# crate-crypto/rust-eth-kzg

Measured on AMD Instinct MI355X. Metric: blobs/sec compute_cells_and_kzg_proofs (4096-pt blob), higher is better.
Workload: dtype u32

## Files before the change

include/c_eth_kzg_test_hooks.h:

```cpp
#ifndef C_ETH_KZG_TEST_HOOKS_H
#define C_ETH_KZG_TEST_HOOKS_H
#include "c_eth_kzg.h"
#ifdef __cplusplus
extern "C" {
#endif

int eth_kzg_amd_test_fr_ntt4096(const DASContext *ctx, const uint8_t *in, uint8_t *out, int inverse_dit);
int eth_kzg_amd_test_g1_fft128(const DASContext *ctx, const uint8_t *in, uint8_t *out, int n_lanes, int inverse);
int eth_kzg_amd_test_fixed_msm(const DASContext *ctx, const uint8_t *scalars, int n_msm, uint8_t *out);
int eth_kzg_amd_test_g1_decompress(const DASContext *ctx, const uint8_t *in, int n, int subgroup_check, int32_t *status,
                                   uint8_t *out);
int eth_kzg_amd_test_field_mul(const DASContext *ctx, const uint8_t *a, const uint8_t *b, uint8_t *out, int n,
                               int is_fp);

int eth_kzg_amd_test_sha256_many(const DASContext *ctx, uint64_t n, const uint8_t *prefix, uint64_t prefix_len, const uint8_t *d_body,
                                 uint64_t body_stride, uint64_t body_len, const uint8_t *d_tail, uint64_t tail_stride, uint64_t tail_len,
                                 uint8_t *d_out);

int eth_kzg_amd_test_verify_msm(const DASContext *ctx, int form, const uint8_t *points, int n_pts, const uint8_t *sc0, int n0,
                                const uint8_t *sc1, int n1, uint8_t *out96, int32_t *sub_status);

int eth_kzg_amd_test_verify_cells_partial_device(const DASContext *ctx, uint64_t n, const uint8_t *d_commitments,
                                                 const uint64_t *d_cell_indices, const uint8_t *d_cells, const uint8_t *d_proofs, uint64_t lo,
                                                 uint64_t hi, uint8_t *out96);
int eth_kzg_amd_test_verify_blob_batch_inputs(const DASContext *ctx, uint64_t n, int on_device, const void *blobs, const void *commitments,
                                              const void *proofs, uint8_t *out96, int32_t *verified);

int eth_kzg_amd_test_rs_decode(const DASContext *ctx, int R, const uint64_t *n_cells, const uint64_t *const *cell_indices,
                               const uint8_t *const *const *cells, int flat_source, int32_t *status, int32_t *deg,
                               uint8_t *zp, uint8_t *zeval, uint8_t *zcinv, uint8_t *coeffs);

int eth_kzg_amd_test_op_info(int op, int32_t *in_words, int32_t *out_words, int32_t *device_only, const char **name);
int eth_kzg_amd_test_op(const DASContext *ctx, int op, int n, const int32_t *in, int32_t *out, int on_device);

int eth_kzg_amd_test_table_info(const DASContext *ctx, int kind, int which, int64_t *out8, int32_t *piece_first_block, int max_pieces);
int eth_kzg_amd_test_table_audit(const DASContext *ctx, int kind, int which, uint64_t *visited, uint64_t *n_findings, int32_t *findings,
                                 int max_findings, double *ms);
int eth_kzg_amd_test_table_read(const DASContext *ctx, int kind, int which, int group, int window, int base, int d0, int n, uint32_t *out);
int eth_kzg_amd_test_table_audit_buffer(const DASContext *ctx, int c, int n_groups, int nb, const uint32_t *table, const uint8_t *bases,
                                        int on_device, uint64_t *visited, uint64_t *n_findings, int32_t *findings, int max_findings);

#ifdef __cplusplus
}
#endif
#endif
```

rust-eth-kzg_amd/__init__.py:

```python
import ctypes as C

import numpy as np
import os

_HERE = os.path.dirname(os.path.abspath(__file__))
LIB_PATH = os.path.join(_HERE, "libc_eth_kzg.so")
HOOKS_LIB_PATH = os.path.join(_HERE, "libc_eth_kzg_hooks.so")

BYTES_PER_BLOB = 131072
BYTES_PER_CELL = 2048
BYTES_PER_COMMITMENT = 48
BYTES_PER_PROOF = 48
CELLS_PER_EXT_BLOB = 128
FIELD_ELEMENTS_PER_BLOB = 4096
FIELD_ELEMENTS_PER_CELL = 64


class KzgError(Exception):
    """An operation the reference would report as `Err(..)` (CResult.status == Err)."""


class CResult(C.Structure):
    _fields_ = [("status", C.c_int), ("error_msg", C.c_void_p)]


VERIFY_PARTIAL_BYTES = 96
SETUP_NO_SUBGROUP_CHECK = 1
SETUP_CHECK_POWERS = 2
SETUP_G1_POINTS = 4096
SETUP_G2_POINTS = 65

EXPORTED_SYMBOLS = [
    "eth_kzg_das_context_new", "eth_kzg_das_context_free", "eth_kzg_free_error_message",
    "eth_kzg_blob_to_kzg_commitment", "eth_kzg_compute_cells_and_kzg_proofs", "eth_kzg_compute_cells",
    "eth_kzg_verify_cell_kzg_proof_batch", "eth_kzg_recover_cells_and_proofs",
    "eth_kzg_constant_bytes_per_cell", "eth_kzg_constant_bytes_per_proof", "eth_kzg_constant_cells_per_ext_blob",
    "eth_kzg_compute_kzg_proof", "eth_kzg_compute_blob_kzg_proof", "eth_kzg_verify_kzg_proof",
    "eth_kzg_verify_blob_kzg_proof", "eth_kzg_verify_blob_kzg_proof_batch",
    "eth_kzg_amd_das_context_new_on_device",
    "eth_kzg_amd_das_context_try_new", "eth_kzg_amd_das_context_new_on_devices", "eth_kzg_amd_context_devices",
    "eth_kzg_amd_das_context_new_with_setup", "eth_kzg_amd_das_context_new_with_setup_file", "eth_kzg_amd_setup_digest",
    "eth_kzg_amd_abi_version", "eth_kzg_amd_window_count", "eth_kzg_amd_glv_table",
    "eth_kzg_amd_compute_cells_and_kzg_proofs_batch", "eth_kzg_amd_blob_to_kzg_commitment_batch",
    "eth_kzg_amd_recover_cells_and_proofs_batch", "eth_kzg_amd_recover_cells_and_proofs_device",
    "eth_kzg_amd_verify_cell_kzg_proof_batch_partial", "eth_kzg_amd_verify_cell_kzg_proof_batch_combine",
    "eth_kzg_amd_compute_cells_and_kzg_proofs_device", "eth_kzg_amd_blob_to_kzg_commitment_device",
    "eth_kzg_amd_verify_cell_kzg_proof_batch_device", "eth_kzg_amd_verify_cell_kzg_proof_batch_many",
    "eth_kzg_amd_compute_blob_kzg_proof_batch", "eth_kzg_amd_compute_kzg_proof_batch",
    "eth_kzg_amd_compute_blob_kzg_proof_device", "eth_kzg_amd_compute_kzg_proof_device",
    "eth_kzg_amd_verify_blob_kzg_proof_batch_device",
    "eth_kzg_amd_table_bytes", "eth_kzg_amd_window_bits", "eth_kzg_amd_tables_ready", "eth_kzg_amd_table_groups_ready", "eth_kzg_amd_table_build_info", "eth_kzg_amd_linmap_info",
    "eth_kzg_amd_set_profiling", "eth_kzg_amd_get_stage_times",
    "eth_kzg_amd_comm_probe", "eth_kzg_amd_comm_unique_id", "eth_kzg_amd_comm_init", "eth_kzg_amd_comm_info",
    "eth_kzg_amd_all_gather", "eth_kzg_amd_comm_destroy",
    "eth_kzg_amd_compute_cells_and_kzg_proofs_batch_multi", "eth_kzg_amd_device_count",
]
TEST_HOOK_SYMBOLS = [
    "eth_kzg_amd_test_fr_ntt4096", "eth_kzg_amd_test_g1_fft128", "eth_kzg_amd_test_fixed_msm",
    "eth_kzg_amd_test_g1_decompress", "eth_kzg_amd_test_field_mul", "eth_kzg_amd_test_op_info", "eth_kzg_amd_test_op",
    "eth_kzg_amd_test_table_info", "eth_kzg_amd_test_table_audit", "eth_kzg_amd_test_table_read", "eth_kzg_amd_test_table_audit_buffer",
    "eth_kzg_amd_test_sha256_many", "eth_kzg_amd_test_verify_msm",
    "eth_kzg_amd_test_verify_cells_partial_device", "eth_kzg_amd_test_verify_blob_batch_inputs", "eth_kzg_amd_test_rs_decode",
]

_lib = None


def load_library():
    global _lib
    if _lib is not None:
        return _lib
    path = os.environ.get("ETH_KZG_AMD_LIB", LIB_PATH)
    if not os.path.exists(path):
        raise RuntimeError(
            f"{LIB_PATH} is missing: build the HIP extension first (python -c 'import __graft_entry__ as g; g.build()' "
            "or make -C rust-eth-kzg_amd/csrc). There is no CPU fallback.")
    lib = C.CDLL(path)
    P, U8P, U64 = C.c_void_p, C.c_char_p, C.c_uint64
    lib.eth_kzg_das_context_new.restype = P
    lib.eth_kzg_das_context_new.argtypes = [C.c_bool]
    lib.eth_kzg_amd_das_context_new_on_device.restype = P
    lib.eth_kzg_amd_das_context_new_on_device.argtypes = [C.c_bool, C.c_int]
    lib.eth_kzg_amd_das_context_try_new.restype = P
    lib.eth_kzg_amd_das_context_try_new.argtypes = [C.c_bool, C.c_int, C.c_double, C.POINTER(CResult)]
    lib.eth_kzg_das_context_free.argtypes = [P]
    lib.eth_kzg_free_error_message.argtypes = [P]
    for name, args in {
        "eth_kzg_blob_to_kzg_commitment": [P, U8P, P],
        "eth_kzg_compute_cells_and_kzg_proofs": [P, U8P, P, P],
        "eth_kzg_compute_cells": [P, U8P, P],
        "eth_kzg_verify_cell_kzg_proof_batch": [P, U64, P, U64, P, U64, P, U64, P, P],
        "eth_kzg_recover_cells_and_proofs": [P, U64, P, U64, P, P, P],
        "eth_kzg_compute_kzg_proof": [P, U8P, U8P, P, P],
        "eth_kzg_compute_blob_kzg_proof": [P, U8P, U8P, P],
        "eth_kzg_verify_kzg_proof": [P, U8P, U8P, U8P, U8P, P],
        "eth_kzg_verify_blob_kzg_proof": [P, U8P, U8P, U8P, P],
        "eth_kzg_verify_blob_kzg_proof_batch": [P, U64, P, U64, P, U64, P, P],
        "eth_kzg_amd_compute_cells_and_kzg_proofs_batch": [P, U64, P, P, P, P],
        "eth_kzg_amd_blob_to_kzg_commitment_batch": [P, U64, P, P, P],
        "eth_kzg_amd_recover_cells_and_proofs_batch": [P, U64, P, P, P, P, P, P, P],
        "eth_kzg_amd_verify_cell_kzg_proof_batch_partial": [P, U64, P, U64, P, U64, P, U64, P, U64, U64, P],
        "eth_kzg_amd_verify_cell_kzg_proof_batch_combine": [P, U64, U8P, P],
        "eth_kzg_amd_recover_cells_and_proofs_device": [P, U64, P, P, P, P, P, P],
        "eth_kzg_amd_compute_cells_and_kzg_proofs_device": [P, U64, P, P, P, P, P],
        "eth_kzg_amd_blob_to_kzg_commitment_device": [P, U64, P, P, P, P],
        "eth_kzg_amd_verify_cell_kzg_proof_batch_device": [P, U64, P, P, P, P, P, P],
        "eth_kzg_amd_verify_cell_kzg_proof_batch_many": [P, U64, P, P, P, P, P, P, P, P, P, P],
        "eth_kzg_amd_compute_blob_kzg_proof_batch": [P, U64, P, P, P, P],
        "eth_kzg_amd_compute_kzg_proof_batch": [P, U64, P, P, P, P, P],
        "eth_kzg_amd_compute_blob_kzg_proof_device": [P, U64, P, P, P, P, P],
        "eth_kzg_amd_compute_kzg_proof_device": [P, U64, P, P, P, P, P, P],
        "eth_kzg_amd_verify_blob_kzg_proof_batch_device": [P, U64, P, P, P, P, P],
        "eth_kzg_amd_comm_unique_id": [P],
        "eth_kzg_amd_comm_probe": [P, P, U64],
        "eth_kzg_amd_comm_info": [P, P, P],
        "eth_kzg_amd_comm_init": [P, U8P, C.c_int, C.c_int],
        "eth_kzg_amd_all_gather": [P, P, P, U64, P],
        "eth_kzg_amd_compute_cells_and_kzg_proofs_batch_multi": [P, U64, U64, P, P, P, P],
    }.items():
        fn = getattr(lib, name)
        fn.restype = CResult
        fn.argtypes = args
    for name in ("eth_kzg_constant_bytes_per_cell", "eth_kzg_constant_bytes_per_proof",
                 "eth_kzg_constant_cells_per_ext_blob"):
        getattr(lib, name).restype = U64
    lib.eth_kzg_amd_comm_destroy.argtypes = [P]
    lib.eth_kzg_amd_comm_destroy.restype = None
    lib.eth_kzg_amd_device_count.restype = C.c_int
    lib.eth_kzg_amd_table_bytes.restype = U64
    lib.eth_kzg_amd_table_bytes.argtypes = [P]
    lib.eth_kzg_amd_window_bits.argtypes = [P]
    lib.eth_kzg_amd_tables_ready.argtypes = [P, C.c_int]
    lib.eth_kzg_amd_tables_ready.restype = C.c_int
    lib.eth_kzg_amd_table_build_info.argtypes = [P, C.POINTER(C.c_double)]
    lib.eth_kzg_amd_table_build_info.restype = None
    lib.eth_kzg_amd_table_groups_ready.argtypes = [P]
    lib.eth_kzg_amd_table_groups_ready.restype = C.c_int
    lib.eth_kzg_amd_linmap_info.argtypes = [P, P]
    lib.eth_kzg_amd_linmap_info.restype = None
    lib.eth_kzg_amd_set_profiling.argtypes = [P, C.c_int]
    lib.eth_kzg_amd_set_profiling.restype = None
    lib.eth_kzg_amd_get_stage_times.argtypes = [P, P, P, C.c_int]
    lib.eth_kzg_amd_das_context_new_on_devices.restype = P
    lib.eth_kzg_amd_das_context_new_on_devices.argtypes = [C.c_bool, P, U64, C.c_double, C.POINTER(CResult)]
    lib.eth_kzg_amd_context_devices.restype = U64
    lib.eth_kzg_amd_context_devices.argtypes = [P, P, U64]
    lib.eth_kzg_amd_abi_version.restype = C.c_int
    if hasattr(lib, "eth_kzg_amd_das_context_new_with_setup"):
        lib.eth_kzg_amd_das_context_new_with_setup.restype = P
        lib.eth_kzg_amd_das_context_new_with_setup.argtypes = [P, U64, P, U64, C.c_uint32, C.c_bool, P, U64, C.c_double, C.POINTER(CResult)]
        lib.eth_kzg_amd_das_context_new_with_setup_file.restype = P
        lib.eth_kzg_amd_das_context_new_with_setup_file.argtypes = [P, U64, C.c_uint32, C.c_bool, P, U64, C.c_double, C.POINTER(CResult)]
        lib.eth_kzg_amd_setup_digest.restype = None
        lib.eth_kzg_amd_setup_digest.argtypes = [P, P]
    lib.eth_kzg_amd_window_count.argtypes = [P]
    lib.eth_kzg_amd_glv_table.argtypes = [P]
    for name, args in {
        "eth_kzg_amd_test_fr_ntt4096": [P, U8P, P, C.c_int],
        "eth_kzg_amd_test_g1_fft128": [P, U8P, P, C.c_int, C.c_int],
        "eth_kzg_amd_test_fixed_msm": [P, U8P, C.c_int, P],
        "eth_kzg_amd_test_g1_decompress": [P, U8P, C.c_int, C.c_int, P, P],
        "eth_kzg_amd_test_field_mul": [P, U8P, U8P, P, C.c_int, C.c_int],
        "eth_kzg_amd_test_op_info": [C.c_int, P, P, P, C.POINTER(C.c_char_p)],
        "eth_kzg_amd_test_op": [P, C.c_int, C.c_int, P, P, C.c_int],
        "eth_kzg_amd_test_table_info": [P, C.c_int, C.c_int, P, P, C.c_int],
        "eth_kzg_amd_test_table_audit": [P, C.c_int, C.c_int, P, P, P, C.c_int, P],
        "eth_kzg_amd_test_table_read": [P, C.c_int, C.c_int, C.c_int, C.c_int, C.c_int, C.c_int, C.c_int, P],
        "eth_kzg_amd_test_table_audit_buffer": [P, C.c_int, C.c_int, C.c_int, P, P, C.c_int, P, P, P, C.c_int],
        "eth_kzg_amd_test_sha256_many": [P, U64, P, U64, P, U64, U64, P, U64, U64, P],
        "eth_kzg_amd_test_verify_msm": [P, C.c_int, U8P, C.c_int, U8P, C.c_int, U8P, C.c_int, P, P],
        "eth_kzg_amd_test_verify_cells_partial_device": [P, U64, P, P, P, P, U64, U64, P],
        "eth_kzg_amd_test_verify_blob_batch_inputs": [P, U64, C.c_int, P, P, P, P, P],
        "eth_kzg_amd_test_rs_decode": [P, C.c_int, P, P, P, C.c_int, P, P, P, P, P, P],
    }.items():
        if hasattr(lib, name):
            getattr(lib, name).argtypes = args
    _lib = lib
    return lib


def present_masks(n, present):
    masks = np.zeros(2 * max(1, n), dtype=np.uint64)
    prev_row, prev_mask = None, 0
    for b in range(n):
        row = present[b]
        if row is prev_row and prev_row is not None:
            m = prev_mask
        else:
            m = 0
            for c in row:
                c = int(c)
                if not 0 <= c < CELLS_PER_EXT_BLOB:
                    raise KzgError("InvalidCellIndex")
                m |= 1 << c
            prev_row, prev_mask = row, m
        masks[2 * b] = m & 0xFFFFFFFFFFFFFFFF
        masks[2 * b + 1] = m >> 64
    return masks


def parse_trusted_setup_json(text):
    import json
    try:
        doc = json.loads(text)
    except ValueError as e:
        raise KzgError(f"InvalidSetup: not JSON ({e})")
    if not isinstance(doc, dict):
        raise KzgError("InvalidSetup: the trusted setup JSON is an object with g1_monomial and g2_monomial")
    out = []
    for key, size in (("g1_monomial", 48), ("g2_monomial", 96)):
        pts = doc.get(key)
        if not isinstance(pts, list):
            raise KzgError(f"InvalidSetup: {key} is missing")
        dec = []
        for i, h in enumerate(pts):
            if not isinstance(h, str) or not h.startswith("0x"):
                raise KzgError(f"InvalidSetup: {key}[{i}] is not a 0x-prefixed hex string")
            try:
                b = bytes.fromhex(h[2:])
            except ValueError:
                raise KzgError(f"InvalidSetup: {key}[{i}] is not hex")
            if len(b) != size:
                raise KzgError(f"InvalidSetup: {key}[{i}] has {len(b)} bytes, not {size}")
            dec.append(b)
        out.append(dec)
    return out[0], out[1]


def _ptr_array(bufs):
    arr = (C.c_void_p * max(1, len(bufs)))()
    keep = []
    for i, b in enumerate(bufs):
        if isinstance(b, (bytes, bytearray)):
            b = C.create_string_buffer(bytes(b), len(b))
        keep.append(b)
        arr[i] = C.addressof(b)
    return arr, keep


def _flat_ptrs(items, size):
    n = len(items)
    flat = np.frombuffer(b"".join(bytes(x) if not isinstance(x, bytes) else x for x in items), dtype=np.uint8) if n else np.zeros(1, np.uint8)
    ptrs = np.uint64(flat.ctypes.data) + np.arange(max(1, n), dtype=np.uint64) * np.uint64(size)
    return ptrs, flat


def _out_ptrs(n_outer, n_inner, size):
    flat = np.zeros(max(1, n_outer * n_inner * size), dtype=np.uint8)
    inner = np.uint64(flat.ctypes.data) + np.arange(max(1, n_outer * n_inner), dtype=np.uint64) * np.uint64(size)
    outer = np.uint64(inner.ctypes.data) + np.arange(max(1, n_outer), dtype=np.uint64) * np.uint64(n_inner * 8)
    return flat, inner, outer


def _split(flat, n_outer, n_inner, size):
    raw = flat.tobytes()
    return [[raw[(b * n_inner + k) * size:(b * n_inner + k + 1) * size] for k in range(n_inner)] for b in range(n_outer)]


def _vp(arr):
    return arr.ctypes.data_as(C.c_void_p)


class DASContext:

    device_index = 0

    def __init__(self, use_precomp=True, device=None, wait_tables=True, table_budget_gb=None, devices=None):
        self.device_index = int(device) if device is not None else int(os.environ.get("ETH_KZG_AMD_DEVICE", "0"))
        self._lib = load_library()
        if devices is not None:
            devs = np.array([int(d) for d in devices], dtype=np.int32)
            self.device_index = int(devs[0]) if len(devs) else 0
            res = CResult()
            self._ctx = C.c_void_p(self._lib.eth_kzg_amd_das_context_new_on_devices(
                bool(use_precomp), _vp(devs) if len(devs) else None, len(devs), float(table_budget_gb or 0.0), C.byref(res)))
            if not self._ctx.value:
                msg = C.cast(res.error_msg, C.c_char_p).value.decode() if res.error_msg else "unknown"
                self._lib.eth_kzg_free_error_message(res.error_msg)
                raise KzgError(msg)
        elif table_budget_gb is not None:
            res = CResult()
            self._ctx = C.c_void_p(self._lib.eth_kzg_amd_das_context_try_new(bool(use_precomp), self.device_index, float(table_budget_gb), C.byref(res)))
            if not self._ctx.value:
                msg = C.cast(res.error_msg, C.c_char_p).value.decode() if res.error_msg else "unknown"
                self._lib.eth_kzg_free_error_message(res.error_msg)
                raise KzgError(msg)
        elif device is None:
            self._ctx = C.c_void_p(self._lib.eth_kzg_das_context_new(bool(use_precomp)))
        else:
            self._ctx = C.c_void_p(self._lib.eth_kzg_amd_das_context_new_on_device(bool(use_precomp), int(device)))
        if not self._ctx.value:
            raise RuntimeError("eth_kzg_das_context_new returned NULL")
        if wait_tables:
            self.tables_ready(-1)

    @classmethod
    def from_trusted_setup(cls, g1_monomial, g2_monomial, *, subgroup_check=True, check_powers=False, use_precomp=True, devices=None,
                           table_budget_gb=None, wait_tables=True):
        def flat(pts, size):
            if isinstance(pts, (bytes, bytearray, memoryview)):
                raw = bytes(pts)
                if len(raw) % size:
                    raise KzgError(f"InvalidSetup: {len(raw)} bytes are not a whole number of {size}-byte points")
                return raw, len(raw) // size
            pts = [bytes(x) for x in pts]
            for i, x in enumerate(pts):
                if len(x) != size:
                    raise KzgError(f"InvalidSetup: point {i} has {len(x)} bytes, not {size}")
            return b"".join(pts), len(pts)
        g1, n1 = flat(g1_monomial, 48)
        g2, n2 = flat(g2_monomial, 96)
        self = cls.__new__(cls)
        self._lib = load_library()
        self._ctx = C.c_void_p(None)
        devs = np.array([int(d) for d in devices], dtype=np.int32) if devices is not None else None
        self.device_index = int(devs[0]) if devs is not None and len(devs) else int(os.environ.get("ETH_KZG_AMD_DEVICE", "0"))
        flags = (0 if subgroup_check else SETUP_NO_SUBGROUP_CHECK) | (SETUP_CHECK_POWERS if check_powers else 0)
        res = CResult()
        b1, b2 = C.create_string_buffer(g1, max(1, len(g1))), C.create_string_buffer(g2, max(1, len(g2)))
        self._ctx = C.c_void_p(self._lib.eth_kzg_amd_das_context_new_with_setup(
            C.addressof(b1), n1, C.addressof(b2), n2, flags, bool(use_precomp), _vp(devs) if devs is not None and len(devs) else None,
            len(devs) if devs is not None else 0, float(table_budget_gb or 0.0), C.byref(res)))
        if not self._ctx.value:
            msg = C.cast(res.error_msg, C.c_char_p).value.decode() if res.error_msg else "unknown"
            self._lib.eth_kzg_free_error_message(res.error_msg)
            raise KzgError(msg)
        if wait_tables:
            self.tables_ready(-1)
        return self

    @classmethod
    def from_trusted_setup_json(cls, text_or_path, *, check_powers=True, **kwargs):
        text = text_or_path
        if not str(text_or_path).lstrip().startswith("{"):
            with open(text_or_path) as f:
                text = f.read()
        g1, g2 = parse_trusted_setup_json(text)
        return cls.from_trusted_setup(g1, g2, check_powers=check_powers, **kwargs)

    @property
    def setup_digest(self):
        out = C.create_string_buffer(32)
        self._lib.eth_kzg_amd_setup_digest(self._ctx, out)
        return out.raw

    def devices(self):
        out = np.zeros(64, dtype=np.int32)
        n = int(self._lib.eth_kzg_amd_context_devices(self._ctx, _vp(out), 64))
        return [int(d) for d in out[:n]]

    def tables_ready(self, wait_ms=0):
        return int(self._lib.eth_kzg_amd_tables_ready(self._ctx, int(wait_ms)))

    def table_build_info(self):
        out = (C.c_double * 4)()
        self._lib.eth_kzg_amd_table_build_info(self._ctx, out)
        return {"hipmalloc_ms": round(out[0], 1), "longest_hipmalloc_ms": round(out[1], 1), "pieces": int(out[2]), "bytes": int(out[3])}

    def table_groups_ready(self):
        return int(self._lib.eth_kzg_amd_table_groups_ready(self._ctx))

    def close(self):
        if getattr(self, "_ctx", None) and self._ctx.value:
            self._lib.eth_kzg_das_context_free(self._ctx)
            self._ctx = C.c_void_p(None)

    def __del__(self):
        try:
            self.close()
        except Exception:
            pass

    @property
    def handle(self):
        return self._ctx

    def _check(self, res):
        if res.status != 0:
            msg = C.string_at(res.error_msg).decode() if res.error_msg else "error"
            self._lib.eth_kzg_free_error_message(res.error_msg)
            raise KzgError(msg)

    def blob_to_kzg_commitment(self, blob):
        if len(blob) != BYTES_PER_BLOB:
            raise KzgError("BlobHasInvalidLength")
        out = C.create_string_buffer(48)
        self._check(self._lib.eth_kzg_blob_to_kzg_commitment(self._ctx, bytes(blob), out))
        return out.raw

    def compute_cells_and_kzg_proofs(self, blob):
        if len(blob) != BYTES_PER_BLOB:
            raise KzgError("BlobHasInvalidLength")
        cells = [C.create_string_buffer(BYTES_PER_CELL) for _ in range(CELLS_PER_EXT_BLOB)]
        proofs = [C.create_string_buffer(48) for _ in range(CELLS_PER_EXT_BLOB)]
        ca, _k1 = _ptr_array(cells)
        pa, _k2 = _ptr_array(proofs)
        self._check(self._lib.eth_kzg_compute_cells_and_kzg_proofs(self._ctx, bytes(blob), ca, pa))
        return [c.raw for c in cells], [p.raw for p in proofs]

    def compute_cells(self, blob):
        if len(blob) != BYTES_PER_BLOB:
            raise KzgError("BlobHasInvalidLength")
        cells = [C.create_string_buffer(BYTES_PER_CELL) for _ in range(CELLS_PER_EXT_BLOB)]
        ca, _k = _ptr_array(cells)
        self._check(self._lib.eth_kzg_compute_cells(self._ctx, bytes(blob), ca))
        return [c.raw for c in cells]

    def verify_cell_kzg_proof_batch(self, commitments, cell_indices, cells, proofs):
        if any(len(c) != 48 for c in commitments) or any(len(p) != 48 for p in proofs) \
                or any(len(c) != BYTES_PER_CELL for c in cells):
            raise KzgError("InvalidLength")
        ca, _k1 = _flat_ptrs(commitments, 48)
        cla, _k2 = _flat_ptrs(cells, BYTES_PER_CELL)
        pa, _k3 = _flat_ptrs(proofs, 48)
        idx = np.array(cell_indices, dtype=np.uint64) if len(cell_indices) else np.zeros(1, np.uint64)
        ok = C.c_bool(False)
        self._check(self._lib.eth_kzg_verify_cell_kzg_proof_batch(
            self._ctx, len(commitments), _vp(ca), len(cell_indices), _vp(idx), len(cells), _vp(cla), len(proofs), _vp(pa),
            C.byref(ok)))
        return bool(ok.value)

    def prepare_verify_cell_kzg_proof_batch(self, commitments, cell_indices, cells, proofs):
        if any(len(c) != 48 for c in commitments) or any(len(p) != 48 for p in proofs) \
                or any(len(c) != BYTES_PER_CELL for c in cells):
            raise KzgError("InvalidLength")
        ca, k1 = _flat_ptrs(commitments, 48)
        cla, k2 = _flat_ptrs(cells, BYTES_PER_CELL)
        pa, k3 = _flat_ptrs(proofs, 48)
        idx = np.array(cell_indices, dtype=np.uint64) if len(cell_indices) else np.zeros(1, np.uint64)
        n = (len(commitments), len(cell_indices), len(cells), len(proofs))

        def run(_keep=(k1, k2, k3)):
            ok = C.c_bool(False)
            self._check(self._lib.eth_kzg_verify_cell_kzg_proof_batch(
                self._ctx, n[0], _vp(ca), n[1], _vp(idx), n[2], _vp(cla), n[3], _vp(pa), C.byref(ok)))
            return bool(ok.value)
        return run

    def prepare_verify_cell_kzg_proof_batch_many(self, problems):
        nb = len(problems)
        keep, lens = [], np.zeros((4, max(1, nb)), dtype=np.uint64)
        tabs = [np.zeros(max(1, nb), dtype=np.uint64) for _ in range(4)]
        for b, (commitments, cell_indices, cells, proofs) in enumerate(problems):
            if any(len(c) != 48 for c in commitments) or any(len(p) != 48 for p in proofs) \
                    or any(len(c) != BYTES_PER_CELL for c in cells):
                commitments, cell_indices, cells, proofs = [], [0], [], []
            ca, k1 = _flat_ptrs(commitments, 48)
            cla, k2 = _flat_ptrs(cells, BYTES_PER_CELL)
            pa, k3 = _flat_ptrs(proofs, 48)
            idx = np.array(cell_indices, dtype=np.uint64) if len(cell_indices) else np.zeros(1, np.uint64)
            keep += [ca, k1, cla, k2, pa, k3, idx]
            lens[:, b] = (len(commitments), len(cell_indices), len(cells), len(proofs))
            tabs[0][b], tabs[1][b], tabs[2][b], tabs[3][b] = ca.ctypes.data, idx.ctypes.data, cla.ctypes.data, pa.ctypes.data
        lens = np.ascontiguousarray(lens)
        ver = (C.c_bool * max(1, nb))()
        st = (C.c_int32 * max(1, nb))()

        def run(_keep=keep):
            self._check(self._lib.eth_kzg_amd_verify_cell_kzg_proof_batch_many(
                self._ctx, nb, _vp(lens[0]), _vp(tabs[0]), _vp(lens[1]), _vp(tabs[1]), _vp(lens[2]), _vp(tabs[2]), _vp(lens[3]), _vp(tabs[3]),
                ver, st))
            return [bool(v) for v in ver][:nb], list(st)[:nb]
        return run

    def verify_cell_kzg_proof_batch_many(self, problems):
        return self.prepare_verify_cell_kzg_proof_batch_many(problems)()

    def verify_cell_kzg_proof_batch_partial(self, commitments, cell_indices, cells, proofs, shard_begin, shard_end):
        if any(len(c) != 48 for c in commitments) or any(len(p) != 48 for p in proofs) \
                or any(len(c) != BYTES_PER_CELL for c in cells):
            raise KzgError("InvalidLength")
        ca, _k1 = _flat_ptrs(commitments, 48)
        cla, _k2 = _flat_ptrs(cells, BYTES_PER_CELL)
        pa, _k3 = _flat_ptrs(proofs, 48)
        idx = np.array(cell_indices, dtype=np.uint64) if len(cell_indices) else np.zeros(1, np.uint64)
        out = C.create_string_buffer(VERIFY_PARTIAL_BYTES)
# ... 264 lines not shown
```

rust-eth-kzg_amd/csrc/c_api_hooks.cpp:

```cpp
#include "../../include/c_eth_kzg_test_hooks.h"
#include "c_ctx.hpp"
#include "launch.hpp"

#include <algorithm>
#include <array>
#include <cstdio>
#include <cstdlib>
#include <cstring>
#include <vector>

namespace {
kzg::Engine* eng(const DASContext* ctx) {
    if (!ctx || !ctx->engine) {
        fprintf(stderr, "c_eth_kzg: context pointer is null\n");
        abort();
    }
    return ctx->engine;
}
}

extern "C" {

int eth_kzg_amd_test_fr_ntt4096(const DASContext* ctx, const uint8_t* in, uint8_t* out, int inverse_dit) {
    return eng(ctx)->test_fr_ntt4096(in, out, inverse_dit);
}
int eth_kzg_amd_test_g1_fft128(const DASContext* ctx, const uint8_t* in, uint8_t* out, int n_lanes, int inverse) {
    return eng(ctx)->test_g1_fft128(in, out, n_lanes, inverse);
}
int eth_kzg_amd_test_fixed_msm(const DASContext* ctx, const uint8_t* scalars, int n_msm, uint8_t* out) {
    return eng(ctx)->test_fixed_msm(scalars, n_msm, out);
}
int eth_kzg_amd_test_g1_decompress(const DASContext* ctx, const uint8_t* in, int n, int subgroup_check, int32_t* status,
                                   uint8_t* out) {
    return eng(ctx)->test_g1_decompress(in, n, subgroup_check, status, out);
}
int eth_kzg_amd_test_field_mul(const DASContext* ctx, const uint8_t* a, const uint8_t* b, uint8_t* out, int n, int is_fp) {
    return eng(ctx)->test_field_mul(a, b, out, n, is_fp);
}
int eth_kzg_amd_test_sha256_many(const DASContext* ctx, uint64_t n, const uint8_t* prefix, uint64_t prefix_len, const uint8_t* d_body,
                                 uint64_t body_stride, uint64_t body_len, const uint8_t* d_tail, uint64_t tail_stride, uint64_t tail_len,
                                 uint8_t* d_out) {
    if (n > (1u << 24) || (prefix_len | body_len | tail_len) >> 31) return kzg::ERR_INPUT;
    return eng(ctx)->test_sha256_many((int)n, prefix, (uint32_t)prefix_len, d_body, body_stride, (uint32_t)body_len, d_tail, tail_stride,
                                      (uint32_t)tail_len, d_out);
}
int eth_kzg_amd_test_verify_msm(const DASContext* ctx, int form, const uint8_t* points, int n_pts, const uint8_t* sc0, int n0,
                                const uint8_t* sc1, int n1, uint8_t* out96, int32_t* sub_status) {
    if (!points || !sc0 || !sc1 || !out96) return kzg::ERR_INPUT;
    return eng(ctx)->test_verify_msm(form, points, n_pts, sc0, n0, sc1, n1, out96, sub_status);
}
int eth_kzg_amd_test_verify_cells_partial_device(const DASContext* ctx, uint64_t n, const uint8_t* d_commitments, const uint64_t* d_cell_indices,
                                                 const uint8_t* d_cells, const uint8_t* d_proofs, uint64_t lo, uint64_t hi, uint8_t* out96) {
    if (!d_commitments || !d_cell_indices || !d_cells || !d_proofs || !out96) return kzg::ERR_INPUT;
    return eng(ctx)->test_verify_cells_partial_device(n, d_commitments, d_cell_indices, d_cells, d_proofs, lo, hi, out96);
}
int eth_kzg_amd_test_verify_blob_batch_inputs(const DASContext* ctx, uint64_t n, int on_device, const void* blobs, const void* commitments,
                                              const void* proofs, uint8_t* out96, int32_t* verified) {
    if (!blobs || !commitments || !proofs || !out96 || !verified) return kzg::ERR_INPUT;
    int v = 0;
    const int rc = eng(ctx)->test_verify_blob_batch_inputs(n, on_device, blobs, commitments, proofs, out96, &v);
    *verified = v;
    return rc;
}
int eth_kzg_amd_test_rs_decode(const DASContext* ctx, int R, const uint64_t* n_cells, const uint64_t* const* cell_indices,
                               const uint8_t* const* const* cells, int flat_source, int32_t* status, int32_t* deg, uint8_t* zp, uint8_t* zeval,
                               uint8_t* zcinv, uint8_t* coeffs) {
    if (R < 1 || R > 4096 || !n_cells || !cell_indices || !cells || (flat_source != 0 && flat_source != 1)) return kzg::ERR_INPUT;
    for (int r = 0; r < R; r++) {
        if (n_cells[r] < 64 || n_cells[r] > 128 || !cell_indices[r] || !cells[r]) return kzg::ERR_INPUT;
        for (uint64_t k = 0; k < n_cells[r]; k++) {
            if (cell_indices[r][k] >= 128 || (k && cell_indices[r][k - 1] >= cell_indices[r][k])) return kzg::ERR_INPUT;
            if (!cells[r][flat_source ? 0 : k]) return kzg::ERR_INPUT;
        }
    }
    return eng(ctx)->test_rs_decode(R, n_cells, cell_indices, cells, flat_source, status, deg, zp, zeval, zcinv, coeffs);
}
int eth_kzg_amd_test_op_info(int op, int32_t* in_words, int32_t* out_words, int32_t* device_only, const char** name) {
    int i, o, d;
    const char* nm;
    if (kzg::launch::test_op_info(op, &i, &o, &d, &nm) != 0) return -1;
    *in_words = i;
    *out_words = o;
    *device_only = d;
    *name = nm;
    return 0;
}
int eth_kzg_amd_test_op(const DASContext* ctx, int op, int n, const int32_t* in, int32_t* out, int on_device) {
    if (on_device) return eng(ctx)->test_op(op, n, in, out);
    int i, o, d;
    const char* nm;
    if (kzg::launch::test_op_info(op, &i, &o, &d, &nm) != 0 || d || n <= 0) return kzg::ERR_INPUT;
    return kzg::launch::test_op_host(op, n, in, out) == 0 ? 0 : kzg::ERR_INPUT;
}

static bool glv_shape_ok(int c, int n_groups, int nb) {
    return kzg::launch::glv_width_supported(c) && n_groups >= 1 && n_groups <= 128 && nb >= 1 && nb <= 64;
}
int eth_kzg_amd_test_table_info(const DASContext* ctx, int kind, int which, int64_t* out8, int32_t* piece_first_block, int max_pieces) {
    return eng(ctx)->test_table_info(kind, which, out8, piece_first_block, max_pieces);
}
int eth_kzg_amd_test_table_audit(const DASContext* ctx, int kind, int which, uint64_t* visited, uint64_t* n_findings, int32_t* findings,
                                 int max_findings, double* ms) {
    return eng(ctx)->test_table_audit(kind, which, visited, n_findings, findings, max_findings, ms);
}
int eth_kzg_amd_test_table_read(const DASContext* ctx, int kind, int which, int group, int window, int base, int d0, int n, uint32_t* out) {
    return eng(ctx)->test_table_read(kind, which, group, window, base, d0, n, out);
}
int eth_kzg_amd_test_table_audit_buffer(const DASContext* ctx, int c, int n_groups, int nb, const uint32_t* table, const uint8_t* bases,
                                        int on_device, uint64_t* visited, uint64_t* n_findings, int32_t* findings, int max_findings) {
    if (!glv_shape_ok(c, n_groups, nb) || max_findings < 0) return kzg::ERR_INPUT;
    if (on_device) return eng(ctx)->test_table_audit_buffer(c, n_groups, nb, table, bases, visited, n_findings, findings, max_findings);
    const int WL = kzg::launch::glv_lower_windows(c), W = kzg::launch::glv_windows(c);
    const size_t lower = kzg::launch::glv_entries_per_base(c, 0, WL) * (size_t)nb, upper = kzg::launch::glv_entries_per_base(c, WL, W) * (size_t)nb;
    std::vector<const void*> blocks((size_t)2 * n_groups);
    const char* t = (const char*)table;
    for (int g = 0; g < n_groups; g++) {
        blocks[2 * g] = t + (size_t)g * (lower + upper) * kzg::launch::SIZEOF_TABP;
        blocks[2 * g + 1] = t + ((size_t)g * (lower + upper) + lower) * kzg::launch::SIZEOF_TABP;
    }
    unsigned long long v = 0, nf = 0;
    kzg::launch::table_audit_host(blocks.data(), bases, c, n_groups, nb, &v, &nf, findings, max_findings);
    std::vector<std::array<int32_t, 5>> f(std::min<unsigned long long>(nf, (unsigned long long)max_findings));
    if (!f.empty()) {
        memcpy(f.data(), findings, f.size() * sizeof(f[0]));
        std::sort(f.begin(), f.end());
        memcpy(findings, f.data(), f.size() * sizeof(f[0]));
    }
    *visited = v;
    *n_findings = nf;
    return 0;
}

}
```

rust-eth-kzg_amd/csrc/engine.hip:

```cpp
#include "engine_internal.hpp"

namespace kzg {

static Fr fr_from_u64(uint64_t v) {
    Fr a = zero<FrParams>();
    a.v[0] = (uint32_t)v;
    a.v[1] = (uint32_t)(v >> 32);
    return to_mont(a);
}
static Fr fr_pow_limbs(const Fr& base, const uint32_t* e, int nl) {
    Fr acc = one<FrParams>();
    for (int i = 32 * nl - 1; i >= 0; i--) {
        acc = sqr(acc);
        if ((e[i >> 5] >> (i & 31)) & 1) acc = mul(acc, base);
    }
    return acc;
}
static Fr fr_root_of_unity(int log_n) {
    uint32_t e[8];
    for (int i = 0; i < 8; i++) e[i] = FrParams::MOD[i];
    e[0] -= 1;
    for (int s = 0; s < log_n; s++) {
        for (int i = 0; i < 8; i++) e[i] = (e[i] >> 1) | (i < 7 ? (e[i + 1] << 31) : 0);
    }
    return fr_pow_limbs(fr_from_u64(7), e, 8);
}
typedef unsigned __int128 u128;
static const u128 GLV_LAMBDA = ((u128)0xac45a4010001a402ULL << 64) | 0x00000000ffffffffULL;
static void glv_split(const Fr& canon, u128& k1, u128& k2) {
    u128 rem = 0, q = 0;
    for (int i = 255; i >= 0; i--) {
        bool top = (rem >> 127) & 1;
        rem = (rem << 1) | ((canon.v[i >> 5] >> (i & 31)) & 1);
        q <<= 1;
        if (top || rem >= GLV_LAMBDA) { rem -= GLV_LAMBDA; q |= 1; }
    }
    k1 = rem;
    k2 = q;
}
static void recode_glv_wnaf(const Fr& k_mont, const Fr& lambda_mont, uint32_t* out) {
    constexpr int TWW = launch::TWIDDLE_WORDS, W = launch::TWIDDLE_WNAF_W;
    u128 r, q;
    glv_split(from_mont(k_mont), r, q);
    struct Half { u128 mag; bool neg; };
    auto signed_sub = [](u128 a, u128 b) { return a >= b ? Half{a - b, false} : Half{b - a, true}; };
    const Half cand[4][2] = {
        {Half{r, false}, Half{q, false}},
        {signed_sub(r, GLV_LAMBDA), Half{q + 1, false}},
        {signed_sub(r, 1), signed_sub(q, GLV_LAMBDA + 1)},
        {signed_sub(r, GLV_LAMBDA + 1), signed_sub(q, GLV_LAMBDA)},
    };
    auto fr_of = [](const Half& h) {
        Fr a = zero<FrParams>();
        for (int i = 0; i < 4; i++) a.v[i] = (uint32_t)(h.mag >> (32 * i));
        a = to_mont(a);
        return h.neg ? neg(a) : a;
    };
    auto naf = [&](const Half& h, int8_t* dg, int& len, int& weight) {
        u128 v = h.mag;
        len = weight = 0;
        for (int t = 0; v != 0; t++, v >>= 1) {
            if (t >= 4 * TWW) throw std::runtime_error("constant recoding too long");
            if (!(v & 1)) continue;
            int d = (int)(v & ((1u << W) - 1));
            if (d >= (1 << (W - 1))) d -= 1 << W;
            if (d < 0) v += (u128)(-d); else v -= (u128)d;
            dg[t] = (int8_t)(h.neg ? -d : d);
            len = t + 1;
            weight++;
        }
    };
    double best_cost = 0;
    int best = -1;
    std::vector<uint32_t> best_words;
    for (int c = 0; c < 4; c++) {
        if (!eq(add(fr_of(cand[c][0]), mul(fr_of(cand[c][1]), lambda_mont)), k_mont)) throw std::runtime_error("GLV split failed");
        std::vector<uint32_t> words(2 * TWW, 0u);
        int len[2], wt[2];
        for (int h = 0; h < 2; h++) naf(cand[c][h], reinterpret_cast<int8_t*>(&words[(size_t)h * TWW]), len[h], wt[h]);
        const double cost = linmap::COST_DBL * std::max(len[0], len[1]) + 5.0e3 * (wt[0] + wt[1]);
        if (best < 0 || cost < best_cost) { best = c; best_cost = cost; best_words = words; }
    }
    for (int i = 0; i < 2 * TWW; i++) out[i] = best_words[i];
    for (int h = 0; h < 2; h++) {
        const int8_t* dg = reinterpret_cast<const int8_t*>(out + (size_t)h * TWW);
        Fr back = zero<FrParams>(), pw = one<FrParams>();
        for (int t = 0; t < 4 * TWW; t++, pw = add(pw, pw)) {
            const int d = dg[t];
            if (!d) continue;
            Fr term = pw;
            for (int m = 1; m < (d < 0 ? -d : d); m++) term = add(term, pw);
            back = d < 0 ? sub(back, term) : add(back, term);
        }
        if (!eq(back, fr_of(cand[best][h]))) throw std::runtime_error("constant recoding failed");
    }
}
double trace_clock_ms() {
    static const auto t0 = std::chrono::steady_clock::now();
    return std::chrono::duration<double, std::milli>(std::chrono::steady_clock::now() - t0).count();
}
static thread_local std::string t_last_error;
const std::string& Engine::last_error() const { return t_last_error; }
void Engine::set_error(const std::exception& e) { t_last_error = e.what(); }

BufferPool::~BufferPool() {
    for (auto& f : free_) {
        if (host_) (void)hipHostFree(f.second);
        else (void)hipFree(f.second);
    }
}
void* BufferPool::get(size_t bytes, size_t* cls) {
    size_t c = 256;
    while (c < bytes) c <<= 1;
    *cls = c;
    for (size_t i = 0; i < free_.size(); i++)
        if (free_[i].first == c) {
            void* p = free_[i].second;
            free_[i] = free_.back();
            free_.pop_back();
            pooled_ -= c;
            return p;
        }
    void* p = nullptr;
    hipError_t e = host_ ? hipHostMalloc(&p, c, hipHostMallocDefault) : hipMalloc(&p, c);
    if (e != hipSuccess) {
        (void)hipGetLastError();
        for (auto& f : free_) { if (host_) (void)hipHostFree(f.second); else (void)hipFree(f.second); }
        free_.clear();
        pooled_ = 0;
        e = host_ ? hipHostMalloc(&p, c, hipHostMallocDefault) : hipMalloc(&p, c);
        if (e != hipSuccess) throw std::runtime_error(host_ ? "hipHostMalloc failed" : "hipMalloc failed");
    }
    return p;
}
void BufferPool::put(void* p, size_t cls) {
    constexpr size_t KEEP = 6ull << 30;
    if (pooled_ + cls > KEEP) {
        if (host_) (void)hipHostFree(p); else (void)hipFree(p);
        return;
    }
    free_.emplace_back(cls, p);
    pooled_ += cls;
}
PoolBuf::PoolBuf(Engine& e, size_t bytes, bool pinned_host) : e_(e), host_(pinned_host) {
    p = (host_ ? e_.pin_pool_ : e_.dev_pool_).get(bytes ? bytes : 1, &cls_);
}
PoolBuf::~PoolBuf() {
    (void)hipStreamSynchronize(e_.stream_);
    (host_ ? e_.pin_pool_ : e_.dev_pool_).put(p, cls_);
}

std::atomic<bool> g_exiting{false};
std::mutex g_engines_mu;
std::vector<Engine*> g_engines;
void Engine::stop_builder() {
    cancel_build_.store(true);
    if (builder_.joinable()) builder_.join();
}
void stop_all_builders_at_exit() {
    g_exiting.store(true);
    std::vector<Engine*> live;
    {
        std::lock_guard<std::mutex> lk(g_engines_mu);
        live = g_engines;
    }
    for (Engine* e : live) e->stop_builder();
}

Engine::SerialLease Engine::lease_serial() {
    return lanes_.lease(this, max_lanes_, auxiliary_, [this] {
        try {
            return std::unique_ptr<Engine>(new Engine(use_precomp_, dev_, this));
        } catch (...) {
            (void)hipGetLastError();
            throw;
        }
    });
}

Engine::Engine(bool use_precomp, int device, const Engine* primary, double table_budget_gb, std::shared_ptr<const TrustedSetup> setup)
    : dev_(device), use_precomp_(use_precomp), primary_(primary), auxiliary_(primary != nullptr) {
    setup_ = primary ? primary->setup_ : setup ? std::move(setup) : TrustedSetup::mainnet();
    knobs_ = primary ? primary->knobs_ : Knobs::from_env();
    if (knobs_.serial_lanes) max_lanes_ = knobs_.serial_lanes;
    if (knobs_.device_batch_max) device_batch_max_ = ((knobs_.device_batch_max + 63) / 64) * 64;
    if (use_precomp) {
        if (launch::glv_width_supported(knobs_.glv_window)) want_glv_c_ = knobs_.glv_window;
        if (table_budget_gb != 0) table_budget_gb_ = table_budget_gb;
        else if (knobs_.table_budget_gb != 0) table_budget_gb_ = knobs_.table_budget_gb;
    }
    vm_search_ = knobs_.vm_search;
    msm_split_ = knobs_.msm_split;
    if (knobs_.pip_shift_min >= 1) pip_shift_min_ = knobs_.pip_shift_min;
#ifdef KZG_CIRC_MAX
    circ_max_ = KZG_CIRC_MAX;
#else
    circ_max_ = 2;
#endif
    try {
        construct();
    } catch (...) {
        teardown();
        throw;
    }
}

void Engine::construct() {
    TraceLap lap{knobs_.trace, "context"};
    HIPCK(hipSetDevice(dev_));
    {
        int cus = 0;
        HIPCK(hipDeviceGetAttribute(&cus, hipDeviceAttributeMultiprocessorCount, dev_));
        wave_slots_ = cus * 4 * 2;
        if (knobs_.msm_chunks >= 0) msm_chunks_ = knobs_.msm_chunks;
    }
    HIPCK(hipStreamCreateWithFlags(&stream_, hipStreamNonBlocking));
    if (!primary_) {
        int prio_low = 0, prio_high = 0;
        HIPCK(hipDeviceGetStreamPriorityRange(&prio_low, &prio_high));
        HIPCK(hipStreamCreateWithPriority(&build_stream_, hipStreamNonBlocking, prio_low));
    }
    if (v_two_streams_) HIPCK(hipStreamCreateWithFlags(&v_side_, hipStreamNonBlocking));
    HIPCK(hipEventCreateWithFlags(&v_decoded_, hipEventDisableTiming));
    HIPCK(hipEventCreateWithFlags(&v_checked_, hipEventDisableTiming));
    for (Work& w : work_) {
        HIPCK(hipEventCreateWithFlags(&w.done, hipEventDisableTiming));
        HIPCK(hipEventCreateWithFlags(&w.ev_in, hipEventDisableTiming));
        HIPCK(hipEventCreateWithFlags(&w.ev_cells, hipEventDisableTiming));
        HIPCK(hipEventCreateWithFlags(&w.ev_cells_host, hipEventDisableTiming));
        HIPCK(hipEventCreateWithFlags(&w.ev_done, hipEventDisableTiming));
        HIPCK(hipEventCreateWithFlags(&w.ev_coeffs, hipEventDisableTiming));
        HIPCK(hipEventCreateWithFlags(&w.ev_side, hipEventDisableTiming));
        if (&w == &work_[0]) continue;
        if (primary_) continue;
        int prio_low = 0, prio_high = 0;
        HIPCK(hipDeviceGetStreamPriorityRange(&prio_low, &prio_high));
        HIPCK(hipStreamCreateWithFlags(&w.stream, hipStreamNonBlocking));
        HIPCK(hipStreamCreateWithPriority(&w.copy, hipStreamNonBlocking, prio_high));
    }
    launch::init_attributes();
    if (!primary_) settle_streams();
    lap("HIP runtime + stream");
    init_constants();
    lap("twiddles, recodings");
    init_srs();
    lap("SRS decompress");
    init_fk20();
    lap("FK20 bases + start tables");
    init_verifier();
    HIPCK(hipStreamSynchronize(stream_));
    lap("verifier (G2 lines, cosets)");
    if (setup_->check_powers && !primary_) {
        check_setup_powers();
        lap("setup: powers of one tau");
    }
    if (knobs_.fault == "constructor" && !primary_) throw std::runtime_error("injected fault (ETH_KZG_AMD_FAULT=constructor)");
    start_builder();
}

bool Engine::streams_overlap(hipStream_t a, hipStream_t b) {
    int khz = 0;
    if (hipDeviceGetAttribute(&khz, hipDeviceAttributeWallClockRate, dev_) != hipSuccess || khz <= 0) khz = 100000;
    const double spin_us = 300.0;
    const uint64_t ticks = (uint64_t)(spin_us * 1e-3 * khz);
    for (int t = 0; t < 3; t++) {
        HIPCK(hipStreamSynchronize(a));
        HIPCK(hipStreamSynchronize(b));
        const auto t0 = std::chrono::steady_clock::now();
        launch::spin(ticks, a);
        launch::spin(ticks, b);
        HIPCK(hipStreamSynchronize(a));
        HIPCK(hipStreamSynchronize(b));
        const double us = std::chrono::duration<double, std::micro>(std::chrono::steady_clock::now() - t0).count();
        if (us < 1.6 * spin_us) return true;
    }
    return false;
}
void Engine::settle_streams() {
    const bool trace = knobs_.trace;
    launch::spin(1, stream_);
    std::vector<hipStream_t> chosen{stream_}, rejected;
    bool gave_up = false;
    for (int i = 1; i < NW; i++) {
        Work& w = work_[i];
        if (!w.stream || gave_up) continue;
        for (int attempt = 0;; attempt++) {
            launch::spin(1, w.stream);
            bool ok = true;
            for (hipStream_t c : chosen) ok = ok && streams_overlap(c, w.stream);
            if (ok || attempt == 5) {
                if (trace) fprintf(stderr, "[eth_kzg_amd] work set %d: stream %s after %d replacement(s)\n", i, ok ? "runs beside the others" : "still shares a queue", attempt);
                if (!ok) gave_up = true;
                break;
            }
            rejected.push_back(w.stream);
            HIPCK(hipStreamCreateWithFlags(&w.stream, hipStreamNonBlocking));
        }
        chosen.push_back(w.stream);
    }
    for (hipStream_t r : rejected) hipStreamDestroy(r);
}

Engine::~Engine() { teardown(); }

void Engine::teardown() noexcept {
    (void)hipSetDevice(dev_);
    lanes_.clear();
    stop_builder();
    {
        std::lock_guard<std::mutex> lk(g_engines_mu);
        g_engines.erase(std::remove(g_engines.begin(), g_engines.end(), this), g_engines.end());
    }
    if (build_stream_) hipStreamDestroy(build_stream_);
    host_pool_.reset();
    vm_pool_.reset();
    stage_pool_.reset();
    void* ptrs[] = {d_w8192_, d_w29_, d_naf_, d_srs_, d_fk_bases_, d_in_, d_cells_, d_proofs_, d_coset_, d_coset_inv_, d_circ_terms_, d_4844_};
    for (void* p : ptrs)
        if (p) hipFree(p);
    for (SlpProgram& P : slp_prog_) {
        if (P.d_words) hipFree(P.d_words);
        if (P.d_naf && P.owns_naf) hipFree(P.d_naf);
    }
    for (Work& w : work_) {
        void* dev[] = {w.coeffs, w.canon, w.scalars, w.X, w.status, w.circ_table, w.slp_arena, w.d_in, w.d_cells, w.d_proofs};
        for (void* p : dev)
            if (p) hipFree(p);
        void* pin[] = {w.h_in, w.h_cells, w.h_proofs, w.h_status};
        for (void* p : pin)
            if (p) hipHostFree(p);
        hipEvent_t evs[] = {w.done, w.ev_in, w.ev_cells, w.ev_cells_host, w.ev_done, w.ev_coeffs, w.ev_side};
        for (hipEvent_t e : evs)
            if (e) hipEventDestroy(e);
        for (hipEvent_t e : w.sub_events) hipEventDestroy(e);
        if (w.stream) hipStreamDestroy(w.stream);
        if (w.copy) hipStreamDestroy(w.copy);
    }
    if (v_dev_) hipFree(v_dev_);
    if (v_pin_) hipHostFree(v_pin_);
    for (VmSlot& v : vm_slot_) {
        if (v.dev) hipFree(v.dev);
        if (v.pin) hipHostFree(v.pin);
        if (v.vs.dev) hipFree(v.vs.dev);
        if (v.vs.pin) hipHostFree(v.vs.pin);
    }
    if (vd_pin_) hipHostFree(vd_pin_);
    for (hipEvent_t e : vd_events_)
        if (e) hipEventDestroy(e);
    if (v_side_) hipStreamDestroy(v_side_);
    if (v_decoded_) hipEventDestroy(v_decoded_);
    if (v_checked_) hipEventDestroy(v_checked_);
    if (stream_) hipStreamDestroy(stream_);
}

void Engine::init_constants() {
    std::vector<Fr> w(N_EXT);
    Fr g = fr_root_of_unity(13);
    w[0] = one<FrParams>();
    for (int i = 1; i < N_EXT; i++) w[i] = mul(w[i - 1], g);
    if (!eq(mul(w[N_EXT - 1], g), one<FrParams>())) throw std::runtime_error("omega_8192 has wrong order");
    HIPCK(hipMalloc(&d_w8192_, N_EXT * sizeof(Fr)));
    HIPCK(hipMemcpy(d_w8192_, w.data(), N_EXT * sizeof(Fr), hipMemcpyHostToDevice));
    {
        std::vector<uint32_t> w29((size_t)N_EXT * 9);
        launch::ntt_twiddles29(w.data(), w29.data());
        HIPCK(hipMalloc(&d_w29_, w29.size() * 4));
        HIPCK(hipMemcpy(d_w29_, w29.data(), w29.size() * 4, hipMemcpyHostToDevice));
    }
    {
        Fr lam = zero<FrParams>();
        for (int i = 0; i < 4; i++) lam.v[i] = (uint32_t)(GLV_LAMBDA >> (32 * i));
        Fr lm = to_mont(lam);
        if (!is_zero(add(add(sqr(lm), lm), one<FrParams>()))) throw std::runtime_error("GLV lambda is not a cube root of unity");
        constexpr int TWW = launch::TWIDDLE_WORDS;
        std::vector<uint32_t> tw((size_t)128 * 2 * TWW, 0u);
        for (int k = 0; k < 128; k++) recode_glv_wnaf(w[64 * k], lm, &tw[(size_t)k * 2 * TWW]);
        HIPCK(hipMalloc(&d_naf_, tw.size() * 4));
        HIPCK(hipMemcpy(d_naf_, tw.data(), tw.size() * 4, hipMemcpyHostToDevice));
        std::vector<uint32_t> plus, minus;
        int max_t = 0;
        for (int d = 0; d < 128; d++) {
            Fr c = zero<FrParams>();
            for (int t = 0; t < 64; t++) c = add(c, w[(64 * d * t) & (N_EXT - 1)]);
            if (d != 0 && (d & 1) == 0) {
                if (!is_zero(c)) throw std::runtime_error("circulant symbol: even entry is not zero");
                continue;
            }
            u128 kk[2];
            glv_split(from_mont(c), kk[0], kk[1]);
            Fr back = zero<FrParams>();
            for (int half = 0; half < 2; half++) {
                u128 k = kk[half];
                Fr pw = half ? lm : one<FrParams>();
                for (int t = 0; k != 0; t++, k >>= 1, pw = add(pw, pw)) {
                    if (!(k & 1)) continue;
                    const int dg = 2 - (int)(k & 3);
                    if (dg < 0) k += 1;
                    const uint32_t word = (uint32_t)d | ((uint32_t)t << 7) | ((uint32_t)half << 15) | ((dg < 0 ? 1u : 0u) << 16) | (1u << 17);
                    (dg < 0 ? minus : plus).push_back(word);
                    back = dg < 0 ? sub(back, pw) : add(back, pw);
                    if (t > max_t) max_t = t;
                }
            }
            if (!eq(back, c)) throw std::runtime_error("circulant term list does not reproduce its symbol");
        }
        if ((int)plus.size() < launch::CIRC_LANES || max_t >= 255) throw std::runtime_error("circulant term list is malformed");
        std::vector<uint32_t> all(plus);
        all.insert(all.end(), minus.begin(), minus.end());
        circ_T_ = max_t + 1;
        circ_per_lane_ = ((int)all.size() + launch::CIRC_LANES - 1) / launch::CIRC_LANES;
        all.resize((size_t)circ_per_lane_ * launch::CIRC_LANES, 0u);
        HIPCK(hipMalloc(&d_circ_terms_, all.size() * 4));
        HIPCK(hipMemcpy(d_circ_terms_, all.data(), all.size() * 4, hipMemcpyHostToDevice));
    }
    init_linmap(reinterpret_cast<const Fr8*>(w.data()));
    for (int sgi = 0; sgi < 3; sgi++) {
        Fr v = zero<FrParams>();
        v.v[sgi + 1] = 1;
        v = to_mont(v);
        memcpy(&seg_shift_[sgi], &v, 32);
    }
    Fr i4096 = inv(fr_from_u64(N_BLOB)), i128 = inv(fr_from_u64(128));
    memcpy(&n_inv4096_, &i4096, 32);
    memcpy(&inv128_, &i128, 32);
}

static linmap::Strategy slp_strategy(int id) {
    linmap::Strategy s;
    s.allow_toom8 = true;
    {
        Fr lam = zero<FrParams>();
        for (int i = 0; i < 4; i++) lam.v[i] = (uint32_t)(GLV_LAMBDA >> (32 * i));
        s.lambda = to_mont(lam);
    }
    auto fixed = [&](int k4, int k8, int k16, int k32) {
        s.tuned = false;
        s.balanced_lincomb = true;
        s.phi = false;
        s.hankel_split = {{2, 2}, {4, k4}, {8, k8}, {16, k16}, {32, k32}};
    };
    switch (id) {
        case 2: fixed(2, 2, 2, 2); break;
        case 3: fixed(4, 2, 4, 2); break;
        case 4: fixed(2, 2, 2, 4); break;
        case 5: fixed(4, 2, 4, 8); break;
        default: break;
    }
    return s;
}
void Engine::build_slp_program(int id) {
    const Fr* w128p = reinterpret_cast<const Fr*>(w128_.data());
    const std::vector<Fr> w128(w128p, w128p + 128);
    const bool verbose = knobs_.trace;
    linmap::Plan plan = linmap::build_fk20_proofs_plan(w128, slp_strategy(id), verbose);
    {
        std::vector<linmap::Ref> perm(128);
        for (int p = 0; p < 128; p++) {
            int k = 0;
            for (int b = 0; b < 7; b++) k |= ((p >> b) & 1) << (6 - b);
            perm[p] = plan.outputs[k];
        }
        plan.outputs = perm;
    }
    const linmap::Schedule sched = linmap::make_schedule(plan, id == SLP_TUNED_FUSED);
    uint64_t st = 0x853c49e6748fea9bull + (uint64_t)id;
    for (int it = 0; it < 2; it++) {
        std::vector<Fr> in(128);
        for (auto& v : in) {
            for (int i = 0; i < 8; i++) { st ^= st << 13; st ^= st >> 7; st ^= st << 17; v.v[i] = (uint32_t)(st >> 16); }
            v.v[7] &= 0x3fffffffu;
        }
        const auto want = linmap::fk20_proofs_map_by_definition(w128, in);
        const auto got1 = linmap::run_over_fr(plan, in);
        const auto got2 = linmap::run_schedule_over_fr(sched, plan.consts, 128, 128, in);
        for (int p = 0; p < 128; p++) {
            int k = 0;
            for (int b = 0; b < 7; b++) k |= ((p >> b) & 1) << (6 - b);
            if (!eq(want[k], got1[p]) || !eq(want[k], got2[p])) throw std::runtime_error("FK20 proofs map: compiled program differs from its definition");
        }
    }
    SlpProgram& P = slp_prog_[id];
    if (id == SLP_TUNED && slp_prog_[SLP_TUNED_FUSED].ready) {
        P.d_naf = slp_prog_[SLP_TUNED_FUSED].d_naf;
    } else {
        Fr lam = zero<FrParams>();
        for (int i = 0; i < 4; i++) lam.v[i] = (uint32_t)(GLV_LAMBDA >> (32 * i));
        const Fr lm = to_mont(lam);
        constexpr int TWW = launch::TWIDDLE_WORDS;
        std::vector<uint32_t> naf(plan.consts.size() * 2 * TWW);
        for (size_t c = 0; c < plan.consts.size(); c++) recode_glv_wnaf(plan.consts[c], lm, &naf[c * 2 * TWW]);
        HIPCK(hipMalloc(&P.d_naf, naf.size() * 4));
        P.owns_naf = true;
        HIPCK(hipMemcpy(P.d_naf, naf.data(), naf.size() * 4, hipMemcpyHostToDevice));
    }
    HIPCK(hipMalloc(&P.d_words, sched.words.size() * 4));
    HIPCK(hipMemcpy(P.d_words, sched.words.data(), sched.words.size() * 4, hipMemcpyHostToDevice));
    P.launches.clear();
    for (auto& L : sched.launches) P.launches.push_back(SlpLaunch{(int)L.kind, L.first, L.count});
    P.n_slots = sched.n_slots;
    P.info[0] = (int)plan.count(linmap::OP_MULC);
    P.info[1] = (int)(plan.count(linmap::OP_ADD) + plan.count(linmap::OP_SUB));
    P.info[2] = (int)plan.doublings();
    P.info[3] = (int)sched.launches.size();
    if (verbose) fprintf(stderr, "[linmap] program %d: %d multiplications, %d additions, %d doublings, %d launches, %d slots\n", id, P.info[0], P.info[1], P.info[2], P.info[3], P.n_slots);
    P.ready = true;
}
const Engine::SlpProgram& Engine::slp_program(int id) {
    std::lock_guard<std::mutex> lk(slp_build_mu_);
    if (!slp_prog_[id].ready) build_slp_program(id);
    return slp_prog_[id];
}
int Engine::pick_slp_program(int lanes) const {
    if (slp_force_ >= 0) return slp_force_;
    const int groups = lanes / 64, simds = wave_slots_ / 2;
    if (712 * groups <= simds) return SLP_KARATSUBA;
    if (456 * groups <= simds) return SLP_DEPTH_456;
    if (606 * groups <= wave_slots_) return SLP_DEPTH_606;
    if (456 * groups <= wave_slots_) return SLP_DEPTH_456;
    if (372 * groups <= wave_slots_) return SLP_DEPTH_372;
    if (456 * groups <= wave_slots_ * 3 / 2) return SLP_DEPTH_456;
    if (groups <= 12) return SLP_DEPTH_372;
    return lanes >= slp_fuse_min_ ? SLP_TUNED_FUSED : SLP_TUNED;
}
void Engine::init_linmap(const Fr8* w8192_mont) {
    static_assert(sizeof(Fr8) == sizeof(Fr), "layout");
    if (knobs_.slp_program >= 0 && knobs_.slp_program < SLP_COUNT) slp_force_ = knobs_.slp_program;
    w128_.resize(128);
    for (int e = 0; e < 128; e++) w128_[e] = w8192_mont[64 * e];
    build_slp_program(SLP_TUNED_FUSED);
    build_slp_program(SLP_TUNED);
    const SlpProgram& fused = slp_prog_[SLP_TUNED_FUSED];
    {
        if (fused.info[0] != slp_prog_[SLP_TUNED].info[0]) throw std::runtime_error("FK20 proofs map: the two schedules differ");
    }
    for (int i = 0; i < 3; i++) slp_info_[i] = fused.info[i];
    slp_info_[3] = fused.info[3];
    const Fr h = inv(fr_from_u64(2));
    memcpy(&half_, &h, 32);
}

void Engine::init_srs() {
    const TrustedSetup& ts = *setup_;
    if (ts.g1.size() != (size_t)N_BLOB * 48) throw std::runtime_error("trusted setup: wrong number of G1 points");
    const bool checked = ts.subgroup_check && !ts.embedded && !primary_;
    uint8_t* d_bytes = nullptr;
    int* d_st = nullptr;
    std::vector<int> st(N_BLOB);
    struct Scratch {
        uint8_t*& b;
        int*& s;
        ~Scratch() { if (b) (void)hipFree(b); if (s) (void)hipFree(s); }
    } scratch{d_bytes, d_st};
    HIPCK(hipMalloc(&d_bytes, (size_t)N_BLOB * 48));
    HIPCK(hipMalloc(&d_st, N_BLOB * sizeof(int)));
    HIPCK(hipMalloc(&d_srs_, N_BLOB * sizeof(G1Affine)));
    HIPCK(hipMemcpy(d_bytes, ts.g1.data(), (size_t)N_BLOB * 48, hipMemcpyHostToDevice));
    {
        Fp12w nobeta{};
        launch::g1_decompress(d_bytes, d_srs_, d_st, N_BLOB, 0, nobeta, stream_);
    }
    HIPCK(hipMemcpyAsync(st.data(), d_st, N_BLOB * sizeof(int), hipMemcpyDeviceToHost, stream_));
    HIPCK(hipStreamSynchronize(stream_));
    for (int i = 0; i < N_BLOB; i++) {
        if (st[i]) throw std::runtime_error("g1_monomial[" + std::to_string(i) + "] is not the encoding of a curve point");
        if ((ts.g1[(size_t)i * 48] >> 6) & 1) throw std::runtime_error("g1_monomial[" + std::to_string(i) + "] is the point at infinity");
    }
    {
        G1Affine P;
        HIPCK(hipMemcpy(&P, (const G1Affine*)d_srs_ + 1, sizeof(G1Affine), hipMemcpyDeviceToHost));
        uint32_t lam[4];
        for (int i = 0; i < 4; i++) lam[i] = (uint32_t)(GLV_LAMBDA >> (32 * i));
        G1Affine Q = to_affine(scalar_mul<4>(to_jac(P), lam));
        Fp bx = mul(Q.x, inv(P.x));
        Fp b3 = mul(sqr(bx), bx);
        if (!eq(b3, one<FpParams>()) || eq(bx, one<FpParams>()) || !eq(Q.y, P.y)) {
            if (!ts.embedded) throw std::runtime_error("g1_monomial[1] is not in the prime-order subgroup (the endomorphism check failed on it)");
            throw std::runtime_error("GLV endomorphism check failed");
        }
        memcpy(&beta_, &bx, 48);
    }
    if (checked) {
        launch::g1_decompress(d_bytes, d_srs_, d_st, N_BLOB, 1, beta_, stream_);
        HIPCK(hipMemcpyAsync(st.data(), d_st, N_BLOB * sizeof(int), hipMemcpyDeviceToHost, stream_));
        HIPCK(hipStreamSynchronize(stream_));
        for (int i = 0; i < N_BLOB; i++) {
            if (st[i] == 2) throw std::runtime_error("g1_monomial[" + std::to_string(i) + "] is not in the prime-order subgroup");
            if (st[i]) throw std::runtime_error("g1_monomial[" + std::to_string(i) + "] is not the encoding of a curve point");
        }
    }
}

}
```

rust-eth-kzg_amd/csrc/engine.hpp:

```cpp
#pragma once
#include "knobs.hpp"
#include "host_sync.hpp"
#include "trusted_setup.hpp"
#include <hip/hip_runtime.h>
#include <cstddef>
#include <cstdint>
#include <atomic>
#include <condition_variable>
#include <deque>
#include <functional>
#include <mutex>
#include <thread>
#include <string>
#include <utility>
#include <vector>
#include <memory>

namespace kzg {

namespace pairing { struct G2Prepared; }
struct Comm;
struct G1Affine;
struct Fr8 { uint32_t v[8]; };
struct Fp12w { uint32_t v[12]; };

constexpr uint64_t MAX_CELLS_PER_VERIFICATION = (1u << 24) - 1;

enum Status : int {
    OK = 0,
    ERR_SCALAR = 1,
    ERR_G1 = 2,
    ERR_INPUT = 3,
    ERR_RECOVERY = 4,
    ERR_DEVICE = 5,
};

class BufferPool {
public:
    explicit BufferPool(bool pinned_host) : host_(pinned_host) {}
    ~BufferPool();
    void* get(size_t bytes, size_t* cls);
    void put(void* p, size_t cls);
private:
    bool host_;
    std::vector<std::pair<size_t, void*>> free_;
    size_t pooled_ = 0;
};
class Engine;
struct PoolBuf {
    void* p = nullptr;
    PoolBuf(Engine& e, size_t bytes, bool pinned_host = false);
    ~PoolBuf();
    PoolBuf(const PoolBuf&) = delete;
    PoolBuf& operator=(const PoolBuf&) = delete;
private:
    Engine& e_;
    size_t cls_ = 0;
    bool host_;
};

struct Work {
    std::mutex mu;
    int cap = 0;
    void *coeffs = nullptr, *canon = nullptr, *scalars = nullptr, *X = nullptr;
    int* status = nullptr;
    void *circ_table = nullptr, *slp_arena = nullptr;
    size_t slp_arena_bytes = 0;
    hipEvent_t done = nullptr;
    int stage_cap = 0;
    uint8_t *d_in = nullptr, *d_cells = nullptr, *d_proofs = nullptr;
    uint8_t *h_in = nullptr, *h_cells = nullptr, *h_proofs = nullptr;
    int* h_status = nullptr;
    hipStream_t stream = nullptr, copy = nullptr;
    hipEvent_t ev_in = nullptr, ev_cells = nullptr, ev_cells_host = nullptr, ev_done = nullptr;
    hipEvent_t ev_coeffs = nullptr, ev_side = nullptr;
    std::vector<hipEvent_t> sub_events;
};
class Engine {
public:
    friend struct PoolBuf;
    struct SharedTable;
    Engine(bool use_precomp, int device, const Engine* primary = nullptr, double table_budget_gb = 0,
           std::shared_ptr<const TrustedSetup> setup = nullptr);
    static constexpr double DEFAULT_TABLE_BUDGET_GB = 108.0;
    ~Engine();
    Engine(const Engine&) = delete;

    using SerialLease = LanePool<Engine>::Lease;
    friend class LanePool<Engine>;

    SerialLease lease_serial();

    int device() const { return dev_; }
    const TrustedSetup& setup() const { return *setup_; }
    Comm* comm() const { return comm_; }
    void set_comm(Comm* c) { comm_ = c; }
    hipStream_t stream() const { return stream_; }
    const std::string& last_error() const;

    int compute_cells_and_kzg_proofs_device(int n, const uint8_t* d_blobs, uint8_t* d_cells, uint8_t* d_proofs,
                                            int* h_status, hipStream_t stream, bool sync);
    int blob_to_kzg_commitment_device(int n, const uint8_t* d_blobs, uint8_t* d_commitments, int* h_status,
                                      hipStream_t stream, bool sync);

    int compute_cells_and_kzg_proofs_host(int n, const uint8_t* const* blobs, uint8_t* const* const* cells,
                                          uint8_t* const* const* proofs, int* h_status);
    int blob_to_kzg_commitment_host(int n, const uint8_t* const* blobs, uint8_t* const* out, int* h_status);

    int verify_cell_kzg_proof_batch_host(uint64_t n_commitments, const uint8_t* const* commitments, uint64_t n_indices,
                                         const uint64_t* cell_indices, uint64_t n_cells, const uint8_t* const* cells,
                                         uint64_t n_proofs, const uint8_t* const* proofs, int* verified);
    int verify_cell_kzg_proof_batch_device(uint64_t n, const uint8_t* d_commitments, const uint64_t* d_cell_indices,
                                           const uint8_t* d_cells, const uint8_t* d_proofs, int* verified, hipStream_t stream);
    int verify_cell_kzg_proof_batch_many_host(uint64_t n_batches, const uint64_t* n_commitments, const uint8_t* const* const* commitments,
                                              const uint64_t* n_indices, const uint64_t* const* cell_indices, const uint64_t* n_cells,
                                              const uint8_t* const* const* cells, const uint64_t* n_proofs,
                                              const uint8_t* const* const* proofs, int* verified, int* status);
    int verify_cell_kzg_proof_batch_combined(uint64_t n_commitments, const uint8_t* const* commitments, uint64_t n_indices,
                                             const uint64_t* cell_indices, uint64_t n_cells, const uint8_t* const* cells,
                                             uint64_t n_proofs, const uint8_t* const* proofs, int* verified);
    int verify_cell_kzg_proof_batch_partial_host(uint64_t n_commitments, const uint8_t* const* commitments, uint64_t n_indices,
                                                 const uint64_t* cell_indices, uint64_t n_cells, const uint8_t* const* cells,
                                                 uint64_t n_proofs, const uint8_t* const* proofs, uint64_t lo, uint64_t hi,
                                                 uint8_t* out96);
    int verify_cell_kzg_proof_batch_combine_host(uint64_t n_partials, const uint8_t* partials96, int* verified);
    int recover_cells_and_kzg_proofs_host(uint64_t n_cells, const uint8_t* const* cells, uint64_t n_indices,
                                          const uint64_t* cell_indices, uint8_t* const* out_cells,
                                          uint8_t* const* out_proofs);

    int compute_kzg_proof_host(const uint8_t* blob, const uint8_t* z, uint8_t* out_proof, uint8_t* out_y);
    int compute_blob_kzg_proof_host(const uint8_t* blob, const uint8_t* commitment, uint8_t* out_proof);
    int verify_kzg_proof_host(const uint8_t* commitment, const uint8_t* z, const uint8_t* y, const uint8_t* proof, int* verified);
    int verify_blob_kzg_proof_host(const uint8_t* blob, const uint8_t* commitment, const uint8_t* proof, int* verified);
    int verify_blob_kzg_proof_batch_host(uint64_t n_blobs, const uint8_t* const* blobs, uint64_t n_commitments,
                                         const uint8_t* const* commitments, uint64_t n_proofs, const uint8_t* const* proofs,
                                         int* verified, G1Affine* sums2 = nullptr);
    int compute_blob_kzg_proof_device(int n, const uint8_t* d_blobs, const uint8_t* d_commitments, uint8_t* d_out_proofs, int* h_status,
                                      hipStream_t stream, bool sync);
    int compute_kzg_proof_device(int n, const uint8_t* d_blobs, const uint8_t* d_z, uint8_t* d_out_proofs, uint8_t* d_out_y, int* h_status,
                                 hipStream_t stream, bool sync);
    int compute_blob_kzg_proof_batch_host(int n, const uint8_t* const* blobs, const uint8_t* const* commitments, uint8_t* const* out_proofs,
                                          int* h_status);
    int compute_kzg_proof_batch_host(int n, const uint8_t* const* blobs, const uint8_t* const* zs, uint8_t* const* out_proofs,
                                     uint8_t* const* out_ys, int* h_status);
    int verify_blob_kzg_proof_batch_device(uint64_t n, const uint8_t* d_blobs, const uint8_t* d_commitments, const uint8_t* d_proofs,
                                           int* verified, hipStream_t stream, G1Affine* sums2 = nullptr);

    int recover_cells_and_kzg_proofs_device(int R, const uint8_t* d_cells, const uint64_t* present_masks, uint8_t* d_out_cells,
                                            uint8_t* d_out_proofs, int* status, hipStream_t stream);
    int recover_cells_and_kzg_proofs_batch_host(int R, const uint64_t* n_cells, const uint8_t* const* const* cells,
                                                const uint64_t* n_indices, const uint64_t* const* cell_indices,
                                                uint8_t* const* const* out_cells, uint8_t* const* const* out_proofs,
                                                int* status);

    int test_fr_ntt4096(const uint8_t* in_be, uint8_t* out_be, int inverse_dit);
    int test_g1_fft128(const uint8_t* in_compressed, uint8_t* out_compressed, int n_lanes, int inverse);
    int test_fixed_msm(const uint8_t* scalars_be, int n_msm, uint8_t* out_compressed);
    int test_g1_decompress(const uint8_t* in, int n, int subgroup_check, int* h_status, uint8_t* out_recompressed);
    int test_field_mul(const uint8_t* a, const uint8_t* b, uint8_t* out, int n, int is_fp);
    int test_op(int op, int n, const int32_t* in, int32_t* out);
    int test_sha256_many(int n, const uint8_t* prefix, uint32_t prefix_len, const uint8_t* d_body, size_t body_stride, uint32_t body_len,
                         const uint8_t* d_tail, size_t tail_stride, uint32_t tail_len, uint8_t* d_out);
    int test_verify_msm(int form, const uint8_t* points, int n_pts, const uint8_t* sc0_be, int n0, const uint8_t* sc1_be, int n1,
                        uint8_t* out96, int32_t* h_status);
    int test_verify_cells_partial_device(uint64_t n, const uint8_t* d_commitments, const uint64_t* d_cell_indices, const uint8_t* d_cells,
                                         const uint8_t* d_proofs, uint64_t lo, uint64_t hi, uint8_t* out96);
    int test_verify_blob_batch_inputs(uint64_t n, int on_device, const void* blobs, const void* commitments, const void* proofs, uint8_t* out96,
                                      int* verified);
    int test_rs_decode(int R, const uint64_t* n_cells, const uint64_t* const* cell_indices, const uint8_t* const* const* cells, int flat_source,
                       int32_t* status, int32_t* deg, uint8_t* zp, uint8_t* zeval, uint8_t* zcinv, uint8_t* coeffs);
    std::shared_ptr<SharedTable> test_table(int kind, int which) const;
    int test_table_info(int kind, int which, int64_t* out8, int32_t* piece_first_block, int max_pieces);
    int test_table_audit(int kind, int which, uint64_t* visited, uint64_t* n_findings, int32_t* findings, int max_findings, double* ms);
    int test_table_read(int kind, int which, int group, int window, int base, int d0, int n, uint32_t* out);
    int test_table_audit_buffer(int c, int n_groups, int nb, const uint32_t* table, const uint8_t* bases, uint64_t* visited, uint64_t* n_findings,
                                int32_t* findings, int max_findings);

    enum Stage { ST_BLOB_TO_COEFFS = 0, ST_COEFFS_TO_CELLS, ST_FK20_SCALARS, ST_MSM_FIXED, ST_G1_IFFT, ST_G1_FFT,
                 ST_COMPRESS, ST_G1_LINMAP, ST_COUNT };
    void set_profiling(bool on);
    void get_stage_times(double* ms, uint64_t* launches);

    struct TableView {
        std::shared_ptr<SharedTable> main, next;
        int c = 0;
        size_t bytes = 0;
    };
    enum TableSel { TAB_FK = 0, TAB_SRS = 1 };
    TableView table_view(TableSel which) const;
    int tables_ready(int wait_ms);
    int table_groups_ready(TableSel which) const;
    void table_build_info(double* out4) const;
    void stop_builder();
    size_t table_bytes() const { return table_view(TAB_FK).bytes + table_view(TAB_SRS).bytes; }
    int window_bits() const { return table_view(TAB_FK).c; }
    int window_count() const { const int c = window_bits(); return c > 0 ? (128 + c - 1) / c : 0; }
    const int* linmap_info() const { return slp_info_; }

private:
    void construct();
    void teardown() noexcept;
    void start_builder();
    void init_constants();
    void init_linmap(const Fr8* w8192_mont);
    void init_srs();
    void check_setup_powers();
    void settle_streams();
    bool streams_overlap(hipStream_t a, hipStream_t b);
    void init_fk20();
    void init_verifier();
    int open_blobs_at(int n, const uint8_t* const* blobs, const Fr8* z_mont, bool want_proofs, uint8_t* h_proofs, Fr8* h_y_canon,
                      int* h_status);
    void open_blobs_core(int n, const uint8_t* d_blobs, const void* d_z_mont, void* d_y, uint8_t* d_proofs, hipStream_t st);
    struct Scratch4844 {
        uint8_t *dig = nullptr, *proofs = nullptr;
        void *z = nullptr, *y = nullptr, *aff = nullptr;
        int *blob_bad = nullptr, *z_bad = nullptr, *g1_bad = nullptr, *status = nullptr;
    };
    Scratch4844 scratch_4844(int n);
    void fs_challenges_device(int n, const uint8_t* d_blobs, const uint8_t* d_commitments, const Scratch4844& s, hipStream_t st);
    int finish_verify_blob_batch(int n, const Fr8* z_mont, const Fr8* y_canon, const uint8_t* const* commitments, const uint8_t* const* proofs,
                                 const void* d_points, G1Affine* sums2 = nullptr);
    int proofs_batch_host(int n, const uint8_t* const* blobs, const uint8_t* const* commitments, const uint8_t* const* zs,
                          uint8_t* const* out_proofs, uint8_t* const* out_ys, int* h_status);
    void open_staged_blobs(int nb, const uint8_t* h_blobs_pinned, const Fr8* z_mont, const uint8_t* h_commitments, uint8_t* h_proofs, Fr8* h_y,
                           int* h_blob_status, int* h_g1_status);
    HostPool* ensure_host_pool();
    void* d_4844_ = nullptr;
    int cap_4844_ = 0;
    int pairing_check_4844(const void* d_points, const std::vector<Fr8>& sc0, const std::vector<Fr8>& sc1, G1Affine* sums2 = nullptr);
    struct VerifyScratch {
        hipStream_t stream = nullptr;
        void* dev = nullptr;
        size_t dev_cap = 0;
        uint8_t* pin = nullptr;
        size_t pin_cap = 0;
    };
    struct VerifyDeviceSource {
        const uint8_t *d_cells, *d_proofs;
        hipEvent_t* chunk_events;
        int chunk_cells, n_chunks;
    };
    int verify_cells_partial(uint64_t n_commitments, const uint8_t* const* commitments, uint64_t n_indices,
                             const uint64_t* cell_indices, uint64_t n_cells, const uint8_t* const* cells, uint64_t n_proofs,
                             const uint8_t* const* proofs, uint64_t lo, uint64_t hi, G1Affine* out2, bool* empty,
                             const VerifyDeviceSource* dsrc = nullptr, VerifyScratch* vs = nullptr);
    int verify_cells_partial_device(uint64_t n, const uint8_t* d_commitments, const uint64_t* d_cell_indices, const uint8_t* d_cells,
                                    const uint8_t* d_proofs, uint64_t lo, uint64_t hi, G1Affine* out2, bool* empty, hipStream_t user_stream);
    bool verify_cells_pairing(const G1Affine* pts2) const;
    bool verify_cells_pairing_split(const G1Affine* pts2);
    struct RsDecodeTap { int* deg = nullptr; Fr8 *zp = nullptr, *zeval = nullptr, *zcinv = nullptr; };
    int rs_decode(int R, const uint8_t* d_cells, bool flat_source, const std::vector<int>& slot, const std::vector<int>& stof,
                  const std::vector<uint32_t>& present, int* st_out, const RsDecodeTap* tap = nullptr);
    int recover_batch_to_coeffs(int R, const uint64_t* n_cells, const uint8_t* const* const* cells,
                                const uint64_t* const* cell_indices, int* st_out);
    void ensure_workspace(int n);
    void ensure_workspace(Work& w, int n, bool release = false);
    void ensure_staging(Work& w, int n);
    void run_proofs_from_coeffs(int n, uint8_t* d_proofs, hipStream_t st) { run_proofs_from_coeffs(work_[0], n, d_proofs, st); }
    enum ProofsPhase { PROOFS_ALL = 0, PROOFS_HEAD = 1, PROOFS_TAIL = 2 };
    void run_proofs_from_coeffs(Work& w, int n, uint8_t* d_proofs, hipStream_t st, const TableView* tv_pre = nullptr, ProofsPhase phase = PROOFS_ALL,
                                int msm_cut = 0);
    void enqueue_compute(Work& w, int n, const uint8_t* d_blobs, uint8_t* d_cells, uint8_t* d_proofs, hipStream_t st,
                         hipEvent_t after_cells);
    Work& lease_work(int first, int last);
    void release_work(Work& w);
    std::mutex lease_mu_;
    std::condition_variable lease_cv_;
    void set_error(const std::exception& e);
    void launch_msm(const void* scalars, TableSel table, void* out, int n_groups, int n_slices, int out_stride,
                    int brp_bits, hipStream_t st, int out_fmt );
    void launch_msm(const void* scalars, const TableView& tv, bool scalars_split, void* out, int n_groups, int n_slices, int out_stride,
                    int brp_bits, hipStream_t st, int out_fmt );
    void launch_msm_range(const void* scalars, const SharedTable& t, int g0, int gcnt, void* out, int n_groups, int n_slices, int out_stride,
                          int brp_bits, hipStream_t st, int out_fmt);
    long msm_waves(long msms, int c) const;
    void build_final_tables();
    void publish(TableSel which, const std::shared_ptr<SharedTable>& main, const std::shared_ptr<SharedTable>& next);
    void g1_fft128_full(void* X, int stride, int inverse, hipStream_t st);

    struct StageMark { int stage; int launches; hipEvent_t a, b; };
    int mark_begin(int stage, hipStream_t st);
    void mark_end(int mark, int launches, hipStream_t st);
    bool profiling_ = false;
    std::vector<StageMark> marks_;
    unsigned marks_gen_ = 0;
    std::mutex marks_mu_;

    int dev_ = 0;
    std::shared_ptr<const TrustedSetup> setup_;
    Comm* comm_ = nullptr;
    bool use_precomp_ = true;
    Knobs knobs_;
    int want_glv_c_ = 0;
    double table_budget_gb_ = DEFAULT_TABLE_BUDGET_GB;
    mutable std::mutex tab_mu_;
    std::condition_variable tab_cv_;
    std::weak_ptr<SharedTable> start_tab_[2];
    Published<SharedTable> pub_[2];
    int tables_state_ = 0;
    std::string tables_error_;
    std::thread builder_;
    std::atomic<bool> cancel_build_{false};
    bool progressive_build_ = false;
    hipStream_t build_stream_ = nullptr;
    int wave_slots_ = 2048;
    int device_batch_max_ = 4096;
    int msm_chunks_ = -1;
    bool msm_split_ = true;
    hipStream_t stream_ = nullptr;
    std::recursive_mutex mu_;
    static constexpr int NW = 4;
    Work work_[NW];
    std::unique_ptr<HostPool> host_pool_;
    std::once_flag host_pool_once_;

    void* d_w8192_ = nullptr;
    void* d_w29_ = nullptr;
    void* d_naf_ = nullptr;
    Fp12w beta_;
    void* d_srs_ = nullptr;
    void* d_fk_bases_ = nullptr;
    BufferPool dev_pool_{false}, pin_pool_{true};
    Fr8 n_inv4096_, inv128_;

    void* d_coset_ = nullptr;
    void* d_coset_inv_ = nullptr;
    Fr8 inv64_, n_inv8192_;
    std::shared_ptr<pairing::G2Prepared> g2_tau_, g2_neg_gen_;
    std::shared_ptr<pairing::G2Prepared> g2_tau1_;

    void* v_dev_ = nullptr;
    size_t v_dev_cap_ = 0;
    uint8_t* v_pin_ = nullptr;
    size_t v_pin_cap_ = 0;
    hipStream_t v_side_ = nullptr;
    bool v_two_streams_ = false;
    hipEvent_t v_decoded_ = nullptr, v_checked_ = nullptr;

    const Engine* primary_ = nullptr;
    bool auxiliary_ = false;
    std::mutex lane_busy_;
    LanePool<Engine> lanes_;
    int max_lanes_ = 4;

    struct VerifyRequest;
    Combiner<VerifyRequest> combiner_{VM_SLOTS};
    std::atomic<int> verify_inflight_{0};
    int verify_lanes_ = 1;
    int comb_max_cells_ = 1024;

    static constexpr int VM_SLOTS = 3;
    struct VmSlot {
        VerifyScratch vs;
        void* dev = nullptr;
        size_t dev_cap = 0;
        uint8_t* pin = nullptr;
        size_t pin_cap = 0;
    };
    VmSlot vm_slot_[VM_SLOTS];
    SlotSet<VM_SLOTS> vm_slots_;
    std::unique_ptr<HostPool> stage_pool_;
    std::once_flag stage_pool_once_;
    std::unique_ptr<HostPool> vm_pool_;
    std::once_flag vm_pool_once_;
    bool vm_search_ = true;
    int vm_small_max_ = -1;
    uint8_t* vd_pin_ = nullptr;
    size_t vd_pin_cap_ = 0;
    static constexpr int VD_CHUNKS = 8;
    hipEvent_t vd_events_[VD_CHUNKS] = {};

    void *d_circ_terms_ = nullptr;
    int pip_shift_min_ = 1;
    int circ_T_ = 0, circ_per_lane_ = 0, circ_max_ = 2;
    Fr8 seg_shift_[3];
    struct SlpLaunch { int kind, first, count; };
    enum SlpProgramId { SLP_TUNED_FUSED = 0, SLP_TUNED = 1, SLP_KARATSUBA = 2, SLP_DEPTH_456 = 3, SLP_DEPTH_606 = 4, SLP_DEPTH_372 = 5, SLP_COUNT = 6 };
    struct SlpProgram {
        std::vector<SlpLaunch> launches;
        void *d_words = nullptr, *d_naf = nullptr;
        bool owns_naf = false, ready = false;
        int n_slots = 0;
        int info[4] = {0, 0, 0, 0};
    };
    SlpProgram slp_prog_[SLP_COUNT];
    std::mutex slp_build_mu_;
    std::vector<Fr8> w128_;
    const SlpProgram& slp_program(int id);
    void build_slp_program(int id);
    int pick_slp_program(int lanes) const;
    int slp_force_ = -1;
    int slp_fuse_min_ = 1024;
    int slp_info_[4] = {0, 0, 0, 0};
    Fr8 half_;

    int& cap_ = work_[0].cap;
    void *&d_coeffs_ = work_[0].coeffs, *&d_canon_ = work_[0].canon, *&d_scalars_ = work_[0].scalars, *&d_X_ = work_[0].X;
    int*& d_status_ = work_[0].status;
    uint8_t *d_in_ = nullptr, *d_cells_ = nullptr, *d_proofs_ = nullptr;
    int stage_cap_ = 0;
};

}
```

rust-eth-kzg_amd/csrc/engine_prover.hip:

```cpp
#include "engine_internal.hpp"

namespace kzg {

void Engine::set_profiling(bool on) { std::lock_guard<std::mutex> lk(marks_mu_); profiling_ = on; }
int Engine::mark_begin(int stage, hipStream_t st) {
    if (!profiling_) return -1;
    std::lock_guard<std::mutex> lk(marks_mu_);
    StageMark m{stage, 0, nullptr, nullptr};
    HIPCK(hipEventCreate(&m.a));
    HIPCK(hipEventCreate(&m.b));
    HIPCK(hipEventRecord(m.a, st));
    marks_.push_back(m);
    return (int)((marks_gen_ & 0x7ff) << 20) | ((int)marks_.size() - 1);
}
void Engine::mark_end(int mark, int launches, hipStream_t st) {
    if (mark < 0) return;
    std::lock_guard<std::mutex> lk(marks_mu_);
    const int idx = mark & 0xfffff;
    if (((mark >> 20) & 0x7ff) != (int)(marks_gen_ & 0x7ff) || idx >= (int)marks_.size()) return;
    marks_[idx].launches = launches;
    HIPCK(hipEventRecord(marks_[idx].b, st));
}
void Engine::get_stage_times(double* ms, uint64_t* launches) {
    std::lock_guard<std::mutex> lk(marks_mu_);
    for (int i = 0; i < ST_COUNT; i++) { ms[i] = 0; launches[i] = 0; }
    hipSetDevice(dev_);
    hipDeviceSynchronize();
    for (auto& m : marks_) {
        float t = 0;
        if (hipEventElapsedTime(&t, m.a, m.b) == hipSuccess) { ms[m.stage] += t; launches[m.stage] += m.launches; }
        hipEventDestroy(m.a);
        hipEventDestroy(m.b);
    }
    marks_.clear();
    marks_gen_++;
}

void Engine::ensure_workspace(int n) {
    ensure_workspace(work_[0], n);
    HIPCK(hipStreamWaitEvent(stream_, work_[0].done, 0));
}
void Engine::ensure_workspace(Work& w, int n, bool release) {
    if (n <= w.cap && !release) return;
    int cap = ((n + 63) / 64) * 64;
    void** ptrs[] = {&w.coeffs, &w.canon, &w.scalars, &w.X, (void**)&w.status};
    for (void** p : ptrs)
        if (*p) { HIPCK(hipFree(*p)); *p = nullptr; }
    w.cap = 0;
    if (release) {
        if (w.slp_arena) { HIPCK(hipFree(w.slp_arena)); w.slp_arena = nullptr; w.slp_arena_bytes = 0; }
        return;
    }
    HIPCK(hipMalloc(&w.coeffs, (size_t)cap * N_BLOB * sizeof(Fr)));
    if (&w == &work_[0]) HIPCK(hipMalloc(&w.canon, (size_t)cap * N_BLOB * sizeof(Fr)));
    HIPCK(hipMalloc(&w.scalars, (size_t)cap * 128 * 64 * sizeof(Fr)));
    HIPCK(hipMalloc(&w.X, (size_t)cap * 128 * launch::SIZEOF_JACS));
    HIPCK(hipMalloc(&w.status, (size_t)cap * sizeof(int)));
    w.cap = cap;
}
void Engine::ensure_staging(Work& w, int n) {
    if (n <= w.stage_cap) return;
    void* dev[] = {w.d_in, w.d_cells, w.d_proofs};
    for (void* p : dev)
        if (p) HIPCK(hipFree(p));
    void* pin[] = {w.h_in, w.h_cells, w.h_proofs, w.h_status};
    for (void* p : pin)
        if (p) HIPCK(hipHostFree(p));
    w.d_in = w.d_cells = w.d_proofs = w.h_in = w.h_cells = w.h_proofs = nullptr;
    w.h_status = nullptr;
    w.stage_cap = 0;
    HIPCK(hipMalloc(&w.d_in, (size_t)n * BYTES_PER_BLOB));
    HIPCK(hipMalloc(&w.d_cells, (size_t)n * N_CELLS * BYTES_PER_CELL));
    HIPCK(hipMalloc(&w.d_proofs, (size_t)n * N_CELLS * 48));
    HIPCK(hipHostMalloc(&w.h_in, (size_t)n * BYTES_PER_BLOB, hipHostMallocDefault));
    HIPCK(hipHostMalloc(&w.h_cells, (size_t)n * N_CELLS * BYTES_PER_CELL, hipHostMallocDefault));
    HIPCK(hipHostMalloc(&w.h_proofs, (size_t)n * N_CELLS * 48, hipHostMallocDefault));
    HIPCK(hipHostMalloc(&w.h_status, (size_t)n * sizeof(int), hipHostMallocDefault));
    w.stage_cap = n;
}
Work& Engine::lease_work(int first, int last) {
    std::unique_lock<std::mutex> lk(lease_mu_);
    for (;;) {
        for (int i = first; i <= last; i++)
            if (work_[i].mu.try_lock()) return work_[i];
        lease_cv_.wait_for(lk, std::chrono::milliseconds(2));
    }
}
void Engine::release_work(Work& w) {
    w.mu.unlock();
    lease_cv_.notify_one();
}

void Engine::launch_msm(const void* scalars, TableSel which, void* out, int n_groups, int n_slices, int out_stride,
                        int brp_bits, hipStream_t st, int out_fmt) {
    launch_msm(scalars, table_view(which), false, out, n_groups, n_slices, out_stride, brp_bits, st, out_fmt);
}
void Engine::launch_msm(const void* scalars, const TableView& tv, bool scalars_split, void* out, int n_groups, int n_slices,
                        int out_stride, int brp_bits, hipStream_t st, int out_fmt) {
    const SharedTable* main = tv.main.get();
    const SharedTable* next = tv.next.get();
    int ready = 0;
    if (next) ready = std::min(n_groups, next->ready_groups.load(std::memory_order_acquire));
    if (!scalars_split) launch::glv_split(const_cast<void*>(scalars), (size_t)n_groups * n_slices * 64, st);
    if (ready > 0) launch_msm_range(scalars, *next, 0, ready, out, n_groups, n_slices, out_stride, brp_bits, st, out_fmt);
    if (ready < n_groups) launch_msm_range(scalars, *main, ready, n_groups - ready, out, n_groups, n_slices, out_stride, brp_bits, st, out_fmt);
}
long Engine::msm_waves(long msms, int c) const {
    const long W = launch::glv_windows(c);
    if (msm_chunks_ > 0 || (msm_chunks_ < 0 && (msms * 4 + 63) / 64 >= (long)wave_slots_)) return msms * 4;
    if (msm_chunks_ < 0 && msm_split_ && (msms * 4 * W + 63) / 64 <= (long)wave_slots_ / 2) return (msms * 4 * W + 63) / 64;
    return (msms * 2 * W + 63) / 64;
}
void Engine::launch_msm_range(const void* scalars, const SharedTable& t, int g0, int gcnt, void* out, int n_groups, int n_slices,
                              int out_stride, int brp_bits, hipStream_t st, int out_fmt) {
    const launch::TabBlocks tb{(const void* const*)t.d_blocks, g0, gcnt};
    const int c = t.c;
    const long msms = (long)gcnt * n_slices;
    int mode = 1;
    if (n_slices <= FLAT_MSM_MAX_SLICES && circ_max_ > 0) mode = 0;
    else if (msm_chunks_ >= 0) mode = msm_chunks_ == 0 ? 1 : 2;
    else if (msm_split_ && (msms * 4 * launch::glv_windows(c) + 63) / 64 <= (long)wave_slots_ / 2) mode = 3;
    else if ((msms * 4 + 63) / 64 >= (long)wave_slots_) {
        mode = 2;
    }
    if (mode == 1 && msm_chunks_ < 0 && msm_split_) {
        const long per_slice = (long)gcnt * 2 * launch::glv_windows(c), slots = (long)wave_slots_ * 64, lanes = per_slice * n_slices;
        const int n_a = (int)(slots / per_slice);
        if (lanes > slots && lanes * 4 <= slots * 5 && n_a >= 1 && n_a < n_slices) {
            const size_t pt = out_fmt == launch::FMT_JACS ? launch::SIZEOF_JACS : launch::SIZEOF_JACQ;
            launch::msm_glv(c, 1, scalars, tb, out, n_groups, n_a, 64, out_stride, brp_bits, beta_, st, out_fmt);
            const int n_b = n_slices - n_a;
            launch::msm_glv(c, (n_b <= FLAT_MSM_MAX_SLICES && circ_max_ > 0) ? 0 : 3, (const char*)scalars + (size_t)n_a * n_groups * 64 * sizeof(Fr), tb,
                            (char*)out + (size_t)n_a * pt, n_groups, n_b, 64, out_stride, brp_bits, beta_, st, out_fmt);
            return;
        }
    }
    launch::msm_glv(c, mode, scalars, tb, out, n_groups, n_slices, 64, out_stride, brp_bits, beta_, st, out_fmt);
}

void Engine::g1_fft128_full(void* X, int stride, int inverse, hipStream_t st) {
    if (!inverse) {
        for (int half = 64; half >= 1; half >>= 1)
            launch::g1_fft_layer(X, stride, half, 128 / (2 * half), 0, 1, d_naf_, beta_, st);
    } else {
        for (int half = 1; half <= 64; half <<= 1)
            launch::g1_fft_layer(X, stride, half, 128 / (2 * half), 1, 0, d_naf_, beta_, st);
    }
}

void Engine::run_proofs_from_coeffs(Work& w, int n, uint8_t* d_proofs, hipStream_t st, const TableView* tv_pre, ProofsPhase phase, int msm_cut) {
    const int bp = ((n + 63) / 64) * 64;
    const int segs = (n > circ_max_ || circ_T_ > 129) ? 1 : n <= 2 ? 4 : n <= 4 ? 2 : 1;
    const Fr8 two_segments[3] = {seg_shift_[1], seg_shift_[1], seg_shift_[1]};
    const bool linmap_mode = n > circ_max_;
    void* X = w.X;
    const SlpProgram* prog = nullptr;
    int mulc_coop_lanes = 0;
    if (linmap_mode) {
        int which = pick_slp_program(bp);
        if (slp_force_ < 0 && bp == 64 && n > 32 && launch::coop_points_max() > 0) which = SLP_DEPTH_456;
        mulc_coop_lanes = n <= 32 ? n : (bp == 64 && which == SLP_DEPTH_456) ? n : 0;
        prog = &slp_program(which);
        const size_t need = (size_t)prog->n_slots * bp * launch::SIZEOF_JACS;
        if (need > w.slp_arena_bytes) {
            if (w.slp_arena) { HIPCK(hipStreamSynchronize(st)); HIPCK(hipFree(w.slp_arena)); w.slp_arena = nullptr; w.slp_arena_bytes = 0; }
            HIPCK(hipMalloc(&w.slp_arena, need));
            w.slp_arena_bytes = need;
        }
        X = w.slp_arena;
    }
    constexpr int fmt = launch::FMT_JACS;
    constexpr size_t pt = launch::SIZEOF_JACS;
    const TableView tv = tv_pre ? *tv_pre : table_view(TAB_FK);
    if (!tv_pre) {
        const int mk1 = mark_begin(ST_FK20_SCALARS, st);
        launch::fk20_scalars(n, w.coeffs, w.scalars, d_w29_, linmap_mode ? half_ : inv128_, segs, segs == 2 ? two_segments : seg_shift_, st);
        mark_end(mk1, 1, st);
    }
    if (phase != PROOFS_ALL) {
        if (!tv_pre || !linmap_mode || segs != 1 || msm_cut <= 0 || msm_cut >= n || msm_cut % 64) throw std::logic_error("run_proofs_from_coeffs: bad MSM cut");
        if (phase == PROOFS_HEAD) {
            launch::g1_set_inf(X, (size_t)128 * bp, st, fmt);
            launch_msm(w.scalars, tv, true, X, 128, msm_cut, bp, 0, st, fmt);
            return;
        }
        launch_msm((char*)w.scalars + (size_t)msm_cut * 128 * 64 * sizeof(Fr), tv, true, (char*)X + (size_t)msm_cut * pt, 128, n - msm_cut, bp, 0, st, fmt);
    }
    if (phase == PROOFS_ALL) launch::g1_set_inf(X, (size_t)128 * bp, st, fmt);
    const int mk2 = mark_begin(ST_MSM_FIXED, st);
    if (phase == PROOFS_ALL) launch_msm(w.scalars, tv, true, X, 128, segs * n, bp, 0, st, fmt);
    mark_end(mk2, 1, st);
    if (linmap_mode) {
        const int mk3 = mark_begin(ST_G1_LINMAP, st);
        int n_launches = 0;
        for (auto& L : prog->launches)
            launch::g1_slp_launch(L.kind, w.slp_arena, bp, (const uint32_t*)prog->d_words + (size_t)L.first * 4, L.count, prog->d_naf, beta_, st, 0,
                                  mulc_coop_lanes, n);
        n_launches = (int)prog->launches.size();
        mark_end(mk3, n_launches, st);
        const int mk4 = mark_begin(ST_COMPRESS, st);
        launch::g1_compress((const char*)w.slp_arena + (size_t)128 * bp * pt, d_proofs, 128, bp, n, st, fmt);
        mark_end(mk4, 1, st);
        return;
    }
    if (n <= circ_max_) {
        if (!w.circ_table) HIPCK(hipMalloc(&w.circ_table, launch::g1_circ_table_bytes(circ_max_, circ_T_)));
        const int mk5 = mark_begin(ST_G1_IFFT, st);
        launch::g1_circ128(w.X, bp, n, segs, w.circ_table, circ_T_, d_circ_terms_, circ_per_lane_, beta_, st);
        mark_end(mk5, 2, st);
    } else throw std::logic_error("run_proofs_from_coeffs: a batch above the circulant form needs the compiled linear map");
    const int mk10 = mark_begin(ST_COMPRESS, st);
    launch::g1_compress(w.X, d_proofs, 128, bp, n, st, fmt);
    mark_end(mk10, 1, st);
}

void Engine::enqueue_compute(Work& w, int n, const uint8_t* d_blobs, uint8_t* d_cells, uint8_t* d_proofs, hipStream_t st,
                             hipEvent_t after_cells) {
    ensure_workspace(w, n);
    HIPCK(hipStreamWaitEvent(st, w.done, 0));
    HIPCK(hipMemsetAsync(w.status, 0, n * sizeof(int), st));
    const int mk11 = mark_begin(ST_BLOB_TO_COEFFS, st);
    launch::blob_to_coeffs(n, d_blobs, w.coeffs, nullptr, w.status, d_w29_, n_inv4096_, st);
    mark_end(mk11, 1, st);
    bool side = d_cells && d_proofs && n <= SIDE_CELLS_MAX && w.copy && !profiling_;
    if (side && n > FLAT_MSM_MAX_SLICES) {
        const long simds = wave_slots_ / 2, waves = msm_waves(128L * n, table_view(TAB_FK).c);
        if (waves > simds * 4 / 5 && waves <= simds) side = false;
    }
    if (side) {
        HIPCK(hipEventRecord(w.ev_coeffs, st));
        HIPCK(hipStreamWaitEvent(w.copy, w.ev_coeffs, 0));
        launch::coeffs_to_cells(n, w.coeffs, d_cells, d_w29_, w.copy);
        if (after_cells) HIPCK(hipEventRecord(after_cells, w.copy));
        HIPCK(hipEventRecord(w.ev_side, w.copy));
        run_proofs_from_coeffs(w, n, d_proofs, st);
        HIPCK(hipStreamWaitEvent(st, w.ev_side, 0));
        return;
    }
    if (d_cells) {
        const int mk12 = mark_begin(ST_COEFFS_TO_CELLS, st);
        launch::coeffs_to_cells(n, w.coeffs, d_cells, d_w29_, st);
        mark_end(mk12, 1, st);
    }
    if (after_cells) HIPCK(hipEventRecord(after_cells, st));
    if (d_proofs) run_proofs_from_coeffs(w, n, d_proofs, st);
}

int Engine::compute_cells_and_kzg_proofs_device(int n, const uint8_t* d_blobs, uint8_t* d_cells, uint8_t* d_proofs,
                                                int* h_status, hipStream_t st, bool sync) {
    if (n <= 0) return OK;
    Work* held = nullptr;
    try {
        HIPCK(hipSetDevice(dev_));
        Work& w = lease_work(1, NW - 1);
        held = &w;
        if (!st) {
            st = w.stream;
            HIPCK(hipEventRecord(w.ev_in, nullptr));
            HIPCK(hipStreamWaitEvent(st, w.ev_in, 0));
        }
        int sub = std::min(n, device_batch_max_);
        for (int b0 = 0; b0 < n;) {
            const int nb = std::min(sub, n - b0);
            try {
                enqueue_compute(w, nb, d_blobs + (size_t)b0 * BYTES_PER_BLOB, d_cells ? d_cells + (size_t)b0 * N_CELLS * BYTES_PER_CELL : nullptr,
                                d_proofs ? d_proofs + (size_t)b0 * N_CELLS * 48 : nullptr, st, nullptr);
            } catch (const HipError& e) {
                if (!e.out_of_memory() || sub <= 64) throw;
                (void)hipGetLastError();
                HIPCK(hipStreamSynchronize(st));
                ensure_workspace(w, 0, true);
                sub = std::max(64, ((sub / 2 + 63) / 64) * 64);
                continue;
            }
            if (h_status) HIPCK(hipMemcpyAsync(h_status + b0, w.status, nb * sizeof(int), hipMemcpyDeviceToHost, st));
            b0 += nb;
        }
        HIPCK(hipEventRecord(w.done, st));
        HIPCK(hipGetLastError());
        release_work(w);
        held = nullptr;
        if (sync || h_status) HIPCK(hipStreamSynchronize(st));
    } catch (const std::exception& e) {
        if (held) release_work(*held);
        set_error(e);
        return ERR_DEVICE;
    }
    return OK;
}

int Engine::blob_to_kzg_commitment_device(int n, const uint8_t* d_blobs, uint8_t* d_commitments, int* h_status,
                                          hipStream_t st, bool sync) {
    if (n <= 0) return OK;
    std::lock_guard<std::recursive_mutex> lk(mu_);
    if (n > device_batch_max_) {
        for (int b0 = 0; b0 < n; b0 += device_batch_max_) {
            const int nb = std::min(device_batch_max_, n - b0);
            const int rc = blob_to_kzg_commitment_device(nb, d_blobs + (size_t)b0 * BYTES_PER_BLOB, d_commitments + (size_t)b0 * 48,
                                                         h_status ? h_status + b0 : nullptr, st, sync);
            if (rc) return rc;
        }
        return OK;
    }
    try {
        HIPCK(hipSetDevice(dev_));
        if (!st) {
            st = stream_;
            HIPCK(hipEventRecord(work_[0].ev_in, nullptr));
            HIPCK(hipStreamWaitEvent(st, work_[0].ev_in, 0));
        }
        ensure_workspace(n);
        HIPCK(hipStreamWaitEvent(st, work_[0].done, 0));
        const int bp = ((n + 63) / 64) * 64;
        HIPCK(hipMemsetAsync(d_status_, 0, n * sizeof(int), st));
        launch::blob_to_coeffs(n, d_blobs, d_coeffs_, d_canon_, d_status_, d_w29_, n_inv4096_, st);
        launch::g1_set_inf(d_X_, (size_t)64 * bp, st, launch::FMT_JACS);
        launch_msm(d_canon_, TAB_SRS, d_X_, 64, n, bp, 0, st, launch::FMT_JACS);
        launch::g1_sum_positions(d_X_, 64, bp, n, st);
        launch::g1_compress(d_X_, d_commitments, 1, bp, n, st, launch::FMT_JACS);
        if (h_status) HIPCK(hipMemcpyAsync(h_status, d_status_, n * sizeof(int), hipMemcpyDeviceToHost, st));
        HIPCK(hipEventRecord(work_[0].done, st));
        HIPCK(hipGetLastError());
        if (sync || h_status) HIPCK(hipStreamSynchronize(st));
    } catch (const std::exception& e) {
        set_error(e);
        return ERR_DEVICE;
    }
    return OK;
}

HostPool* Engine::ensure_host_pool() {
    std::call_once(host_pool_once_, [this] {
        int t = 8;
        const unsigned hw = std::thread::hardware_concurrency();
        if (hw && (int)hw < 2 * t) t = (int)hw / 2 > 1 ? (int)hw / 2 : 1;
        if (knobs_.host_threads) t = knobs_.host_threads;
        host_pool_.reset(new HostPool(t, [d = dev_] { (void)hipSetDevice(d); }));
    });
    return host_pool_.get();
}

int Engine::compute_cells_and_kzg_proofs_host(int n, const uint8_t* const* blobs, uint8_t* const* const* cells,
                                              uint8_t* const* const* proofs, int* h_status) {
    if (n <= 0) return OK;
    constexpr int SUPER = 4096, SUB = 256, PART = 32;
    const bool threaded = n >= 32;
    const bool trace = knobs_.trace;
    const auto t_begin = std::chrono::steady_clock::now();
    auto now_ms = [&]() { return std::chrono::duration<double, std::milli>(std::chrono::steady_clock::now() - t_begin).count(); };
    const double slow_ms = knobs_.trace ? 50.0 : 0.0;
    double step_at[8] = {0};
    int n_steps = 0;
    auto step = [&]() { if (slow_ms > 0 && n_steps < 8) step_at[n_steps++] = now_ms(); };
    struct SlowReport {
        const double& limit; double* at; int& n; std::function<double()> now;
        ~SlowReport() {
            if (limit <= 0 || now() < limit) return;
            fprintf(stderr, "[host-batch] @%.0f ms: slow call, %.1f ms; steps (lease, enqueue sub-batches, enqueue proofs, events recorded, cells back, all back):", trace_clock_ms(), now());
            for (int i = 0; i < n; i++) fprintf(stderr, " %.1f", at[i]);
            fprintf(stderr, "\n");
        }
    } slow_report{slow_ms, step_at, n_steps, now_ms};
    Work* held = nullptr;
    std::atomic<int> failed{0};
    std::mutex err_mu;
    std::string err_text;
    auto fail = [&](const std::exception& e) {
        std::lock_guard<std::mutex> lk(err_mu);
        if (!failed.exchange(1)) err_text = e.what();
    };
    std::atomic<int> outstanding{0};
    auto nap = [] { std::this_thread::sleep_for(std::chrono::microseconds(30)); };
    auto drain = [&]() { while (outstanding.load(std::memory_order_acquire) > 0) nap(); };
    try {
        HIPCK(hipSetDevice(dev_));
        if (threaded) ensure_host_pool();
        Work& w = lease_work(1, NW - 1);
        held = &w;
        step();
        for (int s0 = 0; s0 < n && !failed.load(); s0 += SUPER) {
            const int ns = std::min(SUPER, n - s0);
            std::vector<int> cut{0};
            if (ns > SUB) cut.push_back(SUB / 4);
            if (ns > SUB) cut.push_back(SUB);
            while (cut.back() < ns) cut.push_back(std::min(ns, cut.back() + SUB));
            const int n_sub = (int)cut.size() - 1;
            ensure_workspace(w, ns);
            ensure_staging(w, ns);
            while ((int)w.sub_events.size() < 3 * n_sub) {
                hipEvent_t e;
                HIPCK(hipEventCreateWithFlags(&e, hipEventDisableTiming));
                w.sub_events.push_back(e);
            }
            HIPCK(hipStreamWaitEvent(w.stream, w.done, 0));
            HIPCK(hipMemsetAsync(w.status, 0, ns * sizeof(int), w.stream));
            std::vector<std::atomic<int>> gathered(n_sub);
            std::function<void(int, int, int)> scatter_cells;
            std::function<void(int, int)> scatter_proofs;
            struct Drain {
                std::function<void()> f;
                ~Drain() { f(); }
            } drain_on_exit{drain};
            for (int i = 0; i < n_sub; i++) {
                const int lo = cut[i], hi = cut[i + 1], parts = (hi - lo + PART - 1) / PART;
                gathered[i].store(threaded ? parts : 0, std::memory_order_relaxed);
                if (!threaded) {
                    for (int b = lo; b < hi; b++) memcpy(w.h_in + (size_t)b * BYTES_PER_BLOB, blobs[s0 + b], BYTES_PER_BLOB);
                    continue;
                }
                for (int p0 = lo; p0 < hi; p0 += PART) {
                    const int p1 = std::min(hi, p0 + PART);
                    outstanding.fetch_add(1, std::memory_order_relaxed);
                    host_pool_->submit([&, i, p0, p1, s0] {
                        for (int b = p0; b < p1; b++) memcpy(w.h_in + (size_t)b * BYTES_PER_BLOB, blobs[s0 + b], BYTES_PER_BLOB);
                        gathered[i].fetch_sub(1, std::memory_order_release);
                        outstanding.fetch_sub(1, std::memory_order_release);
                    });
                }
            }
            scatter_cells = [&](int i, int lo, int hi) {
                const hipError_t q = hipEventQuery(w.sub_events[2 * i + 1]);
                if (q == hipErrorNotReady) {
                    nap();
                    host_pool_->submit([&, i, lo, hi] { scatter_cells(i, lo, hi); });
                    return;
                }
                try {
                    HIPCK(q);
                    for (int b = lo; b < hi; b++) {
                        if (h_status) h_status[s0 + b] = w.h_status[b] ? ERR_SCALAR : OK;
                        if (w.h_status[b] || !cells) continue;
                        const uint8_t* src = w.h_cells + (size_t)b * N_CELLS * BYTES_PER_CELL;
                        for (int k = 0; k < N_CELLS; k++) memcpy(cells[s0 + b][k], src + (size_t)k * BYTES_PER_CELL, BYTES_PER_CELL);
                    }
                } catch (const std::exception& e) { fail(e); }
                outstanding.fetch_sub(1, std::memory_order_release);
            };
            const bool side = cells && proofs && ns <= circ_max_;
            const bool early_scalars = proofs && ns > circ_max_;
            const TableView tv_call = table_view(TAB_FK);
            constexpr int early_msm_blobs = 256;
            int msm_cut = 0;
            if (early_scalars && early_msm_blobs > 0 && ns >= 4 * early_msm_blobs)
                for (int c : cut)
                    if (!msm_cut && c >= early_msm_blobs && c % 64 == 0 && c < ns) msm_cut = c;
            for (int i = 0; i < n_sub; i++) {
                const int lo = cut[i], hi = cut[i + 1], nb = hi - lo;
                while (gathered[i].load(std::memory_order_acquire) > 0) std::this_thread::yield();
                HIPCK(hipMemcpyAsync(w.d_in + (size_t)lo * BYTES_PER_BLOB, w.h_in + (size_t)lo * BYTES_PER_BLOB, (size_t)nb * BYTES_PER_BLOB,
                                     hipMemcpyHostToDevice, w.copy));
                HIPCK(hipEventRecord(w.sub_events[2 * n_sub + i], w.copy));
                HIPCK(hipStreamWaitEvent(w.stream, w.sub_events[2 * n_sub + i], 0));
                launch::blob_to_coeffs(nb, w.d_in + (size_t)lo * BYTES_PER_BLOB, (char*)w.coeffs + (size_t)lo * N_BLOB * sizeof(Fr), nullptr,
                                       w.status + lo, d_w29_, n_inv4096_, w.stream);
                if (cells && !side)
                    launch::coeffs_to_cells(nb, (char*)w.coeffs + (size_t)lo * N_BLOB * sizeof(Fr),
                                            w.d_cells + (size_t)lo * N_CELLS * BYTES_PER_CELL, d_w29_, w.stream);
                HIPCK(hipEventRecord(w.sub_events[2 * i], w.stream));
                if (early_scalars)
                    launch::fk20_scalars(nb, (char*)w.coeffs + (size_t)lo * N_BLOB * sizeof(Fr), (char*)w.scalars + (size_t)lo * 128 * 64 * sizeof(Fr),
                                         d_w29_, half_, 1, seg_shift_, w.stream);
                if (msm_cut && hi == msm_cut) run_proofs_from_coeffs(w, ns, w.d_proofs, w.stream, &tv_call, PROOFS_HEAD, msm_cut);
                if (trace) fprintf(stderr, "[host-batch] sub-batch %d (%d blobs) enqueued at %.2f ms\n", i, nb, now_ms());
            }
            for (int i = 0; i < n_sub; i++) {
                const int lo = cut[i], hi = cut[i + 1], nb = hi - lo;
                HIPCK(hipStreamWaitEvent(w.copy, w.sub_events[2 * i], 0));
                if (side)
                    launch::coeffs_to_cells(nb, (char*)w.coeffs + (size_t)lo * N_BLOB * sizeof(Fr),
                                            w.d_cells + (size_t)lo * N_CELLS * BYTES_PER_CELL, d_w29_, w.copy);
                HIPCK(hipMemcpyAsync(w.h_status + lo, w.status + lo, (size_t)nb * sizeof(int), hipMemcpyDeviceToHost, w.copy));
                if (cells)
                    HIPCK(hipMemcpyAsync(w.h_cells + (size_t)lo * N_CELLS * BYTES_PER_CELL, w.d_cells + (size_t)lo * N_CELLS * BYTES_PER_CELL,
                                         (size_t)nb * N_CELLS * BYTES_PER_CELL, hipMemcpyDeviceToHost, w.copy));
                HIPCK(hipEventRecord(w.sub_events[2 * i + 1], w.copy));
                if (threaded) {
                    for (int p0 = lo; p0 < hi; p0 += PART) {
                        const int p1 = std::min(hi, p0 + PART);
                        outstanding.fetch_add(1, std::memory_order_relaxed);
                        host_pool_->submit([&, i, p0, p1] { scatter_cells(i, p0, p1); });
                    }
                }
            }
            step();
            if (proofs) {
                if (msm_cut) run_proofs_from_coeffs(w, ns, w.d_proofs, w.stream, &tv_call, PROOFS_TAIL, msm_cut);
                else run_proofs_from_coeffs(w, ns, w.d_proofs, w.stream, early_scalars ? &tv_call : nullptr);
                HIPCK(hipMemcpyAsync(w.h_proofs, w.d_proofs, (size_t)ns * N_CELLS * 48, hipMemcpyDeviceToHost, w.stream));
            }
            step();
            HIPCK(hipEventRecord(w.ev_done, w.stream));
            HIPCK(hipEventRecord(w.done, w.stream));
            HIPCK(hipGetLastError());
            step();
            if (!threaded) {
                HIPCK(hipEventSynchronize(w.sub_events[1]));
                for (int b = 0; b < ns; b++) {
                    if (h_status) h_status[s0 + b] = w.h_status[b] ? ERR_SCALAR : OK;
                    if (w.h_status[b] || !cells) continue;
                    const uint8_t* src = w.h_cells + (size_t)b * N_CELLS * BYTES_PER_CELL;
                    for (int k = 0; k < N_CELLS; k++) memcpy(cells[s0 + b][k], src + (size_t)k * BYTES_PER_CELL, BYTES_PER_CELL);
                }
            }
            step();
            HIPCK(hipEventSynchronize(w.ev_done));
            HIPCK(hipStreamSynchronize(w.copy));
            step();
            if (trace) fprintf(stderr, "[host-batch] proofs of %d blobs back at %.2f ms\n", ns, now_ms());
            if (proofs) {
                scatter_proofs = [&, s0](int lo, int hi) {
                    for (int b = lo; b < hi; b++) {
                        if (w.h_status[b]) continue;
                        const uint8_t* src = w.h_proofs + (size_t)b * N_CELLS * 48;
                        for (int k = 0; k < N_CELLS; k++) memcpy(proofs[s0 + b][k], src + (size_t)k * 48, 48);
                    }
                };
                if (threaded && ns >= 256) {
                    const int parts = 8;
                    for (int t = 1; t < parts; t++) {
                        outstanding.fetch_add(1, std::memory_order_relaxed);
                        host_pool_->submit([&, t] { scatter_proofs(t * ns / parts, (t + 1) * ns / parts); outstanding.fetch_sub(1, std::memory_order_release); });
                    }
                    scatter_proofs(0, ns / parts);
                } else scatter_proofs(0, ns);
            }
        }
        release_work(w);
        held = nullptr;
        if (trace) fprintf(stderr, "[host-batch] %d blobs delivered at %.2f ms\n", n, now_ms());
        if (failed.load()) throw std::runtime_error(err_text);
// ... 56 lines not shown
```

rust-eth-kzg_amd/csrc/engine_testhooks.hip:

```cpp
#include "engine_internal.hpp"
#include "curve29.hpp"

#include <array>

namespace kzg {

int Engine::test_fr_ntt4096(const uint8_t* in_be, uint8_t* out_be, int inverse_dit) {
    std::lock_guard<std::recursive_mutex> lk(mu_);
    try {
        HIPCK(hipSetDevice(dev_));
        uint8_t *di, *dout;
        HIPCK(hipMalloc(&di, BYTES_PER_BLOB));
        HIPCK(hipMalloc(&dout, BYTES_PER_BLOB));
        HIPCK(hipMemcpy(di, in_be, BYTES_PER_BLOB, hipMemcpyHostToDevice));
        launch::test_ntt4096(di, dout, d_w29_, n_inv4096_, inverse_dit, stream_);
        HIPCK(hipStreamSynchronize(stream_));
        HIPCK(hipMemcpy(out_be, dout, BYTES_PER_BLOB, hipMemcpyDeviceToHost));
        HIPCK(hipFree(di));
        HIPCK(hipFree(dout));
    } catch (const std::exception& e) {
        set_error(e);
        return ERR_DEVICE;
    }
    return OK;
}

int Engine::test_sha256_many(int n, const uint8_t* prefix, uint32_t prefix_len, const uint8_t* d_body, size_t body_stride, uint32_t body_len,
                             const uint8_t* d_tail, size_t tail_stride, uint32_t tail_len, uint8_t* d_out) {
    std::lock_guard<std::recursive_mutex> lk(mu_);
    try {
        HIPCK(hipSetDevice(dev_));
        PoolBuf d_prefix(*this, prefix_len);
        if (prefix_len) HIPCK(hipMemcpyAsync(d_prefix.p, prefix, prefix_len, hipMemcpyHostToDevice, stream_));
        launch::sha256_many(n, (const uint8_t*)d_prefix.p, prefix_len, d_body, body_stride, body_len, d_tail, tail_stride, tail_len, d_out, stream_);
        HIPCK(hipGetLastError());
        HIPCK(hipStreamSynchronize(stream_));
    } catch (const std::exception& e) {
        set_error(e);
        return ERR_DEVICE;
    }
    return OK;
}

int Engine::test_g1_fft128(const uint8_t* in, uint8_t* out, int n_lanes, int inverse) {
    std::lock_guard<std::recursive_mutex> lk(mu_);
    try {
        HIPCK(hipSetDevice(dev_));
        int stride = ((n_lanes + 63) / 64) * 64;
        size_t bytes = (size_t)n_lanes * 128 * 48;
        uint8_t *di, *dout;
        void* X;
        HIPCK(hipMalloc(&di, bytes));
        HIPCK(hipMalloc(&dout, bytes));
        size_t nx = (size_t)128 * stride;
        const size_t PS = launch::SIZEOF_JACQ;
        HIPCK(hipMalloc(&X, nx * PS));
        HIPCK(hipMemcpy(di, in, bytes, hipMemcpyHostToDevice));
        launch::g1_set_inf(X, nx, stream_, launch::FMT_JACQ);
        launch::test_load_points(di, X, n_lanes, stride, stream_);
        HIPCK(hipStreamSynchronize(stream_));
        std::vector<uint8_t> hx(nx * PS), hy(nx * PS);
        auto brp = [](int v) { int r = 0; for (int i = 0; i < 7; i++) r |= ((v >> i) & 1) << (6 - i); return r; };
        auto permute = [&]() {
            HIPCK(hipMemcpy(hx.data(), X, nx * PS, hipMemcpyDeviceToHost));
            for (int p = 0; p < 128; p++) memcpy(&hy[(size_t)brp(p) * stride * PS], &hx[(size_t)p * stride * PS], stride * PS);
            HIPCK(hipMemcpy(X, hy.data(), nx * PS, hipMemcpyHostToDevice));
        };
        if (inverse) permute();
        g1_fft128_full(X, stride, inverse, stream_);
        HIPCK(hipStreamSynchronize(stream_));
        if (!inverse) permute();
        launch::g1_compress(X, dout, 128, stride, n_lanes, stream_, launch::FMT_JACQ);
        HIPCK(hipStreamSynchronize(stream_));
        HIPCK(hipMemcpy(out, dout, bytes, hipMemcpyDeviceToHost));
        HIPCK(hipFree(di)); HIPCK(hipFree(dout)); HIPCK(hipFree(X));
    } catch (const std::exception& e) {
        set_error(e);
        return ERR_DEVICE;
    }
    return OK;
}

int Engine::test_fixed_msm(const uint8_t* scalars_be, int n_msm, uint8_t* out) {
    std::lock_guard<std::recursive_mutex> lk(mu_);
    try {
        HIPCK(hipSetDevice(dev_));
        size_t ns = (size_t)n_msm * 128 * 64;
        int stride = ((n_msm + 63) / 64) * 64;
        uint8_t *di, *dout;
        void *sc, *X;
        HIPCK(hipMalloc(&di, ns * 32));
        HIPCK(hipMalloc(&sc, ns * sizeof(Fr)));
        HIPCK(hipMalloc(&X, (size_t)128 * stride * launch::SIZEOF_JACQ));
        HIPCK(hipMalloc(&dout, (size_t)n_msm * 128 * 48));
        HIPCK(hipMemcpy(di, scalars_be, ns * 32, hipMemcpyHostToDevice));
        launch::test_scalars_be(di, sc, ns, stream_);
        launch::g1_set_inf(X, (size_t)128 * stride, stream_, launch::FMT_JACQ);
        launch_msm(sc, TAB_FK, X, 128, n_msm, stride, 0, stream_, launch::FMT_JACQ);
        launch::g1_compress(X, dout, 128, stride, n_msm, stream_, launch::FMT_JACQ);
        HIPCK(hipStreamSynchronize(stream_));
        HIPCK(hipMemcpy(out, dout, (size_t)n_msm * 128 * 48, hipMemcpyDeviceToHost));
        HIPCK(hipFree(di)); HIPCK(hipFree(sc)); HIPCK(hipFree(X)); HIPCK(hipFree(dout));
    } catch (const std::exception& e) {
        set_error(e);
        return ERR_DEVICE;
    }
    return OK;
}

int Engine::test_g1_decompress(const uint8_t* in, int n, int subgroup_check, int* h_status, uint8_t* out) {
    std::lock_guard<std::recursive_mutex> lk(mu_);
    try {
        HIPCK(hipSetDevice(dev_));
        uint8_t *di, *dout;
        void* pts;
        int* st;
        HIPCK(hipMalloc(&di, (size_t)n * 48)); HIPCK(hipMalloc(&dout, (size_t)n * 48));
        HIPCK(hipMalloc(&pts, (size_t)n * sizeof(G1Affine))); HIPCK(hipMalloc(&st, n * sizeof(int)));
        HIPCK(hipMemcpy(di, in, (size_t)n * 48, hipMemcpyHostToDevice));
        launch::g1_decompress(di, pts, st, n, subgroup_check, beta_, stream_);
        launch::test_recompress(pts, dout, n, stream_);
        HIPCK(hipStreamSynchronize(stream_));
        HIPCK(hipMemcpy(h_status, st, n * sizeof(int), hipMemcpyDeviceToHost));
        HIPCK(hipMemcpy(out, dout, (size_t)n * 48, hipMemcpyDeviceToHost));
        HIPCK(hipFree(di)); HIPCK(hipFree(dout)); HIPCK(hipFree(pts)); HIPCK(hipFree(st));
    } catch (const std::exception& e) {
        set_error(e);
        return ERR_DEVICE;
    }
    return OK;
}

int Engine::test_field_mul(const uint8_t* a, const uint8_t* b, uint8_t* out, int n, int is_fp) {
    std::lock_guard<std::recursive_mutex> lk(mu_);
    try {
        HIPCK(hipSetDevice(dev_));
        size_t nb = (size_t)n * (is_fp ? 48 : 32);
        uint8_t *da, *db, *dout;
        HIPCK(hipMalloc(&da, nb)); HIPCK(hipMalloc(&db, nb)); HIPCK(hipMalloc(&dout, nb));
        HIPCK(hipMemcpy(da, a, nb, hipMemcpyHostToDevice));
        HIPCK(hipMemcpy(db, b, nb, hipMemcpyHostToDevice));
        launch::test_field_mul(da, db, dout, n, is_fp, stream_);
        HIPCK(hipStreamSynchronize(stream_));
        HIPCK(hipMemcpy(out, dout, nb, hipMemcpyDeviceToHost));
        HIPCK(hipFree(da)); HIPCK(hipFree(db)); HIPCK(hipFree(dout));
    } catch (const std::exception& e) {
        set_error(e);
        return ERR_DEVICE;
    }
    return OK;
}

int Engine::test_op(int op, int n, const int32_t* in, int32_t* out) {
    int in_w, out_w, dev_only;
    const char* name;
    if (launch::test_op_info(op, &in_w, &out_w, &dev_only, &name) != 0 || n <= 0) return ERR_INPUT;
    std::lock_guard<std::recursive_mutex> lk(mu_);
    try {
        HIPCK(hipSetDevice(dev_));
        const size_t ni = (size_t)n * in_w * sizeof(int32_t), no = (size_t)n * out_w * sizeof(int32_t);
        int32_t *di, *dout;
        HIPCK(hipMalloc(&di, ni)); HIPCK(hipMalloc(&dout, no));
        HIPCK(hipMemcpy(di, in, ni, hipMemcpyHostToDevice));
        HIPCK(hipMemset(dout, 0, no));
        launch::test_op_device(op, n, di, dout, stream_);
        HIPCK(hipGetLastError());
        HIPCK(hipStreamSynchronize(stream_));
        HIPCK(hipMemcpy(out, dout, no, hipMemcpyDeviceToHost));
        HIPCK(hipFree(di)); HIPCK(hipFree(dout));
    } catch (const std::exception& e) {
        set_error(e);
        return ERR_DEVICE;
    }
    return OK;
}

int Engine::test_verify_msm(int form, const uint8_t* points, int n_pts, const uint8_t* sc0_be, int n0, const uint8_t* sc1_be, int n1,
                            uint8_t* out96, int32_t* h_status) {
    if (form < 0 || form > 2 || n0 < 1 || n1 < n0 || n_pts < n1 || n_pts > (1 << 20)) return ERR_INPUT;
    std::vector<Fr> sc((size_t)n0 + n1);
    for (int j = 0; j < n0 + n1; j++) {
        const uint8_t* b = j < n0 ? sc0_be + (size_t)j * 32 : sc1_be + (size_t)(j - n0) * 32;
        Fr& x = sc[j];
        for (int i = 0; i < 8; i++)
            x.v[7 - i] = ((uint32_t)b[4 * i] << 24) | ((uint32_t)b[4 * i + 1] << 16) | ((uint32_t)b[4 * i + 2] << 8) | b[4 * i + 3];
        if (geq_mod<FrParams>(x.v)) return ERR_SCALAR;
    }
    std::lock_guard<std::recursive_mutex> lk(mu_);
    struct DevBuf {
        void* p = nullptr;
        ~DevBuf() { if (p) (void)hipFree(p); }
    } d_in, d_pts, d_st, d_sc, d_ws, d_out;
    try {
        HIPCK(hipSetDevice(dev_));
        const bool shifted = form != 0;
        HIPCK(hipMalloc(&d_in.p, (size_t)n_pts * 48));
        HIPCK(hipMalloc(&d_pts.p, (size_t)n_pts * sizeof(G1Affine)));
        HIPCK(hipMalloc(&d_st.p, (size_t)n_pts * sizeof(int)));
        HIPCK(hipMalloc(&d_sc.p, sc.size() * sizeof(Fr)));
        HIPCK(hipMalloc(&d_ws.p, shifted ? launch::pip_shift_workspace_bytes(n_pts) : launch::pip_workspace_bytes(n_pts)));
        HIPCK(hipMalloc(&d_out.p, 512));
        hipStream_t st = stream_;
        HIPCK(hipMemcpyAsync(d_in.p, points, (size_t)n_pts * 48, hipMemcpyHostToDevice, st));
        HIPCK(hipMemcpyAsync(d_sc.p, sc.data(), sc.size() * sizeof(Fr), hipMemcpyHostToDevice, st));
        HIPCK(hipMemsetAsync(d_st.p, 0xff, (size_t)n_pts * sizeof(int), st));
        HIPCK(hipMemsetAsync(d_out.p, 0xff, 512, st));
        const uint8_t* in0 = (const uint8_t*)d_in.p;
        G1Affine* p0 = (G1Affine*)d_pts.p;
        int* st0 = (int*)d_st.p;
        const int rest = n_pts - n0;
        const Fr *s0 = (const Fr*)d_sc.p, *s1 = s0 + n0;
        G1Affine out[2];
        if (form == 2) {
            launch::g1_decode2(in0, p0, st0, n0, in0 + (size_t)n0 * 48, p0 + n0, st0 + n0, rest, beta_, st);
            launch::pip_shift_prepare_and_subgroup(p0, n_pts, n_pts, d_ws.p, p0, st0, n0, p0 + n0, st0 + n0, rest, beta_, st);
        } else {
            launch::g1_decompress2(in0, p0, st0, n0, in0 + (size_t)n0 * 48, p0 + n0, st0 + n0, rest, beta_, st);
            if (form == 1) launch::pip_shift_prepare(p0, n_pts, n_pts, d_ws.p, beta_, st);
        }
        std::vector<int32_t> status(n_pts);
        HIPCK(hipMemcpyAsync(status.data(), d_st.p, (size_t)n_pts * sizeof(int), hipMemcpyDeviceToHost, st));
        if (shifted) {
            launch::msm_pippenger2_shifted(s0, n0, s1, n1, n_pts, d_ws.p, d_out.p, st);
            JacQ sums[2];
            static_assert(sizeof(sums) <= 512 && sizeof(JacQ) == launch::SIZEOF_JACQ, "result slot");
            HIPCK(hipMemcpyAsync(sums, d_out.p, sizeof sums, hipMemcpyDeviceToHost, st));
            HIPCK(hipGetLastError());
            HIPCK(hipStreamSynchronize(st));
            for (int i = 0; i < 2; i++) {
                if (sums[i].x.v[0] == 0xffffffffu && sums[i].z.v[0] == 0xffffffffu) throw std::runtime_error("verification MSM left no result");
                out[i] = to_affine(jac_from_jacq(sums[i]));
            }
        } else {
            launch::msm_pippenger2(p0, s0, n0, s1, n1, d_ws.p, d_out.p, beta_, st);
            HIPCK(hipMemcpyAsync(out, d_out.p, 2 * sizeof(G1Affine), hipMemcpyDeviceToHost, st));
            HIPCK(hipGetLastError());
            HIPCK(hipStreamSynchronize(st));
        }
        for (int i = 0; i < 2; i++)
            if (out[i].x.v[11] > FpParams::MOD[11] || out[i].y.v[11] > FpParams::MOD[11]) throw std::runtime_error("verification MSM left no result");
        if (h_status) memcpy(h_status, status.data(), (size_t)n_pts * sizeof(int32_t));
        for (int i = 0; i < 2; i++) g1_compress(out96 + 48 * i, out[i]);
    } catch (const std::exception& e) {
        set_error(e);
        return ERR_DEVICE;
    }
    return OK;
}

int Engine::test_verify_cells_partial_device(uint64_t n, const uint8_t* d_commitments, const uint64_t* d_cell_indices, const uint8_t* d_cells,
                                             const uint8_t* d_proofs, uint64_t lo, uint64_t hi, uint8_t* out96) {
    if (n < 1 || n > MAX_CELLS_PER_VERIFICATION || lo > hi || hi > n) return ERR_INPUT;
    std::lock_guard<std::recursive_mutex> lk(mu_);
    G1Affine pts[2];
    bool empty = false;
    const int rc = verify_cells_partial_device(n, d_commitments, d_cell_indices, d_cells, d_proofs, lo, hi, pts, &empty, nullptr);
    if (rc) return rc;
    g1_compress(out96, pts[0]);
    g1_compress(out96 + 48, pts[1]);
    return OK;
}
int Engine::test_verify_blob_batch_inputs(uint64_t n, int on_device, const void* blobs, const void* commitments, const void* proofs,
                                          uint8_t* out96, int* verified) {
    if (n < 1 || n > (1u << 24)) return ERR_INPUT;
    G1Affine sums[2] = {aff_inf(), aff_inf()};
    const int rc = on_device ? verify_blob_kzg_proof_batch_device(n, (const uint8_t*)blobs, (const uint8_t*)commitments, (const uint8_t*)proofs, verified,
                                                                  nullptr, sums)
                             : verify_blob_kzg_proof_batch_host(n, (const uint8_t* const*)blobs, n, (const uint8_t* const*)commitments, n,
                                                                (const uint8_t* const*)proofs, verified, sums);
    if (rc) return rc;
    g1_compress(out96, sums[0]);
    g1_compress(out96 + 48, sums[1]);
    return OK;
}

static void fr_mont_to_be(uint8_t* out, const uint32_t* mont) {
    Fr x;
    for (int i = 0; i < 8; i++) x.v[i] = mont[i];
    x = from_mont(x);
    for (int i = 0; i < 8; i++) {
        const uint32_t w = x.v[7 - i];
        out[4 * i] = (uint8_t)(w >> 24); out[4 * i + 1] = (uint8_t)(w >> 16); out[4 * i + 2] = (uint8_t)(w >> 8); out[4 * i + 3] = (uint8_t)w;
    }
}
int Engine::test_rs_decode(int R, const uint64_t* n_cells, const uint64_t* const* cell_indices, const uint8_t* const* const* cells, int flat_source,
                           int32_t* status, int32_t* deg, uint8_t* zp, uint8_t* zeval, uint8_t* zcinv, uint8_t* coeffs) {
    std::lock_guard<std::recursive_mutex> lk(mu_);
    try {
        HIPCK(hipSetDevice(dev_));
        ensure_workspace(R);
        std::vector<uint32_t> present((size_t)R * 4, 0);
        std::vector<int> slot, stof, st_out(R, OK);
        size_t total_cells = 0;
        for (int r = 0; r < R; r++) total_cells += n_cells[r];
        const size_t src_bytes = (flat_source ? (size_t)R * N_CELLS : total_cells) * BYTES_PER_CELL;
        PoolBuf h_src(*this, src_bytes, true), d_src(*this, src_bytes);
        uint8_t* h = (uint8_t*)h_src.p;
        size_t pos = 0;
        for (int r = 0; r < R; r++) {
            if (flat_source) memcpy(h + (size_t)r * N_CELLS * BYTES_PER_CELL, cells[r][0], (size_t)N_CELLS * BYTES_PER_CELL);
            for (uint64_t k = 0; k < n_cells[r]; k++) {
                const int c = (int)cell_indices[r][k], i = brp7(c);
                present[(size_t)r * 4 + (i >> 5)] |= 1u << (i & 31);
                if (!flat_source) memcpy(h + pos * BYTES_PER_CELL, cells[r][k], BYTES_PER_CELL);
                slot.push_back(r * N_CELLS + c);
                stof.push_back(r);
                pos++;
            }
        }
        HIPCK(hipMemcpyAsync(d_src.p, h, src_bytes, hipMemcpyHostToDevice, stream_));
        std::vector<int> h_deg(R);
        std::vector<Fr8> h_zp((size_t)R * 65), h_zeval((size_t)R * N_CELLS), h_zcinv((size_t)R * N_CELLS);
        RsDecodeTap tap;
        tap.deg = h_deg.data(); tap.zp = h_zp.data(); tap.zeval = h_zeval.data(); tap.zcinv = h_zcinv.data();
        const int rc = rs_decode(R, (const uint8_t*)d_src.p, flat_source != 0, slot, stof, present, st_out.data(), &tap);
        if (rc) return rc;
        for (int r = 0; r < R; r++) {
            if (status) status[r] = st_out[r];
            if (deg) deg[r] = h_deg[r];
        }
        for (size_t i = 0; i < h_zp.size() && zp; i++) fr_mont_to_be(zp + 32 * i, h_zp[i].v);
        for (size_t i = 0; i < h_zeval.size() && zeval; i++) fr_mont_to_be(zeval + 32 * i, h_zeval[i].v);
        for (size_t i = 0; i < h_zcinv.size() && zcinv; i++) fr_mont_to_be(zcinv + 32 * i, h_zcinv[i].v);
        if (coeffs) {
            std::vector<Fr8> h_c((size_t)R * N_BLOB);
            HIPCK(hipMemcpy(h_c.data(), d_coeffs_, h_c.size() * sizeof(Fr8), hipMemcpyDeviceToHost));
            for (size_t i = 0; i < h_c.size(); i++) fr_mont_to_be(coeffs + 32 * i, h_c[i].v);
        }
    } catch (const std::exception& e) {
        set_error(e);
        return ERR_DEVICE;
    }
    return OK;
}

std::shared_ptr<Engine::SharedTable> Engine::test_table(int kind, int which) const {
    if (primary_) return primary_->test_table(kind, which);
    if (kind != TAB_FK && kind != TAB_SRS) return nullptr;
    if (which == 2) return start_tab_[kind].lock();
    const TableView v = table_view((TableSel)kind);
    return which == 0 ? v.main : which == 1 ? v.next : nullptr;
}

int Engine::test_table_info(int kind, int which, int64_t* out8, int32_t* piece_first_block, int max_pieces) {
    const auto t = test_table(kind, which);
    if (!t) return ERR_INPUT;
    const int ready = t->state.load() == 1 ? t->n_groups : t->ready_groups.load(std::memory_order_acquire);
    const int n_pieces = (int)t->piece_count.load(std::memory_order_acquire);
    out8[0] = t->c; out8[1] = t->n_groups; out8[2] = t->nb; out8[3] = t->state.load(); out8[4] = ready;
    out8[5] = (int64_t)t->bytes; out8[6] = t->build_chunk; out8[7] = n_pieces;
    for (int k = 0; k < n_pieces && k < max_pieces && piece_first_block; k++) piece_first_block[k] = t->piece_first_block[k];
    return OK;
}

static const void* table_bases(const void* fk, const void* srs, int kind) { return kind == 0 ? fk : srs; }

int Engine::test_table_audit(int kind, int which, uint64_t* visited, uint64_t* n_findings, int32_t* findings, int max_findings, double* ms) {
    const auto t = test_table(kind, which);
    if (!t || max_findings < 0) return ERR_INPUT;
    std::lock_guard<std::recursive_mutex> lk(mu_);
    try {
        HIPCK(hipSetDevice(dev_));
        const int groups = t->state.load() == 1 ? t->n_groups : t->ready_groups.load(std::memory_order_acquire);
        const int FW = launch::TABLE_FINDING_WORDS;
        char* d_out;
        int32_t* d_find;
        HIPCK(hipMalloc(&d_out, launch::SIZEOF_AUDIT_OUT));
        HIPCK(hipMalloc(&d_find, (size_t)std::max(1, max_findings) * FW * sizeof(int32_t)));
        struct { unsigned long long visited; unsigned int n, max; int32_t* f; } h = {0, 0, (unsigned)max_findings, d_find};
        static_assert(sizeof(h) == launch::SIZEOF_AUDIT_OUT, "audit::Out");
        HIPCK(hipMemcpy(d_out, &h, sizeof(h), hipMemcpyHostToDevice));
        hipEvent_t e0, e1;
        HIPCK(hipEventCreate(&e0)); HIPCK(hipEventCreate(&e1));
        HIPCK(hipEventRecord(e0, stream_));
        if (groups > 0) launch::table_audit_device(t->d_blocks, table_bases(d_fk_bases_, d_srs_, kind), t->c, groups, t->nb, d_out, stream_);
        HIPCK(hipGetLastError());
        HIPCK(hipEventRecord(e1, stream_));
        HIPCK(hipStreamSynchronize(stream_));
        float dt = 0;
        HIPCK(hipEventElapsedTime(&dt, e0, e1));
        HIPCK(hipEventDestroy(e0)); HIPCK(hipEventDestroy(e1));
        HIPCK(hipMemcpy(&h, d_out, sizeof(h), hipMemcpyDeviceToHost));
        const int kept = (int)std::min<unsigned>(h.n, (unsigned)max_findings);
        std::vector<std::array<int32_t, 5>> f(kept);
        if (kept) HIPCK(hipMemcpy(f.data(), d_find, (size_t)kept * FW * sizeof(int32_t), hipMemcpyDeviceToHost));
        std::sort(f.begin(), f.end());
        if (kept) memcpy(findings, f.data(), (size_t)kept * FW * sizeof(int32_t));
        *visited = h.visited;
        *n_findings = h.n;
        if (ms) *ms = dt;
        HIPCK(hipFree(d_out)); HIPCK(hipFree(d_find));
    } catch (const std::exception& e) {
        set_error(e);
        return ERR_DEVICE;
    }
    return OK;
}

int Engine::test_table_read(int kind, int which, int group, int window, int base, int d0, int n, uint32_t* out) {
    const auto t = test_table(kind, which);
    if (!t) return ERR_INPUT;
    const int c = t->c, W = launch::glv_windows(c), WL = launch::glv_lower_windows(c);
    const int ready = t->state.load() == 1 ? t->n_groups : t->ready_groups.load(std::memory_order_acquire);
    if (group < 0 || group >= ready || window < 0 || window >= W || base < 0 || base >= t->nb || d0 < 1 || n < 1) return ERR_INPUT;
    const long T = 1l << (launch::glv_window_bits(c, window) - 1);
    if ((long)d0 - 1 + n > T) return ERR_INPUT;
// ... 61 lines not shown
```

rust-eth-kzg_amd/csrc/fr29_ntt.hpp:

```cpp
#pragma once
#include "fr29.hpp"

namespace kzg {

constexpr int NTT_N = 4096, NTT_W = 8192;

HD Fr29 fr29_twiddled(const Fr29& b, const Fr29* __restrict__ w29, int e) {
    return e ? fr29_mul(b, w29[e]) : fr29_partial_reduce(b);
}
template <class Elems>
HD void ntt4096_dit_inverse_unit(const Elems& m, const Fr29* __restrict__ w29, int h, int u) {
    const int j = u & (h - 1), i0 = ((u - j) << 2) + j;
    const int step_a = NTT_W / (2 * h), step_b = step_a >> 1;
    const int ea = (NTT_W - j * step_a) & (NTT_W - 1), eb0 = (NTT_W - j * step_b) & (NTT_W - 1), eb1 = NTT_W - (j + h) * step_b;
    const Fr29 x0 = m.load(i0), x1 = m.load(i0 + h), x2 = m.load(i0 + 2 * h), x3 = m.load(i0 + 3 * h);
    const Fr29 ta = fr29_twiddled(x1, w29, ea), tc = fr29_twiddled(x3, w29, ea);
    const Fr29 a0 = fr29_add<false>(x0, ta), a1 = fr29_sub2r<false>(x0, ta), a2 = fr29_add<false>(x2, tc), a3 = fr29_sub2r<false>(x2, tc);
    const Fr29 tb0 = fr29_twiddled(a2, w29, eb0), tb1 = fr29_mul(a3, w29[eb1]);
    m.store(i0, fr29_add<true>(a0, tb0));
    m.store(i0 + 2 * h, fr29_sub2r<true>(a0, tb0));
    m.store(i0 + h, fr29_add<true>(a1, tb1));
    m.store(i0 + 3 * h, fr29_sub2r<true>(a1, tb1));
}
template <class Elems>
HD void ntt4096_ct_forward_unit(const Elems& m, const Fr29* __restrict__ w29, int h, int log_m, int u) {
    const int j = u & (h - 1), blk = u / h, i0 = ((u - j) << 2) + j;
    unsigned rb = 0;
    for (int b = 0; b < log_m; b++) rb |= (((unsigned)blk >> b) & 1u) << (log_m - 1 - b);
    const int ea = (int)rb * (2 * h) * (NTT_W / NTT_N);
    const int eb0 = (int)rb * h * (NTT_W / NTT_N), eb1 = (int)(rb + (1u << log_m)) * h * (NTT_W / NTT_N);
    const Fr29 x0 = m.load(i0), x1 = m.load(i0 + h), x2 = m.load(i0 + 2 * h), x3 = m.load(i0 + 3 * h);
    const Fr29 ta = fr29_twiddled(x2, w29, ea), tc = fr29_twiddled(x3, w29, ea);
    const Fr29 a0 = fr29_add<false>(x0, ta), a2 = fr29_sub2r<false>(x0, ta), a1 = fr29_add<false>(x1, tc), a3 = fr29_sub2r<false>(x1, tc);
    const Fr29 tb0 = fr29_twiddled(a1, w29, eb0), tb1 = fr29_mul(a3, w29[eb1]);
    m.store(i0, fr29_add<true>(a0, tb0));
    m.store(i0 + h, fr29_sub2r<true>(a0, tb0));
    m.store(i0 + 2 * h, fr29_add<true>(a2, tb1));
    m.store(i0 + 3 * h, fr29_sub2r<true>(a2, tb1));
}

}
```

rust-eth-kzg_amd/csrc/k_ntt.hip:

```cpp
#include "engine.hpp"
#include "kcommon.hpp"
#include "fr29.hpp"
#include "fr29_ntt.hpp"
#include "glv.hpp"
#include "launch.hpp"

namespace kzg {

__device__ __forceinline__ Fr29 lds_load(const uint32_t* s, int idx) {
    Fr29 r;
#pragma unroll
    for (int l = 0; l < RL; l++) r.v[l] = s[l * N_BLOB + idx];
    return r;
}
__device__ __forceinline__ void lds_store(uint32_t* s, int idx, const Fr29& a) {
#pragma unroll
    for (int l = 0; l < RL; l++) s[l * N_BLOB + idx] = a.v[l];
}

struct LdsElems {
    uint32_t* s;
    __device__ __forceinline__ Fr29 load(int i) const { return lds_load(s, i); }
    __device__ __forceinline__ void store(int i, const Fr29& v) const { lds_store(s, i, v); }
};
__device__ __forceinline__ void dit_inverse_pass(uint32_t* s, const Fr29* __restrict__ w29, int h) {
    ntt4096_dit_inverse_unit(LdsElems{s}, w29, h, (int)threadIdx.x);
}
__device__ __forceinline__ void ntt4096_dit_inverse(uint32_t* s, const Fr29* __restrict__ w29) {
    dit_inverse_pass(s, w29, 1);
    __builtin_amdgcn_wave_barrier();
    dit_inverse_pass(s, w29, 4);
    __builtin_amdgcn_wave_barrier();
    dit_inverse_pass(s, w29, 16);
    __builtin_amdgcn_wave_barrier();
    dit_inverse_pass(s, w29, 64);
    __syncthreads();
    dit_inverse_pass(s, w29, 256);
    __syncthreads();
    dit_inverse_pass(s, w29, 1024);
    __builtin_amdgcn_wave_barrier();
}
__device__ __forceinline__ void ct_forward_pass(uint32_t* s, const Fr29* __restrict__ w29, int h, int log_m) {
    ntt4096_ct_forward_unit(LdsElems{s}, w29, h, log_m, (int)threadIdx.x);
}
__device__ __forceinline__ void ntt4096_ct_forward(uint32_t* s, const Fr29* __restrict__ w29) {
    __builtin_amdgcn_wave_barrier();
    ct_forward_pass(s, w29, 1024, 0);
    __syncthreads();
    ct_forward_pass(s, w29, 256, 2);
    __syncthreads();
    ct_forward_pass(s, w29, 64, 4);
    __builtin_amdgcn_wave_barrier();
    ct_forward_pass(s, w29, 16, 6);
    __builtin_amdgcn_wave_barrier();
    ct_forward_pass(s, w29, 4, 8);
    __builtin_amdgcn_wave_barrier();
    ct_forward_pass(s, w29, 1, 10);
    __syncthreads();
}
__device__ __forceinline__ Fr fr_words_of(const Fr29& canonical) {
    Fr r;
    fr29_to_words(r.v, canonical);
    return r;
}

struct NttConsts {
    Fr29 ninv_to_sat;
    Fr29 ninv_plain;
    Fr29 one;
};
__global__ __launch_bounds__(1024) void k_blob_to_coeffs(const uint8_t* __restrict__ blobs, Fr* __restrict__ coeffs,
                                                        Fr* __restrict__ canon_out, int* __restrict__ status,
                                                        const Fr29* __restrict__ w29, NttConsts K) {
    extern __shared__ uint32_t s[];
    const int b = blockIdx.x, tid = threadIdx.x;
    const uint8_t* blob = blobs + (size_t)b * BYTES_PER_BLOB;
    bool bad = false;
    for (int e = tid; e < N_BLOB; e += 1024) {
        const Fr x = load_fr_be(blob + 32 * e);
        bad |= geq_mod<FrParams>(x.v);
        lds_store(s, e, fr29_from_plain(x));
    }
    if (bad) atomicOr(&status[b], 1);
    __syncthreads();
    ntt4096_dit_inverse(s, w29);
    for (int e = tid; e < N_BLOB; e += 1024) {
        const Fr29 x = lds_load(s, e);
        coeffs[(size_t)b * N_BLOB + e] = fr_words_of(fr29_reduce_once(fr29_mul(x, K.ninv_to_sat)));
        if (canon_out) canon_out[(size_t)b * N_BLOB + e] = fr_words_of(fr29_reduce_once(fr29_mul(x, K.ninv_plain)));
    }
}

__global__ __launch_bounds__(1024) void k_coeffs_to_cells(const Fr* __restrict__ coeffs, uint8_t* __restrict__ cells,
                                                         const Fr29* __restrict__ w29) {
    extern __shared__ uint32_t s[];
    const int b = blockIdx.x, h = blockIdx.y, tid = threadIdx.x;
    for (int e = tid; e < N_BLOB; e += 1024) {
        Fr29 c = fr29_from_fr_mont(coeffs[(size_t)b * N_BLOB + e]);
        if (h && e) c = fr29_mul(c, w29[e]);
        lds_store(s, e, c);
    }
    __syncthreads();
    ntt4096_ct_forward(s, w29);
    uint8_t* out = cells + ((size_t)b * N_EXT + (size_t)h * N_BLOB) * 32;
    const Fr29 one_plain = fr29_const(r29::ONE_PLAIN);
    for (int e = tid; e < N_BLOB; e += 1024)
        store_fr_be(out + 32 * e, fr_words_of(fr29_reduce_once(fr29_mul(lds_load(s, e), one_plain))));
}

struct SegShifts { Fr29 p[3]; };
__global__ __launch_bounds__(256) void k_fk20_scalars(const Fr* __restrict__ coeffs, Fr* __restrict__ scalars,
                                                      const Fr29* __restrict__ w29, Fr29 scale , int n,
                                                      int segs, SegShifts sh) {
    __shared__ uint32_t s[4][RL][128];
    const int b = blockIdx.x >> 4, wv = threadIdx.x >> 6, lane = threadIdx.x & 63;
    const int i = ((blockIdx.x & 15) << 2) + wv;
    const Fr* a = coeffs + (size_t)b * N_BLOB;
    uint32_t(*sv)[128] = s[wv];
    {
        Fr29 lo, hi;
#pragma unroll
        for (int l = 0; l < RL; l++) lo.v[l] = hi.v[l] = 0;
        if (lane == 0) lo = fr29_mul(fr29_from_plain(a[N_BLOB - 1 - i]), scale);
        else hi = fr29_mul(fr29_from_plain(a[64 * lane - 1 - i]), scale);
#pragma unroll
        for (int l = 0; l < RL; l++) { sv[l][lane] = lo.v[l]; sv[l][64 + lane] = hi.v[l]; }
    }
    __builtin_amdgcn_wave_barrier();
    int log_m = 0;
    for (int half = 64; half >= 1; half >>= 1, log_m++) {
        const int j = lane & (half - 1), blk = lane / half;
        const int i0 = ((lane - j) << 1) + j, i1 = i0 + half;
        const int e = log_m ? (int)(__brev((unsigned)blk) >> (32 - log_m)) * half * (N_EXT / 128) : 0;
        Fr29 x, y;
#pragma unroll
        for (int l = 0; l < RL; l++) { x.v[l] = sv[l][i0]; y.v[l] = sv[l][i1]; }
        const Fr29 t = e ? fr29_mul(y, w29[e]) : fr29_partial_reduce(y);
        Fr29 sum = fr29_add<false>(x, t), d = fr29_sub2r<false>(x, t);
        if ((log_m & 1) || half == 1) { fr29_normalise(sum); fr29_normalise(d); }
#pragma unroll
        for (int l = 0; l < RL; l++) { sv[l][i0] = sum.v[l]; sv[l][i1] = d.v[l]; }
        __builtin_amdgcn_wave_barrier();
    }
    auto emit = [&](size_t at, const Fr29& x) {
        Fr k = fr_words_of(fr29_reduce_once(fr29_partial_reduce(x)));
        uint32_t h[8];
        glv_split_balanced(k, h);
#pragma unroll
        for (int l = 0; l < 8; l++) k.v[l] = h[l];
        scalars[at] = k;
    };
    for (int q = lane; q < 128; q += 64) {
        Fr29 x;
#pragma unroll
        for (int l = 0; l < RL; l++) x.v[l] = sv[l][q];
        const int j = __brev((unsigned)q) >> 25;
        emit(((size_t)b * 128 + j) * 64 + i, x);
        for (int sg = 1; sg < segs; sg++)
            emit(((size_t)(sg * n + b) * 128 + j) * 64 + i, fr29_mul(x, sh.p[sg - 1]));
    }
}

#ifdef KZG_TEST_HOOKS
__global__ __launch_bounds__(1024) void k_test_ntt4096(const uint8_t* in, uint8_t* out, const Fr29* w29, NttConsts K, int inverse_dit) {
    extern __shared__ uint32_t s[];
    for (int e = threadIdx.x; e < N_BLOB; e += 1024) lds_store(s, e, fr29_from_plain(load_fr_be(in + 32 * e)));
    __syncthreads();
    if (inverse_dit) ntt4096_dit_inverse(s, w29);
    else ntt4096_ct_forward(s, w29);
    for (int e = threadIdx.x; e < N_BLOB; e += 1024) {
        const Fr29 c = lds_load(s, e);
        store_fr_be(out + 32 * e, fr_words_of(fr29_reduce_once(fr29_mul(c, inverse_dit ? K.ninv_plain : K.one))));
    }
}
__global__ void k_test_scalars_be(const uint8_t* in, Fr* out, size_t n) {
    size_t i = (size_t)blockIdx.x * blockDim.x + threadIdx.x;
    if (i < n) out[i] = load_fr_be(in + 32 * i);
}
template <class F>
__global__ void k_test_field_mul(const uint8_t* a, const uint8_t* b, uint8_t* out, int n) {
    int i = blockIdx.x * blockDim.x + threadIdx.x;
    if (i >= n) return;
    constexpr int NB = F::N * 4;
    F x, y;
    for (int k = 0; k < F::N; k++) {
        const uint8_t* pa = a + (size_t)i * NB + 4 * k;
        const uint8_t* pb = b + (size_t)i * NB + 4 * k;
        x.v[F::N - 1 - k] = ((uint32_t)pa[0] << 24) | ((uint32_t)pa[1] << 16) | ((uint32_t)pa[2] << 8) | pa[3];
        y.v[F::N - 1 - k] = ((uint32_t)pb[0] << 24) | ((uint32_t)pb[1] << 16) | ((uint32_t)pb[2] << 8) | pb[3];
    }
    F z = from_mont(mul(to_mont(x), to_mont(y)));
    for (int k = 0; k < F::N; k++) {
        uint32_t w = z.v[F::N - 1 - k];
        uint8_t* po = out + (size_t)i * NB + 4 * k;
        po[0] = (uint8_t)(w >> 24); po[1] = (uint8_t)(w >> 16); po[2] = (uint8_t)(w >> 8); po[3] = (uint8_t)w;
    }
}

#endif

namespace launch {
void preload_k_ntt() {
    hipFuncAttributes a;
    (void)hipFuncGetAttributes(&a, reinterpret_cast<const void*>(&k_blob_to_coeffs));
}
static Fr as_fr(const Fr8& x) { Fr r; for (int i = 0; i < 8; i++) r.v[i] = x.v[i]; return r; }

constexpr size_t LDS_NTT29 = (size_t)N_BLOB * RL * 4;
void init_attributes() {
    hipFuncSetAttribute(reinterpret_cast<const void*>(k_blob_to_coeffs), hipFuncAttributeMaxDynamicSharedMemorySize, (int)LDS_NTT29);
    hipFuncSetAttribute(reinterpret_cast<const void*>(k_coeffs_to_cells), hipFuncAttributeMaxDynamicSharedMemorySize, (int)LDS_NTT29);
#ifdef KZG_TEST_HOOKS
    hipFuncSetAttribute(reinterpret_cast<const void*>(k_test_ntt4096), hipFuncAttributeMaxDynamicSharedMemorySize, (int)LDS_NTT29);
#endif
}
static Fr29 fr29_mont_of(const Fr& y_mont) {
    Fr c32 = zero<FrParams>();
    c32.v[0] = 32;
    return fr29_from_plain(mul(y_mont, to_mont(c32)));
}
static Fr29 fr29_mont_of(const Fr8& y_mont) { return fr29_mont_of(as_fr(y_mont)); }
static Fr29 fr29_int32x_of(const Fr8& s_mont) {
    Fr c32 = zero<FrParams>();
    c32.v[0] = 32;
    return fr29_from_plain(from_mont(mul(as_fr(s_mont), to_mont(c32))));
}
static NttConsts ntt_consts(const Fr8& n_inv_mont) {
    NttConsts K;
    K.ninv_to_sat = fr29_mont_of(to_mont(as_fr(n_inv_mont)));
    K.ninv_plain = fr29_mont_of(n_inv_mont);
    K.one = fr29_mont_of(one<FrParams>());
    return K;
}
void ntt_twiddles29(const void* w8192_mont_host , void* out_host ) {
    const Fr* w = (const Fr*)w8192_mont_host;
    Fr29* o = (Fr29*)out_host;
    for (int k = 0; k < N_EXT; k++) o[k] = fr29_mont_of(*(const Fr8*)&w[k]);
}
void blob_to_coeffs(int n, const uint8_t* blobs, void* coeffs, void* canon, int* status, const void* w29, const Fr8& n_inv, hipStream_t st) {
    k_blob_to_coeffs<<<n, 1024, LDS_NTT29, st>>>(blobs, (Fr*)coeffs, (Fr*)canon, status, (const Fr29*)w29, ntt_consts(n_inv));
}
void coeffs_to_cells(int n, const void* coeffs, uint8_t* cells, const void* w29, hipStream_t st) {
    k_coeffs_to_cells<<<dim3(n, 2), 1024, LDS_NTT29, st>>>((const Fr*)coeffs, cells, (const Fr29*)w29);
}
void fk20_scalars(int n, const void* coeffs, void* scalars, const void* w29, const Fr8& inv128, int segs, const Fr8* seg_shifts,
                  hipStream_t st) {
    SegShifts sh;
    for (int i = 0; i < 3; i++) sh.p[i] = fr29_mont_of(seg_shifts[i]);
    k_fk20_scalars<<<n * 16, 256, 0, st>>>((const Fr*)coeffs, (Fr*)scalars, (const Fr29*)w29, fr29_int32x_of(inv128), n, segs, sh);
}
#ifdef KZG_TEST_HOOKS
void test_ntt4096(const uint8_t* in, uint8_t* out, const void* w29, const Fr8& n_inv, int inverse_dit, hipStream_t st) {
    k_test_ntt4096<<<1, 1024, LDS_NTT29, st>>>(in, out, (const Fr29*)w29, ntt_consts(n_inv), inverse_dit);
}
void test_scalars_be(const uint8_t* in, void* out, size_t n, hipStream_t st) {
    k_test_scalars_be<<<(unsigned)((n + 255) / 256), 256, 0, st>>>(in, (Fr*)out, n);
}
void test_field_mul(const uint8_t* a, const uint8_t* b, uint8_t* out, int n, int is_fp, hipStream_t st) {
    if (is_fp) k_test_field_mul<Fp><<<(n + 63) / 64, 64, 0, st>>>(a, b, out, n);
    else k_test_field_mul<Fr><<<(n + 63) / 64, 64, 0, st>>>(a, b, out, n);
}
#endif
}
}
```

rust-eth-kzg_amd/csrc/knobs.hpp:

```cpp
#pragma once
#include <cstdlib>
#include <cstring>
#include <string>
#include <vector>

namespace kzg {

struct Knobs {
    int device = 0;
    std::vector<int> devices;
    double table_budget_gb = 0;
    int glv_window = 0;
    bool progressive = true;
    int host_threads = 0;
    int serial_lanes = 0;
    bool trace = false;
    int msm_chunks = -1, slp_program = -1, pip_shift_min = 0;
    bool vm_search = true, vm_fold = true, verify_combine = true, msm_split = true;
    std::string fault;
    int device_batch_max = 0;

    static Knobs from_env() {
        Knobs k;
        auto num = [](const char* name, int lo, int hi, int& out) {
            if (const char* s = getenv(name)) { const int v = atoi(s); if (v >= lo && v <= hi) out = v; }
        };
        auto flag = [](const char* name, bool& out) {
            if (const char* s = getenv(name)) out = atoi(s) != 0;
        };
        num("ETH_KZG_AMD_DEVICE", 0, 4095, k.device);
        if (const char* s = getenv("ETH_KZG_AMD_DEVICES")) {
            if (!strcmp(s, "all") || !strcmp(s, "ALL")) k.devices.push_back(-1);
            else
                for (const char* p = s; *p;) {
                    char* end = nullptr;
                    const long v = strtol(p, &end, 10);
                    if (end == p) break;
                    if (v >= 0 && v <= 4095 && k.devices.size() < 64) k.devices.push_back((int)v);
                    p = *end == ',' ? end + 1 : end;
                    if (*end && *end != ',') break;
                }
        }
        if (const char* s = getenv("ETH_KZG_AMD_TABLE_GB")) {
            if (!strcmp(s, "max") || !strcmp(s, "MAX")) k.table_budget_gb = -1;
            else if (atof(s) > 0) k.table_budget_gb = atof(s);
        }
        num("ETH_KZG_AMD_GLV_WINDOW", 8, 16, k.glv_window);
        flag("ETH_KZG_AMD_PROGRESSIVE", k.progressive);
        num("ETH_KZG_AMD_HOST_THREADS", 1, 64, k.host_threads);
        num("ETH_KZG_AMD_SERIAL_LANES", 1, 16, k.serial_lanes);
        k.trace = getenv("ETH_KZG_AMD_TRACE") != nullptr;
        num("ETH_KZG_AMD_MSM_CHUNKS", 0, 4, k.msm_chunks);
        num("ETH_KZG_AMD_SLP_PROGRAM", 0, 15, k.slp_program);
        num("ETH_KZG_AMD_PIP_SHIFT_MIN", 1, 1 << 24, k.pip_shift_min);
        flag("ETH_KZG_AMD_VM_SEARCH", k.vm_search);
        flag("ETH_KZG_AMD_VM_FOLD", k.vm_fold);
        flag("ETH_KZG_AMD_VERIFY_COMBINE", k.verify_combine);
        flag("ETH_KZG_AMD_MSM_SPLIT", k.msm_split);
        if (const char* s = getenv("ETH_KZG_AMD_FAULT")) k.fault = s;
        num("ETH_KZG_AMD_DEVICE_BATCH_MAX", 64, 1 << 20, k.device_batch_max);
        return k;
    }
};

}
```

rust-eth-kzg_amd/csrc/launch.hpp:

```cpp
#pragma once
#include <hip/hip_runtime.h>
#include <cstddef>
#include <cstdint>

namespace kzg {
struct Fr8;
struct Fp12w;
namespace launch {

void init_attributes();
void preload_code_objects();

constexpr size_t SIZEOF_FR29 = 36;
void ntt_twiddles29(const void* w8192_mont_host , void* out_host );
void blob_to_coeffs(int n, const uint8_t* blobs, void* coeffs , void* canon , int* status,
                    const void* w29, const Fr8& n_inv, hipStream_t st);
void coeffs_to_cells(int n, const void* coeffs, uint8_t* cells, const void* w29, hipStream_t st);
void fk20_scalars(int n, const void* coeffs, void* scalars, const void* w29, const Fr8& inv128, int segs, const Fr8* seg_shifts,
                  hipStream_t st);
void test_ntt4096(const uint8_t* in, uint8_t* out, const void* w29, const Fr8& n_inv, int inverse_dit, hipStream_t st);
void test_scalars_be(const uint8_t* in, void* out, size_t n, hipStream_t st);
void test_field_mul(const uint8_t* a, const uint8_t* b, uint8_t* out, int n, int is_fp, hipStream_t st);
int test_op_info(int op, int* in_words, int* out_words, int* device_only, const char** name);
int test_op_host(int op, int n, const int32_t* in, int32_t* out);
int test_op_device(int op, int n, const int32_t* d_in, int32_t* d_out, hipStream_t st);
constexpr int TABLE_FINDING_WORDS = 5;
constexpr size_t SIZEOF_AUDIT_OUT = 24;
void table_audit_device(const void* const* blocks, const void* bases, int c, int n_groups, int nb, void* out, hipStream_t st);
void table_audit_host(const void* const* blocks, const void* bases, int c, int n_groups, int nb, unsigned long long* visited,
                      unsigned long long* n_findings, int32_t* findings, int max_findings);

struct TabBlocks {
    const void* const* blocks;
    int g0, gcnt;
};
constexpr int glv_windows(int c) { return (128 + c - 1) / c; }
constexpr int glv_lower_windows(int c) { return (glv_windows(c) + 1) / 2; }
constexpr int glv_base_bits(int c) { return 128 / glv_windows(c); }
constexpr int glv_wide_windows(int c) { return 128 - glv_windows(c) * glv_base_bits(c); }
constexpr int glv_window_bits(int c, int w) { return glv_base_bits(c) + (w < glv_wide_windows(c) ? 1 : 0); }
constexpr int glv_window_lo(int c, int w) { return w * glv_base_bits(c) + (w < glv_wide_windows(c) ? w : glv_wide_windows(c)); }
constexpr size_t glv_entries_per_base(int c, int w0, int w1) {
    size_t n = 0;
    for (int w = w0; w < w1; w++) n += (size_t)1 << (glv_window_bits(c, w) - 1);
    return n;
}
constexpr int GLV_WIDTHS[] = {16, 15, 14, 12, 8};
bool glv_width_supported(int c);
void glv_split(void* scalars, size_t n, hipStream_t st);
constexpr int FMT_JACQ = 0, FMT_JACS = 1;
void msm_glv(int c, int mode, const void* scalars, const TabBlocks& table, void* out , int n_groups, int n_slices, int nb, int out_stride,
             int brp_bits, const Fp12w& beta, hipStream_t st, int out_fmt);
#ifdef TABS_STRIDE_128
constexpr size_t SIZEOF_TABP = 128;
#else
constexpr size_t SIZEOF_TABP = 96;
#endif
size_t table_glv_entries(int c, int n_groups, int nb);
size_t table_glv_side_bytes(int c, int n_groups, int nb);
bool build_table_glv(int c, const void* bases, void* const* blocks, void* scratch, void* side, int n_groups, int nb, int* err, hipStream_t st);

void g1_fft_layer(void* X, int stride, int half, int tw_step, int inverse, int mode, const void* tw, const Fp12w& beta,
                  hipStream_t st);

void g1_slp_launch(int kind, void* arena, int stride, const uint32_t* words, int count, const void* naf, const Fp12w& beta,
                   hipStream_t st, int lanes = 0 ,
                   int coop_lanes = 0 ,
                   int n_active = 0 );

void g1_set_inf(void* X, size_t n, hipStream_t st, int fmt);
int coop_points_max();
void spin(uint64_t wall_clock_ticks, hipStream_t st);
void g1_compress(const void* X, uint8_t* out, int n_pos, int stride, int n_slices, hipStream_t st, int fmt);
void g1_sum_positions(void* X , int n_pos, int stride, int n_slices, hipStream_t st);
void g1_decompress(const uint8_t* in, void* out , int* status, int n, int subgroup_check, const Fp12w& beta,
                   hipStream_t st);
void g1_decompress2(const uint8_t* in0, void* out0, int* status0, int n0, const uint8_t* in1, void* out1, int* status1, int n1,
                    const Fp12w& beta, hipStream_t st);
void g1_decode2(const uint8_t* in0, void* out0, int* status0, int n0, const uint8_t* in1, void* out1, int* status1, int n1,
                const Fp12w& beta, hipStream_t st);
void g1_subgroup2(const void* pts0, int* status0, int n0, const void* pts1, int* status1, int n1, const Fp12w& beta, hipStream_t st);
void fk20_srs_vectors(const void* srs, void* X, hipStream_t st);
void fk20_gather_bases(const void* X, void* bases, hipStream_t st);
void test_load_points(const uint8_t* in, void* X, int n_lanes, int stride, hipStream_t st);
void test_recompress(const void* pts, uint8_t* out, int n, hipStream_t st);

constexpr int TWIDDLE_WNAF_W = 5;
constexpr int TWIDDLE_WORDS = 33;
constexpr int CIRC_LANES = 256;
size_t g1_circ_table_bytes(int n, int T);
void g1_circ128(void* X , int stride, int n, int segs, void* D, int T, const void* terms, int per_lane, const Fp12w& beta, hipStream_t st);
void init_attributes_verify();
void cells_to_fr(const uint8_t* cells, void* evals, const int* slot_of, int* status, const int* status_of, const int* src_of, int n,
                 hipStream_t st);
void rec_vanishing_poly(const uint32_t* present, const void* w8192, void* zp, int* deg, int R, hipStream_t st);
void rec_vanishing(const void* zp, const int* deg, const void* w8192, const Fr8& seven64, void* zeval, void* zcinv, int R,
                   hipStream_t st);
void verify_scalars(const Fr8* pow_table24, int k0, const int* cell_idx, const void* w8192, void* rp_mont, void* s1, void* s2,
                    int n, hipStream_t st);
void verify_weights(const void* rp_mont, const int* row, void* weights, int n, int m, hipStream_t st);
void interp(const void* evals, const int* cell_idx, const void* rp_mont, const void* w8192, const Fr8& inv64, void* partial,
            int nblocks, void* out_neg_canon, int n, hipStream_t st);
void interp_cells(const void* evals, const int* cell_idx, const void* w8192, const Fr8& inv64, void* coef, int n, hipStream_t st);
void interp_sum(const void* coef, const void* rp_mont, void* partial, int nblocks, void* out_neg_canon, int n, hipStream_t st);
size_t pip_shift_workspace_bytes(int n_max);
void pip_shift_prepare(const void* points, int n_pts, int n_max, void* workspace, const Fp12w& beta, hipStream_t st);
void pip_shift_prepare_and_subgroup(const void* points, int n_pts, int n_max, void* workspace, const void* pts0, int* status0, int n0,
                                    const void* pts1, int* status1, int n1, const Fp12w& beta, hipStream_t st);
void msm_pippenger2_shifted(const void* sc0, int n0, const void* sc1, int n1, int n_max, void* workspace, void* out_jacq2,
                            hipStream_t st);
size_t pip_workspace_bytes(int n_max);
void copy_affine(const void* src, void* dst, int n, hipStream_t st);
void msm_pippenger2(const void* points, const void* sc0, int n0, const void* sc1, int n1, void* workspace, void* out_affine2,
                    const Fp12w& beta, hipStream_t st);
void rec_dit_half(int R, const void* V, const void* fac, void* T, const void* w8192, hipStream_t st);
void rec_dit_last(int R, const void* T, const void* shift, const Fr8& n_inv, void* U, void* coeffs, int* status,
                  const void* w8192, int final_pass, hipStream_t st);
void rec_dif_half(int R, const void* U, const void* fac, void* V, const void* w8192, hipStream_t st);

void vm_scalars(const void* pow_tables , const int* batch_of, const int* pos_in_batch, const int* cell_idx, const void* w8192,
                void* rp_mont, void* s1, void* s2, int n, hipStream_t st);
void vm_weights(const void* rp_mont, const int* row, const int* row_batch, const int* cell_start, void* weights, int m, hipStream_t st);
void vm_interp_sum(const void* coef, const void* rp_mont, const int* cell_start, void* out_neg_canon, int n_batches, hipStream_t st);
void vm_mul(const void* pts, const void* s1, const void* s2, const void* wts, void* prod, int n, int m, const Fp12w& beta, hipStream_t st);
void vm_mul_small(const void* pts, const void* s1, const void* s2, const void* wts, const void* isc, const void* srs, void* prod, int n, int m,
                  int n_batches, int* status, const Fp12w& beta, hipStream_t st);
void vm_reduce_small(const void* prod, const int* cell_start, const int* row_start, void* out, int n, int m, int n_batches, hipStream_t st);
void vm_reduce(const void* prod, const void* icommit, const int* cell_start, const int* row_start, void* out , int n,
               int n_batches, hipStream_t st);
void vm_fold(const void* sums, const uint32_t* rho, void* prod, void* out2, int n_batches, const Fp12w& beta, hipStream_t st);
void vm_fold_ranges(const void* prod, const int* ranges , void* out , int n_ranges, hipStream_t st);

void quotient_by_linear(int n, const void* coeffs, const void* z_mont, void* quotient, void* y_out, hipStream_t st);
void fr_from_be32(int n, const uint8_t* in, void* out_mont, int* bad, bool reduce, hipStream_t st);
void fr_to_be32(int n, const void* canon , uint8_t* out, hipStream_t st);
void status_4844(int n, const int* blob_bad, const int* z_bad, const int* g1_bad, int* out, hipStream_t st);

void sha256_many(int n, const uint8_t* prefix, uint32_t prefix_len, const uint8_t* body, size_t body_stride, uint32_t body_len,
                 const uint8_t* tail, size_t tail_stride, uint32_t tail_len, uint8_t* out, hipStream_t st);

constexpr size_t SIZEOF_FR = 32, SIZEOF_G1AFFINE = 96, SIZEOF_G1JAC = 144;
constexpr size_t SIZEOF_JACS = 156;
constexpr size_t SIZEOF_AFFQ = 112, SIZEOF_JACQ = 168;

}
}
```

Measured before the change: 40740.

## Fuse coeffs-to-cells NTT with FK20 scalar generation in one kernel

Adds a kernel that runs the first passes of the 4096-point coset NTT in LDS, reads the intermediate state to emit the FK20 GLV-split scalars using precomputed tap constants, then finishes the NTT to write cells. For h==0 it copies the original blob bytes into the cells instead of finishing the NTT. This replaces the separate fk20_scalars kernel and its extra read of the coefficients, and is enabled by default when the side-stream path is off and segs==1. It adds a table of precomputed tap constants and more work per block, and the fused kernel serializes cells and scalars rather than overlapping them on side streams.

```diff
diff --git a/include/c_eth_kzg_test_hooks.h b/include/c_eth_kzg_test_hooks.h
--- a/include/c_eth_kzg_test_hooks.h
+++ b/include/c_eth_kzg_test_hooks.h
@@ -12,6 +12,9 @@
                                    uint8_t *out);
 int eth_kzg_amd_test_field_mul(const DASContext *ctx, const uint8_t *a, const uint8_t *b, uint8_t *out, int n,
                                int is_fp);
+
+int eth_kzg_amd_test_prover_scalars(const DASContext *ctx, int n, const uint8_t *blobs, uint32_t *scalars, uint64_t max_words,
+                                    uint64_t *n_words, uint8_t *cells, uint8_t *proofs, int32_t *status, int32_t *fused_launches);
 
 int eth_kzg_amd_test_sha256_many(const DASContext *ctx, uint64_t n, const uint8_t *prefix, uint64_t prefix_len, const uint8_t *d_body,
                                  uint64_t body_stride, uint64_t body_len, const uint8_t *d_tail, uint64_t tail_stride, uint64_t tail_len,
diff --git a/rust-eth-kzg_amd/__init__.py b/rust-eth-kzg_amd/__init__.py
--- a/rust-eth-kzg_amd/__init__.py
+++ b/rust-eth-kzg_amd/__init__.py
@@ -61,6 +61,7 @@
     "eth_kzg_amd_test_table_info", "eth_kzg_amd_test_table_audit", "eth_kzg_amd_test_table_read", "eth_kzg_amd_test_table_audit_buffer",
     "eth_kzg_amd_test_sha256_many", "eth_kzg_amd_test_verify_msm",
     "eth_kzg_amd_test_verify_cells_partial_device", "eth_kzg_amd_test_verify_blob_batch_inputs", "eth_kzg_amd_test_rs_decode",
+    "eth_kzg_amd_test_prover_scalars",
 ]
 
 _lib = None
@@ -172,6 +173,7 @@
         "eth_kzg_amd_test_verify_cells_partial_device": [P, U64, P, P, P, P, U64, U64, P],
         "eth_kzg_amd_test_verify_blob_batch_inputs": [P, U64, C.c_int, P, P, P, P, P],
         "eth_kzg_amd_test_rs_decode": [P, C.c_int, P, P, P, C.c_int, P, P, P, P, P, P],
+        "eth_kzg_amd_test_prover_scalars": [P, C.c_int, P, P, U64, P, P, P, P, P],
     }.items():
         if hasattr(lib, name):
             getattr(lib, name).argtypes = args
diff --git a/rust-eth-kzg_amd/csrc/c_api_hooks.cpp b/rust-eth-kzg_amd/csrc/c_api_hooks.cpp
--- a/rust-eth-kzg_amd/csrc/c_api_hooks.cpp
+++ b/rust-eth-kzg_amd/csrc/c_api_hooks.cpp
@@ -29,6 +29,11 @@
 }
 int eth_kzg_amd_test_fixed_msm(const DASContext* ctx, const uint8_t* scalars, int n_msm, uint8_t* out) {
     return eng(ctx)->test_fixed_msm(scalars, n_msm, out);
+}
+int eth_kzg_amd_test_prover_scalars(const DASContext* ctx, int n, const uint8_t* blobs, uint32_t* scalars, uint64_t max_words, uint64_t* n_words,
+                                    uint8_t* cells, uint8_t* proofs, int32_t* status, int32_t* fused_launches) {
+    if (!blobs || !scalars || !n_words || !cells || !proofs || !status || !fused_launches) return kzg::ERR_INPUT;
+    return eng(ctx)->test_prover_scalars(n, blobs, scalars, max_words, n_words, cells, proofs, status, fused_launches);
 }
 int eth_kzg_amd_test_g1_decompress(const DASContext* ctx, const uint8_t* in, int n, int subgroup_check, int32_t* status,
                                    uint8_t* out) {
diff --git a/rust-eth-kzg_amd/csrc/engine.hip b/rust-eth-kzg_amd/csrc/engine.hip
--- a/rust-eth-kzg_amd/csrc/engine.hip
+++ b/rust-eth-kzg_amd/csrc/engine.hip
@@ -191,6 +191,7 @@
     }
     vm_search_ = knobs_.vm_search;
     msm_split_ = knobs_.msm_split;
+    fused_scalars_ = knobs_.fused_scalars;
     if (knobs_.pip_shift_min >= 1) pip_shift_min_ = knobs_.pip_shift_min;
 #ifdef KZG_CIRC_MAX
     circ_max_ = KZG_CIRC_MAX;
@@ -315,7 +316,7 @@
     host_pool_.reset();
     vm_pool_.reset();
     stage_pool_.reset();
-    void* ptrs[] = {d_w8192_, d_w29_, d_naf_, d_srs_, d_fk_bases_, d_in_, d_cells_, d_proofs_, d_coset_, d_coset_inv_, d_circ_terms_, d_4844_};
+    void* ptrs[] = {d_w8192_, d_w29_, d_tapk_, d_naf_, d_srs_, d_fk_bases_, d_in_, d_cells_, d_proofs_, d_coset_, d_coset_inv_, d_circ_terms_, d_4844_};
     for (void* p : ptrs)
         if (p) hipFree(p);
     for (SlpProgram& P : slp_prog_) {
@@ -423,6 +424,10 @@
     Fr i4096 = inv(fr_from_u64(N_BLOB)), i128 = inv(fr_from_u64(128));
     memcpy(&n_inv4096_, &i4096, 32);
     memcpy(&inv128_, &i128, 32);
+    HIPCK(hipMalloc(&d_tapk_, (size_t)2 * N_EXT * launch::SIZEOF_FR29));
+    launch::fk20_tap_consts(d_w29_, half_, d_tapk_, stream_);
+    launch::fk20_tap_consts(d_w29_, inv128_, (char*)d_tapk_ + (size_t)N_EXT * launch::SIZEOF_FR29, stream_);
+    HIPCK(hipGetLastError());
 }
 
 static linmap::Strategy slp_strategy(int id) {
diff --git a/rust-eth-kzg_amd/csrc/engine.hpp b/rust-eth-kzg_amd/csrc/engine.hpp
--- a/rust-eth-kzg_amd/csrc/engine.hpp
+++ b/rust-eth-kzg_amd/csrc/engine.hpp
@@ -156,6 +156,8 @@
     int test_fr_ntt4096(const uint8_t* in_be, uint8_t* out_be, int inverse_dit);
     int test_g1_fft128(const uint8_t* in_compressed, uint8_t* out_compressed, int n_lanes, int inverse);
     int test_fixed_msm(const uint8_t* scalars_be, int n_msm, uint8_t* out_compressed);
+    int test_prover_scalars(int n, const uint8_t* blobs, uint32_t* scalars, uint64_t max_words, uint64_t* n_words, uint8_t* cells, uint8_t* proofs,
+                            int32_t* status, int32_t* fused_launches);
     int test_g1_decompress(const uint8_t* in, int n, int subgroup_check, int* h_status, uint8_t* out_recompressed);
     int test_field_mul(const uint8_t* a, const uint8_t* b, uint8_t* out, int n, int is_fp);
     int test_op(int op, int n, const int32_t* in, int32_t* out);
@@ -263,6 +265,7 @@
                                 int msm_cut = 0);
     void enqueue_compute(Work& w, int n, const uint8_t* d_blobs, uint8_t* d_cells, uint8_t* d_proofs, hipStream_t st,
                          hipEvent_t after_cells);
+    int fk20_segs(int n) const;
     Work& lease_work(int first, int last);
     void release_work(Work& w);
     std::mutex lease_mu_;
@@ -307,6 +310,8 @@
     int wave_slots_ = 2048;
     int device_batch_max_ = 4096;
     int msm_chunks_ = -1;
+    int fused_scalars_ = -1;
+    std::atomic<uint64_t> fused_launches_{0};
     bool msm_split_ = true;
     hipStream_t stream_ = nullptr;
     std::recursive_mutex mu_;
@@ -322,6 +327,7 @@
     void* d_srs_ = nullptr;
     void* d_fk_bases_ = nullptr;
     BufferPool dev_pool_{false}, pin_pool_{true};
+    void* d_tapk_ = nullptr;
     Fr8 n_inv4096_, inv128_;
 
     void* d_coset_ = nullptr;
diff --git a/rust-eth-kzg_amd/csrc/engine_prover.hip b/rust-eth-kzg_amd/csrc/engine_prover.hip
--- a/rust-eth-kzg_amd/csrc/engine_prover.hip
+++ b/rust-eth-kzg_amd/csrc/engine_prover.hip
@@ -148,9 +148,10 @@
     }
 }
 
+int Engine::fk20_segs(int n) const { return (n > circ_max_ || circ_T_ > 129) ? 1 : n <= 2 ? 4 : n <= 4 ? 2 : 1; }
 void Engine::run_proofs_from_coeffs(Work& w, int n, uint8_t* d_proofs, hipStream_t st, const TableView* tv_pre, ProofsPhase phase, int msm_cut) {
     const int bp = ((n + 63) / 64) * 64;
-    const int segs = (n > circ_max_ || circ_T_ > 129) ? 1 : n <= 2 ? 4 : n <= 4 ? 2 : 1;
+    const int segs = fk20_segs(n);
     const Fr8 two_segments[3] = {seg_shift_[1], seg_shift_[1], seg_shift_[1]};
     const bool linmap_mode = n > circ_max_;
     void* X = w.X;
@@ -226,6 +227,22 @@
     if (side && n > FLAT_MSM_MAX_SLICES) {
         const long simds = wave_slots_ / 2, waves = msm_waves(128L * n, table_view(TAB_FK).c);
         if (waves > simds * 4 / 5 && waves <= simds) side = false;
+    }
+    const int segs = fk20_segs(n);
+    const bool fused = d_cells && d_proofs && fused_scalars_ != 0 && (fused_scalars_ == 1 || (!side && segs == 1));
+    if (fused) {
+        const bool linmap_mode = n > circ_max_;
+        const Fr8 two_segments[3] = {seg_shift_[1], seg_shift_[1], seg_shift_[1]};
+        const TableView tv = table_view(TAB_FK);
+        const int mk = mark_begin(ST_COEFFS_TO_CELLS, st);
+        launch::coeffs_to_cells_scalars(n, w.coeffs, d_cells, w.scalars, d_blobs, w.status, d_w29_,
+                                        (const char*)d_tapk_ + (linmap_mode ? 0 : (size_t)N_EXT * launch::SIZEOF_FR29), segs,
+                                        segs == 2 ? two_segments : seg_shift_, st);
+        mark_end(mk, 1, st);
+        fused_launches_.fetch_add(1, std::memory_order_relaxed);
+        if (after_cells) HIPCK(hipEventRecord(after_cells, st));
+        run_proofs_from_coeffs(w, n, d_proofs, st, &tv);
+        return;
     }
     if (side) {
         HIPCK(hipEventRecord(w.ev_coeffs, st));
diff --git a/rust-eth-kzg_amd/csrc/engine_testhooks.hip b/rust-eth-kzg_amd/csrc/engine_testhooks.hip
--- a/rust-eth-kzg_amd/csrc/engine_testhooks.hip
+++ b/rust-eth-kzg_amd/csrc/engine_testhooks.hip
@@ -102,6 +102,45 @@
         HIPCK(hipMemcpy(out, dout, (size_t)n_msm * 128 * 48, hipMemcpyDeviceToHost));
         HIPCK(hipFree(di)); HIPCK(hipFree(sc)); HIPCK(hipFree(X)); HIPCK(hipFree(dout));
     } catch (const std::exception& e) {
+        set_error(e);
+        return ERR_DEVICE;
+    }
+    return OK;
+}
+
+int Engine::test_prover_scalars(int n, const uint8_t* blobs, uint32_t* scalars, uint64_t max_words, uint64_t* n_words, uint8_t* cells,
+                                uint8_t* proofs, int32_t* status, int32_t* fused_launches) {
+    if (n < 1 || n > 4096) return ERR_INPUT;
+    const uint64_t words = (uint64_t)fk20_segs(n) * n * N_EXT * 8;
+    if (words > max_words) return ERR_INPUT;
+    struct DevBuf {
+        void* p = nullptr;
+        ~DevBuf() { if (p) (void)hipFree(p); }
+    } d_in, d_cells, d_proofs;
+    Work* held = nullptr;
+    try {
+        HIPCK(hipSetDevice(dev_));
+        Work& w = lease_work(1, NW - 1);
+        held = &w;
+        HIPCK(hipMalloc(&d_in.p, (size_t)n * BYTES_PER_BLOB));
+        HIPCK(hipMalloc(&d_cells.p, (size_t)n * N_CELLS * BYTES_PER_CELL));
+        HIPCK(hipMalloc(&d_proofs.p, (size_t)n * N_CELLS * 48));
+        HIPCK(hipMemcpyAsync(d_in.p, blobs, (size_t)n * BYTES_PER_BLOB, hipMemcpyHostToDevice, w.stream));
+        const uint64_t before = fused_launches_.load();
+        enqueue_compute(w, n, (const uint8_t*)d_in.p, (uint8_t*)d_cells.p, (uint8_t*)d_proofs.p, w.stream, nullptr);
+        HIPCK(hipEventRecord(w.done, w.stream));
+        HIPCK(hipGetLastError());
+        HIPCK(hipStreamSynchronize(w.stream));
+        *fused_launches = (int32_t)(fused_launches_.load() - before);
+        *n_words = words;
+        HIPCK(hipMemcpy(scalars, w.scalars, words * 4, hipMemcpyDeviceToHost));
+        HIPCK(hipMemcpy(cells, d_cells.p, (size_t)n * N_CELLS * BYTES_PER_CELL, hipMemcpyDeviceToHost));
+        HIPCK(hipMemcpy(proofs, d_proofs.p, (size_t)n * N_CELLS * 48, hipMemcpyDeviceToHost));
+        HIPCK(hipMemcpy(status, w.status, (size_t)n * sizeof(int), hipMemcpyDeviceToHost));
+        release_work(w);
+        held = nullptr;
+    } catch (const std::exception& e) {
+        if (held) { (void)hipStreamSynchronize(held->stream); (void)hipStreamSynchronize(held->copy); release_work(*held); }
         set_error(e);
         return ERR_DEVICE;
     }
diff --git a/rust-eth-kzg_amd/csrc/fr29_ntt.hpp b/rust-eth-kzg_amd/csrc/fr29_ntt.hpp
--- a/rust-eth-kzg_amd/csrc/fr29_ntt.hpp
+++ b/rust-eth-kzg_amd/csrc/fr29_ntt.hpp
@@ -39,4 +39,20 @@
     m.store(i0 + 3 * h, fr29_sub2r<true>(a2, tb1));
 }
 
+HD int fk20_tap_row(int e, int h) {
+    const int q = e >> 6;
+    int rb = 0;
+    for (int b = 0; b < 6; b++) rb |= ((q >> b) & 1) << (5 - b);
+    return 2 * rb + h;
 }
+HD int fk20_tap_column(int e) { return 63 - (e & 63); }
+HD int fk20_tap_exponent(int e, int h) { return (64 * 65 * fk20_tap_row(e, h) + NTT_W - (e & 63) * h) & (NTT_W - 1); }
+HD Fr29 fk20_tap_const(const Fr29* __restrict__ w29, const Fr29& scale_plain, int idx) {
+    return fr29_reduce_once(fr29_mul(w29[fk20_tap_exponent(idx & (NTT_N - 1), idx >> 12)], scale_plain));
+}
+template <class Elems>
+HD Fr29 fk20_tap_scalar(const Elems& m, const Fr29* __restrict__ tapk, int e, int h) {
+    return fr29_mul(m.load(e), tapk[h * NTT_N + e]);
+}
+
+}
diff --git a/rust-eth-kzg_amd/csrc/k_ntt.hip b/rust-eth-kzg_amd/csrc/k_ntt.hip
--- a/rust-eth-kzg_amd/csrc/k_ntt.hip
+++ b/rust-eth-kzg_amd/csrc/k_ntt.hip
@@ -43,25 +43,39 @@
 __device__ __forceinline__ void ct_forward_pass(uint32_t* s, const Fr29* __restrict__ w29, int h, int log_m) {
     ntt4096_ct_forward_unit(LdsElems{s}, w29, h, log_m, (int)threadIdx.x);
 }
+__device__ __forceinline__ void ntt4096_ct_forward_head(uint32_t* s, const Fr29* __restrict__ w29) {
+    __builtin_amdgcn_wave_barrier();
+    ct_forward_pass(s, w29, 1024, 0);
+    __syncthreads();
+    ct_forward_pass(s, w29, 256, 2);
+    __syncthreads();
+    ct_forward_pass(s, w29, 64, 4);
+}
+__device__ __forceinline__ void ntt4096_ct_forward_tail(uint32_t* s, const Fr29* __restrict__ w29) {
+    __builtin_amdgcn_wave_barrier();
+    ct_forward_pass(s, w29, 16, 6);
+    __builtin_amdgcn_wave_barrier();
+    ct_forward_pass(s, w29, 4, 8);
+    __builtin_amdgcn_wave_barrier();
+    ct_forward_pass(s, w29, 1, 10);
+    __syncthreads();
+}
 __device__ __forceinline__ void ntt4096_ct_forward(uint32_t* s, const Fr29* __restrict__ w29) {
-    __builtin_amdgcn_wave_barrier();
-    ct_forward_pass(s, w29, 1024, 0);
-    __syncthreads();
-    ct_forward_pass(s, w29, 256, 2);
-    __syncthreads();
-    ct_forward_pass(s, w29, 64, 4);
-    __builtin_amdgcn_wave_barrier();
-    ct_forward_pass(s, w29, 16, 6);
-    __builtin_amdgcn_wave_barrier();
-    ct_forward_pass(s, w29, 4, 8);
-    __builtin_amdgcn_wave_barrier();
-    ct_forward_pass(s, w29, 1, 10);
-    __syncthreads();
+    ntt4096_ct_forward_head(s, w29);
+    ntt4096_ct_forward_tail(s, w29);
 }
 __device__ __forceinline__ Fr fr_words_of(const Fr29& canonical) {
     Fr r;
     fr29_to_words(r.v, canonical);
     return r;
+}
+__device__ __forceinline__ void store_split_scalar(Fr* __restrict__ at, const Fr29& x) {
+    Fr k = fr_words_of(fr29_reduce_once(x));
+    uint32_t h[8];
+    glv_split_balanced(k, h);
+#pragma unroll
+    for (int l = 0; l < 8; l++) k.v[l] = h[l];
+    *at = k;
 }
 
 struct NttConsts {
@@ -143,12 +157,7 @@
         __builtin_amdgcn_wave_barrier();
     }
     auto emit = [&](size_t at, const Fr29& x) {
-        Fr k = fr_words_of(fr29_reduce_once(fr29_partial_reduce(x)));
-        uint32_t h[8];
-        glv_split_balanced(k, h);
-#pragma unroll
-        for (int l = 0; l < 8; l++) k.v[l] = h[l];
-        scalars[at] = k;
+        store_split_scalar(&scalars[at], fr29_partial_reduce(x));
     };
     for (int q = lane; q < 128; q += 64) {
         Fr29 x;
@@ -159,6 +168,46 @@
         for (int sg = 1; sg < segs; sg++)
             emit(((size_t)(sg * n + b) * 128 + j) * 64 + i, fr29_mul(x, sh.p[sg - 1]));
     }
+}
+
+__global__ __launch_bounds__(1024) void k_coeffs_to_cells_scalars(const Fr* __restrict__ coeffs, uint8_t* __restrict__ cells,
+                                                                 Fr* __restrict__ scalars, const uint8_t* __restrict__ blobs,
+                                                                 const int* __restrict__ status, const Fr29* __restrict__ w29,
+                                                                 const Fr29* __restrict__ tapk, int n, int segs, SegShifts sh) {
+    extern __shared__ uint32_t s[];
+    const int b = blockIdx.x, h = blockIdx.y, tid = threadIdx.x;
+    for (int e = tid; e < N_BLOB; e += 1024) {
+        Fr29 c = fr29_from_fr_mont(coeffs[(size_t)b * N_BLOB + e]);
+        if (h && e) c = fr29_mul(c, w29[e]);
+        lds_store(s, e, c);
+    }
+    __syncthreads();
+    ntt4096_ct_forward_head(s, w29);
+    const int e0 = ((tid >> 6) << 8) + (tid & 63);
+#pragma unroll 1
+    for (int k = 0; k < 4; k++) {
+        const int e = e0 + 64 * k;
+        const Fr29 x = fk20_tap_scalar(LdsElems{s}, tapk, e, h);
+        const size_t at = (size_t)fk20_tap_row(e, h) * 64 + fk20_tap_column(e);
+        store_split_scalar(&scalars[(size_t)b * N_EXT + at], x);
+        for (int sg = 1; sg < segs; sg++)
+            store_split_scalar(&scalars[(size_t)(sg * n + b) * N_EXT + at], fr29_mul(x, sh.p[sg - 1]));
+    }
+    uint8_t* out = cells + ((size_t)b * N_EXT + (size_t)h * N_BLOB) * 32;
+    if (h == 0 && blobs && status[b] == 0) {
+        const uint4* src = reinterpret_cast<const uint4*>(blobs + (size_t)b * BYTES_PER_BLOB);
+        uint4* dst = reinterpret_cast<uint4*>(out);
+        for (int k = tid; k < BYTES_PER_BLOB / 16; k += 1024) dst[k] = src[k];
+        return;
+    }
+    ntt4096_ct_forward_tail(s, w29);
+    const Fr29 one_plain = fr29_const(r29::ONE_PLAIN);
+    for (int e = tid; e < N_BLOB; e += 1024)
+        store_fr_be(out + 32 * e, fr_words_of(fr29_reduce_once(fr29_mul(lds_load(s, e), one_plain))));
+}
+__global__ void k_fk20_tap_consts(const Fr29* __restrict__ w29, Fr29 scale_plain, Fr29* __restrict__ out) {
+    const int idx = blockIdx.x * blockDim.x + threadIdx.x;
+    if (idx < 2 * N_BLOB) out[idx] = fk20_tap_const(w29, scale_plain, idx);
 }
 
 #ifdef KZG_TEST_HOOKS
@@ -210,6 +259,7 @@
 void init_attributes() {
     hipFuncSetAttribute(reinterpret_cast<const void*>(k_blob_to_coeffs), hipFuncAttributeMaxDynamicSharedMemorySize, (int)LDS_NTT29);
     hipFuncSetAttribute(reinterpret_cast<const void*>(k_coeffs_to_cells), hipFuncAttributeMaxDynamicSharedMemorySize, (int)LDS_NTT29);
+    hipFuncSetAttribute(reinterpret_cast<const void*>(k_coeffs_to_cells_scalars), hipFuncAttributeMaxDynamicSharedMemorySize, (int)LDS_NTT29);
 #ifdef KZG_TEST_HOOKS
     hipFuncSetAttribute(reinterpret_cast<const void*>(k_test_ntt4096), hipFuncAttributeMaxDynamicSharedMemorySize, (int)LDS_NTT29);
 #endif
@@ -249,6 +299,19 @@
     for (int i = 0; i < 3; i++) sh.p[i] = fr29_mont_of(seg_shifts[i]);
     k_fk20_scalars<<<n * 16, 256, 0, st>>>((const Fr*)coeffs, (Fr*)scalars, (const Fr29*)w29, fr29_int32x_of(inv128), n, segs, sh);
 }
+void fk20_tap_consts(const void* w29, const Fr8& scale, void* out, hipStream_t st) {
+    k_fk20_tap_consts<<<2 * N_BLOB / 256, 256, 0, st>>>((const Fr29*)w29, fr29_from_plain(from_mont(as_fr(scale))), (Fr29*)out);
+}
+void coeffs_to_cells_scalars(int n, const void* coeffs, uint8_t* cells, void* scalars, const uint8_t* blobs, const int* status, const void* w29,
+                             const void* tapk, int segs, const Fr8* seg_shifts, hipStream_t st) {
+    const uintptr_t pb = (uintptr_t)blobs, pc = (uintptr_t)cells;
+    const bool apart = pb + (size_t)n * BYTES_PER_BLOB <= pc || pc + (size_t)n * N_EXT * 32 <= pb;
+    if (!status || ((pb | pc) & 15) || !apart) blobs = nullptr;
+    SegShifts sh;
+    for (int i = 0; i < 3; i++) sh.p[i] = fr29_mont_of(seg_shifts[i]);
+    k_coeffs_to_cells_scalars<<<dim3(n, 2), 1024, LDS_NTT29, st>>>((const Fr*)coeffs, cells, (Fr*)scalars, blobs, status, (const Fr29*)w29,
+                                                                   (const Fr29*)tapk, n, segs, sh);
+}
 #ifdef KZG_TEST_HOOKS
 void test_ntt4096(const uint8_t* in, uint8_t* out, const void* w29, const Fr8& n_inv, int inverse_dit, hipStream_t st) {
     k_test_ntt4096<<<1, 1024, LDS_NTT29, st>>>(in, out, (const Fr29*)w29, ntt_consts(n_inv), inverse_dit);
diff --git a/rust-eth-kzg_amd/csrc/knobs.hpp b/rust-eth-kzg_amd/csrc/knobs.hpp
--- a/rust-eth-kzg_amd/csrc/knobs.hpp
+++ b/rust-eth-kzg_amd/csrc/knobs.hpp
@@ -15,7 +15,7 @@
     int host_threads = 0;
     int serial_lanes = 0;
     bool trace = false;
-    int msm_chunks = -1, slp_program = -1, pip_shift_min = 0;
+    int msm_chunks = -1, slp_program = -1, pip_shift_min = 0, fused_scalars = -1;
     bool vm_search = true, vm_fold = true, verify_combine = true, msm_split = true;
     std::string fault;
     int device_batch_max = 0;
@@ -57,6 +57,7 @@
         flag("ETH_KZG_AMD_VM_FOLD", k.vm_fold);
         flag("ETH_KZG_AMD_VERIFY_COMBINE", k.verify_combine);
         flag("ETH_KZG_AMD_MSM_SPLIT", k.msm_split);
+        num("ETH_KZG_AMD_FUSED_SCALARS", 0, 1, k.fused_scalars);
         if (const char* s = getenv("ETH_KZG_AMD_FAULT")) k.fault = s;
         num("ETH_KZG_AMD_DEVICE_BATCH_MAX", 64, 1 << 20, k.device_batch_max);
         return k;
diff --git a/rust-eth-kzg_amd/csrc/launch.hpp b/rust-eth-kzg_amd/csrc/launch.hpp
--- a/rust-eth-kzg_amd/csrc/launch.hpp
+++ b/rust-eth-kzg_amd/csrc/launch.hpp
@@ -18,6 +18,9 @@
 void coeffs_to_cells(int n, const void* coeffs, uint8_t* cells, const void* w29, hipStream_t st);
 void fk20_scalars(int n, const void* coeffs, void* scalars, const void* w29, const Fr8& inv128, int segs, const Fr8* seg_shifts,
                   hipStream_t st);
+void fk20_tap_consts(const void* w29, const Fr8& scale, void* out , hipStream_t st);
+void coeffs_to_cells_scalars(int n, const void* coeffs, uint8_t* cells, void* scalars, const uint8_t* blobs, const int* status, const void* w29,
+                             const void* tapk, int segs, const Fr8* seg_shifts, hipStream_t st);
 void test_ntt4096(const uint8_t* in, uint8_t* out, const void* w29, const Fr8& n_inv, int inverse_dit, hipStream_t st);
 void test_scalars_be(const uint8_t* in, void* out, size_t n, hipStream_t st);
 void test_field_mul(const uint8_t* a, const uint8_t* b, uint8_t* out, int n, int is_fp, hipStream_t st);
```

After: 41300, median of 6. 1.01x the previous value.
